# GDMCF/GDMCF

Hardware: AMD Instinct MI355X
Metric: training users/sec (higher is better)
Workload: dtype f32; 1 GPU; yelp-shape synthetic rows, batch=400/GPU, dims=[1000], T=5, noise_scale=0.01, linear-var, mean_type=x0, reweight, AdamW lr=1e-5 (BASELINE configs[1]); n_items=34395, global_batch=400, parallelism=dp1, batch_rows=device CSR rows (CsrBatch)

## Files before the change

### gdmcf_amd/_lib.py

```python
import ctypes
import os
from ctypes import c_char_p, c_double, c_float, c_int, c_int64, c_size_t, c_uint64, c_void_p

_HERE = os.path.dirname(os.path.abspath(__file__))
LIB_PATH = os.path.join(_HERE, "csrc", "libgdmcf_hip.so")

GDMCF_OK, E_SHAPE, E_ARG, E_UNSUPPORTED, E_HIP, E_WORKSPACE = 0, -1, -2, -3, -4, -5
N_TABLES = 13
TABLE_NAMES = (
    "betas", "alphas_cumprod", "alphas_cumprod_prev", "alphas_cumprod_next", "sqrt_alphas_cumprod",
    "sqrt_one_minus_alphas_cumprod", "log_one_minus_alphas_cumprod", "sqrt_recip_alphas_cumprod",
    "sqrt_recipm1_alphas_cumprod", "posterior_variance", "posterior_log_variance_clipped",
    "posterior_mean_coef1", "posterior_mean_coef2",
)

P = c_void_p
_SIGNATURES = {
    "gdmcf_version": (c_int, []),
    "gdmcf_debug_last_gemm": (c_int, []),
    "gdmcf_last_error": (c_char_p, []),
    "gdmcf_device_info": (c_int, [P, P, c_char_p, c_int]),
    "gdmcf_prof_enable": (c_int, [c_int]),
    "gdmcf_prof_collect": (c_int, [c_int, P, P, P]),
    "gdmcf_schedule_build": (c_int, [c_int, c_double, c_double, c_double, c_int, c_int, P]),
    "gdmcf_densify_rows_f32": (c_int, [P, P, P, P, c_int, c_int, P, c_int64, P]),
    "gdmcf_dnn_prep_input_f32": (c_int, [P, c_int64, P, P, P, c_int, P, c_int64, c_int, P, c_int64, c_float, c_uint64,
                                         c_uint64, c_int, P, P, c_int, c_int, c_int, P, c_int64, P, c_int64, P, P, P]),
    "gdmcf_dnn_emb_cols_f32": (c_int, [P, P, P, c_int, c_int, c_int, P, c_int64, P, P]),
    "gdmcf_topn_metrics_f64": (c_int, [P, c_int64, c_int, P, P, P, c_int, P, P]),
    "gdmcf_gemm_precision": (c_int, [c_int]),
    "gdmcf_bf16_shadow_set": (c_int, [P, P, c_int64, c_int64, c_int64]),
    "gdmcf_bf16_shadow_clear": (c_int, [P]),
    "gdmcf_bf16_shadow_get": (P, [P]),
    "gdmcf_bf16_shadow_info": (c_int, [P, P, P, P, P]),
    "gdmcf_bf16_shadow_sync": (c_int, [P, c_int64, P]),
    "gdmcf_linear_ws_bytes": (c_size_t, [c_int, c_int, c_int]),
    "gdmcf_linear_fwd_f32": (c_int, [P, c_int64, P, c_int64, P, c_int, c_int, c_int, c_int, P, c_int64, P, c_size_t, P]),
    "gdmcf_linear_fwd_wt_f32": (c_int, [P, c_int64, P, c_int64, P, c_int, c_int, c_int, c_int, P, c_int64, P, c_size_t, P]),
    "gdmcf_loss_tiles": (c_int, [c_int]),
    "gdmcf_linear_loss_fwd_f32": (c_int, [P, c_int64, P, c_int64, P, P, c_int64, P, c_int, c_int, c_int, P, c_int64, P,
                                          c_int64, P, P, P]),
    "gdmcf_linear_posterior_fwd_f32": (c_int, [P, c_int64, P, c_int64, P, P, c_int64, P, P, P, P, P, P, c_int64, c_int,
                                               c_int, c_int, P, c_int64, P, c_int64, P]),
    "gdmcf_linear_bwd_input_f32": (c_int, [P, c_int64, P, c_int64, P, P, c_int64, c_int, c_int, c_int, c_int, P,
                                           c_int64, P, c_size_t, P]),
    "gdmcf_linear_bwd_weight_f32": (c_int, [P, c_int64, P, c_int64, P, c_int, c_int, c_int, c_int, P, c_int64, P, c_int, P]),
    "gdmcf_linear_bwd_weight_adamw_f32": (c_int, [P, c_int64, P, c_int64, P, c_int, c_int, c_int, c_int, P, c_int64, P, P, P, c_float,
                                                  c_float, c_float, c_float, c_float, c_int, c_float, P]),
    "gdmcf_rowscale_f32": (c_int, [P, c_int64, P, c_int, c_int, P, c_int64, P]),
    "gdmcf_emb_bwd_f32": (c_int, [P, c_int64, P, c_int64, c_int, c_int, P, c_int, c_int, P, P, P, P]),
    "gdmcf_row_loss_finish_f64": (c_int, [P, P, P, P, P, P, c_int, c_int, c_int, P, P, c_int, P, P, P, P]),
    "gdmcf_lt_history_update": (c_int, [P, P, c_int, c_int, c_int, P, P, P]),
    "gdmcf_onehot_noise_f32": (c_int, [P, c_int64, P, c_int, c_int, c_float, P, c_int64, c_uint64, c_uint64, P, c_int64, P,
                                     c_int64, P]),
    "gdmcf_row_norms_f32": (c_int, [P, c_int64, c_int, c_int, P, P, P]),
    "gdmcf_normalize_rows_bwd_f32": (c_int, [P, c_int64, P, c_int64, P, c_int, c_int, P, c_int64, P]),
    "gdmcf_tanh_bwd_f32": (c_int, [P, c_int64, P, c_int64, P, c_int64, P, c_int, c_int, P, c_int64, P]),
    "gdmcf_gather_rows_f32": (c_int, [P, c_int64, P, c_int, c_int, P, c_int64, P]),
    "gdmcf_scatter_add_rows_f32": (c_int, [P, c_int64, P, c_int, c_int, P, c_int64, P]),
    "gdmcf_normalize_rows_bwd_adamw_f32": (c_int, [P, c_int64, P, c_int64, P, c_int, c_int, P, c_int64, P, P, c_float, c_float,
                                                   c_float, c_float, c_float, c_int, c_float, P]),
    "gdmcf_scatter_rows_adamw_f32": (c_int, [P, c_int64, P, c_int, c_int, c_int, P, c_int64, P, P, c_float, c_float, c_float,
                                             c_float, c_float, c_int, c_float, P]),
    "gdmcf_dp_pack_f64": (c_int, [P, P, c_int, P, P, c_int, c_int, c_int, P, P]),
    "gdmcf_dp_unpack_f64": (c_int, [P, P, P, c_int, c_int, c_int, P, P, P]),
    "gdmcf_randn_f32": (c_int, [P, c_int64, c_int, c_int, c_int, c_uint64, c_uint64, P]),
    "gdmcf_eps_target_f32": (c_int, [P, c_int64, P, c_int64, P, c_int64, P, P, P, c_int, c_int, c_int, P, c_int64, P, P, P]),
    "gdmcf_sample_timesteps": (c_int, [P, P, c_int, c_int, c_int, c_double, c_uint64, c_uint64, P, P, P, P]),
    "gdmcf_adamw_f32": (c_int, [P, c_int, c_int, c_float, c_float, c_float, c_float, c_float, c_int, c_float, P]),
    "gdmcf_adamw_bf16s_f32": (c_int, [P, P, c_int, c_int, c_float, c_float, c_float, c_float, c_float, c_int, c_float, P]),
    "gdmcf_topk_masked_f32": (c_int, [P, c_int64, c_int, c_int, P, P, c_int, P, P, P]),
    "gdmcf_spmm_csr_f32": (c_int, [P, P, P, P, c_int, c_int, P, P, c_int, P, P, c_int, P, c_int64, c_int, P, c_int64, P, P, c_int,
                                   c_int64, c_float, c_double, P]),
    "gdmcf_spmm_bundled_f32": (c_int, [P, c_int, P, P, P, P, c_int, P, P, P, P, c_int, P, P, c_int, P, P, c_int64, c_int, c_int, P, c_int64, c_int, P,
                                       c_int64, P, P, c_int, c_int64, c_float, c_double, P]),
    "gdmcf_spmm_stream_f32": (c_int, [P, c_int, P, c_int64, P, c_int, P, P, c_int, c_int, c_int, P, c_int64, c_int, P, c_int64, P, P,
                                      c_int, c_int64, c_float, c_double, P]),
    "gdmcf_graph_guided_step_u8": (c_int, [P, c_int64, P, c_int, c_int, c_float, P, c_int64, P, P, c_int, c_uint64, c_uint64, P,
                                           c_int64, P, P]),
    "gdmcf_debug_spmm_stamps": (c_int, [c_int, P]),
    "gdmcf_graph_state_bytes": (c_int, []),
    "gdmcf_adam_hyper_bytes": (c_int, []),
    "gdmcf_graph_state_init": (c_int, [P, c_uint64, c_uint64, c_int64, c_int64, c_int64, P]),
    "gdmcf_adam_hyper_fill": (c_int, [P, c_int, c_float, c_float, c_float, c_float, c_float, c_int64, c_float]),
    "gdmcf_graph_state_bind": (c_int, [P]),
    "gdmcf_graph_state_tick": (c_int, [P, P]),
    "gdmcf_row_loss_finish_mean_f64": (c_int, [P, P, P, P, P, P, c_int, c_int, c_int, P, P, c_int, P, P, P, P, P, P]),
    "gdmcf_dnn_prep_input_csr_f32": (c_int, [P, P, P, P, P, P, c_int, P, c_int64, c_int, P, c_int64, c_float, c_uint64, c_uint64,
                                             P, P, c_int, c_int, c_int, P, c_int64, P, P, c_int64, P]),
    "gdmcf_linear_loss_fwd_bits_f32": (c_int, [P, c_int64, P, c_int64, P, P, c_int64, P, c_int, c_int, c_int, P, c_int64, P,
                                               c_int64, P, P, P]),
    "gdmcf_scale_f32": (c_int, [P, c_int64, c_float, P, P]),
}
EXPORTED_SYMBOLS = tuple(_SIGNATURES)

_lib = None


def load():
    global _lib
    if _lib is not None:
        return _lib
    if not os.path.exists(LIB_PATH):
        raise ImportError(
            f"{LIB_PATH} is missing: build it with `python -m gdmcf_amd.build` (hipcc, gfx950). "
            "gdmcf_amd has no CPU / PyTorch fallback.")
    lib = ctypes.CDLL(LIB_PATH)
    for name, (res, args) in _SIGNATURES.items():
        fn = getattr(lib, name)
        fn.restype = res
        fn.argtypes = args
    if lib.gdmcf_version() != 1:
        raise ImportError("libgdmcf_hip.so ABI version mismatch; rebuild with `python -m gdmcf_amd.build --force`")
    _lib = lib
    return lib


_EXC = {E_SHAPE: AssertionError, E_ARG: ValueError, E_UNSUPPORTED: NotImplementedError, E_HIP: RuntimeError,
        E_WORKSPACE: RuntimeError}


def check(rc):
    if rc != GDMCF_OK:
        msg = load().gdmcf_last_error().decode(errors="replace")
        raise _EXC.get(rc, RuntimeError)(msg or f"gdmcf error {rc}")


def ptr(t):
    return None if t is None else t.data_ptr()


def require_gpu(t, what):
    if not t.is_cuda:
        raise RuntimeError(f"gdmcf_amd: {what} must live on the MI355X (got device '{t.device}'); "
                           "the HIP path has no CPU fallback")


def shadow_info(data_ptr):
    p16 = ctypes.c_void_p()
    rows, cols, ld = ctypes.c_int64(), ctypes.c_int64(), ctypes.c_int64()
    if not load().gdmcf_bf16_shadow_info(data_ptr, ctypes.byref(p16), ctypes.byref(rows), ctypes.byref(cols), ctypes.byref(ld)):
        return None
    return int(p16.value), int(rows.value), int(cols.value), int(ld.value)


def stream_ptr():
    import torch
    return torch.cuda.current_stream().cuda_stream


def philox_randn(shape, device, seed, offset, stream_id=4, out=None):
    import torch
    rows, cols = int(shape[0]), int(shape[1])
    if out is None:
        out = torch.empty(rows, cols, dtype=torch.float32, device=device)
    require_gpu(out, "philox_randn output")
    check(load().gdmcf_randn_f32(out.data_ptr(), out.stride(0), rows, cols, int(stream_id), int(seed) & (2 ** 64 - 1),
                                 int(offset) & (2 ** 64 - 1), stream_ptr()))
    return out


def schedule_tables(kind, noise_scale, noise_min, noise_max, steps, beta_fixed=True):
    import numpy as np
    out = np.zeros((N_TABLES, steps), dtype=np.float64)
    rc = load().gdmcf_schedule_build(kind, float(noise_scale), float(noise_min), float(noise_max), int(steps),
                                     int(bool(beta_fixed)), out.ctypes.data_as(c_void_p))
    check(rc)
    return out


class Bf16Shadow:

    def __init__(self, t, sync=True):
        import weakref

        import torch
        require_gpu(t, "bf16 shadow source")
        if t.dim() != 2 or t.dtype != torch.float32 or t.stride(1) != 1:
            raise RuntimeError("gdmcf_amd: a bf16 shadow needs a 2-D float32 tensor with unit column stride")
        self.rows, self.cols = t.shape
        self.ptr = t.data_ptr()
        self.ld = t.stride(0)
        self.buf = torch.zeros((self.rows + 63) // 64 * 64, (self.cols + 63) // 64 * 64, dtype=torch.bfloat16,
                               device=t.device)
        self._lib = load()
        self._fin = weakref.finalize(self, self._lib.gdmcf_bf16_shadow_clear, self.ptr)
        self.register()
        if sync:
            self.sync()

    def register(self):
        check(self._lib.gdmcf_bf16_shadow_set(self.ptr, self.buf.data_ptr(), self.rows, self.cols, self.buf.stride(0)))

    def unregister(self):
        self._lib.gdmcf_bf16_shadow_clear(self.ptr)

    def sync(self):
        check(self._lib.gdmcf_bf16_shadow_sync(self.ptr, self.ld, stream_ptr()))

    def close(self):
        self._fin()
```

### gdmcf_amd/csrc/common.h

```cpp
#pragma once
#include <hip/hip_runtime.h>
#include <stdint.h>
#include <stdio.h>

#include "../../include/gdmcf_hip.h"

typedef float f32x4 __attribute__((ext_vector_type(4)));

void gdmcf_set_error(const char* fmt, ...);

#define GD_CHECK_SHAPE(cond, msg)            \
    do {                                     \
        if (!(cond)) {                       \
            gdmcf_set_error("%s", msg);      \
            return GDMCF_E_SHAPE;            \
        }                                    \
    } while (0)

#define GD_CHECK_ARG(cond, msg)              \
    do {                                     \
        if (!(cond)) {                       \
            gdmcf_set_error("%s", msg);      \
            return GDMCF_E_ARG;              \
        }                                    \
    } while (0)

static inline int gd_launch_status(const char* what) {
    hipError_t e = hipGetLastError();
    if (e != hipSuccess) {
        gdmcf_set_error("%s: %s", what, hipGetErrorString(e));
        return GDMCF_E_HIP;
    }
    return GDMCF_OK;
}

extern bool g_gd_prof_on;
void gd_prof_begin(int tag, double work, hipStream_t s);
void gd_prof_end(hipStream_t s);
struct GdProfScope {
    hipStream_t s;
    bool on;
    GdProfScope(int tag, double work, hipStream_t st) : s(st), on(g_gd_prof_on) {
        if (on) gd_prof_begin(tag, work, s);
    }
    ~GdProfScope() {
        if (on) gd_prof_end(s);
    }
};

static inline int gd_cdiv(int a, int b) { return (a + b - 1) / b; }
static inline bool gd_aligned16(const void* p) { return (reinterpret_cast<uintptr_t>(p) & 15u) == 0; }

struct GdShadow {
    void* p16;
    int64_t ld16;
    int64_t rows, cols;
};
bool gd_shadow_lookup(const void* f32, GdShadow* out);
int gd_cast_bf16(const float* src, int64_t ld, void* dst, int64_t ld16, int64_t rows, int64_t cols, hipStream_t s);

enum { GD_LAY_KC = 0, GD_LAY_MC = 1 };
enum { GD_EPI_SLAB = 0, GD_EPI_BIAS_ACT = 1, GD_EPI_LOSS = 2, GD_EPI_POST = 3, GD_EPI_STORE = 4, GD_EPI_ADAMW = 5 };

struct GdAdamHyper {
    float decay;
    float one_m_b1;
    float beta2;
    float one_m_b2;
    float bc2_sqrt;
    float eps;
    float neg_step;
    float grad_scale;
    float inv_bc2_sqrt;
    float pad_[3];
};
GdAdamHyper gd_adam_hyper(float lr, float beta1, float beta2, float eps, float weight_decay, int step, float grad_scale);

__device__ __forceinline__ void gd_adam_elem(float& p, float g, float& m, float& v, const GdAdamHyper& h) {
#pragma clang fp contract(off)
    g = g * h.grad_scale;
    p = p * h.decay;
    m = __builtin_fmaf(g - m, h.one_m_b1, m);
    v = __builtin_fmaf(h.one_m_b2 * g, g, v * h.beta2);
    const float denom = __builtin_fmaf(__builtin_amdgcn_sqrtf(v), h.inv_bc2_sqrt, h.eps);
    p = __builtin_fmaf(h.neg_step * m, __builtin_amdgcn_rcpf(denom), p);
}

struct GdStepState {
    uint64_t prep_offset;
    uint64_t ts_offset;
    int64_t adam_step;
    int64_t table_first;
    int64_t table_len;
    const GdAdamHyper* hyper_table;
    GdAdamHyper hyper;
};
extern thread_local const GdStepState* t_gd_step_state;

struct GdGemm {
    const float* A;
    int64_t lda;
    const float* B;
    int64_t ldb;
    int M, N, K;
    int kchunk;
    int splits;
    int tiles_m, tiles_n;
    int m_fastest;
    float* C;
    int64_t ldc;
    int64_t slab_stride;
    const float* bias;
    int act;
    const float* aux;
    int64_t ldaux;
    const uint32_t* aux_bits;
    int64_t ldbits;
    const float* aux2;
    int64_t ldaux2;
    const float* r0;
    const float* r1;
    const float* r2;
    const float* r3;
    const float* r4;
    float* out2;
    int64_t ldout2;
    float* rowpart;
    int ld_rowpart;
    int accumulate;
    int prof_tag;
    GdAdamHyper adam;
    const GdAdamHyper* adam_dev;
    const void* A16;
    int64_t lda16;
    const void* B16;
    int64_t ldb16;
    void* C16;
    int64_t ldc16;
    size_t ws_cap;
    int dbg;
    int bf16;
};

int gd_dr_kn_splits(int M, int N, int K);
extern thread_local int t_gd_last_gemm;

int gd_gemm_launch(int layA, int layB, int epi, int shape_class, GdGemm& g, hipStream_t s);
int gd_gemm_bf16_launch(int layA, int layB, int epi, int shape_class, GdGemm& g, hipStream_t s);
int gd_gemm_split_launch(int layA, int layB, int epi, int shape_class, GdGemm& g, hipStream_t s);
int gd_gemm_small_launch(int layA, int layB, int epi, GdGemm& g, hipStream_t s);
enum { GD_DR_NOT_TAKEN = 1 };
int gd_gemm_dr_launch(int layA, int layB, int epi, GdGemm& g, hipStream_t s);
int gd_gemm_tile_m(int shape_class);
int gd_gemm_tile_n(int shape_class);
int gd_gemm_bk(int layA, int layB);
int gd_pick_shape_class(int M, int N);
```

### gdmcf_amd/csrc/gemm_dr.hip

```cpp
#include <stdlib.h>

#include "common.h"

namespace {

typedef int i32x4 __attribute__((ext_vector_type(4)));
typedef unsigned int u32x4 __attribute__((ext_vector_type(4)));
typedef f32x4 f32x4_dr_u __attribute__((aligned(4)));

__device__ unsigned int g_dr_ticket[32][8][32];

__device__ __forceinline__ i32x4 dr_srd(const void* p, uint32_t bytes) {
    const uint64_t a = (uint64_t)p;
    return i32x4{(int)(uint32_t)a, (int)((uint32_t)(a >> 32) & 0xffffu), (int)bytes, 0x00020000};
}

__device__ __forceinline__ f32x4 dr_load(i32x4 srd, uint32_t voff, uint32_t soff) {
    f32x4 v;
    asm volatile("buffer_load_dwordx4 %0, %1, %2, %3 offen" : "=v"(v) : "v"(voff), "s"(srd), "s"(soff) : "memory");
    return v;
}

template <int N>
__device__ __forceinline__ void dr_wait() {
    asm volatile("s_waitcnt vmcnt(%0)" ::"n"(N) : "memory");
}

__device__ __forceinline__ unsigned int dr_ticket_issue(unsigned int* ctr) {
    unsigned int t;
    unsigned long long save;
    const unsigned int zero = 0, one = 1;
    asm volatile("s_mov_b64 %1, exec\n\ts_mov_b64 exec, 1\n\tglobal_atomic_add %0, %2, %3, %4 sc0\n\ts_mov_b64 exec, %1"
                 : "=&v"(t), "=&s"(save) : "v"(zero), "v"(one), "s"(ctr) : "memory");
    return t;
}

#ifndef GD_ADAMW_DBG
#define GD_ADAMW_DBG 0
#endif
#ifndef DR_ADAM_UB
#define DR_ADAM_UB 2
#endif

struct DrArgs {
    GdGemm g;
    int tiles_m, tiles_n, m_fastest;
    int ksp;
    int ctr;
    const GdAdamHyper* adam_dev;
    int stagger;
};

template <int TA, int TB, int D, int EPI>
__global__ __launch_bounds__(512, 2) void dr_tn_kernel(const DrArgs d) {
    static_assert(EPI == GD_EPI_STORE, "plain weight-gradient product (the fused-AdamW form: dr_tn_adamw_kernel)");
    constexpr int LPS = TA + TB;
    constexpr int R = D + 1;
    static_assert(LPS * D <= 63, "vmcnt is a 6-bit counter");
    const GdGemm& g = d.g;
    const int lane = threadIdx.x & 63;
    const int r = lane & 15, q = lane >> 4;
    const int n_waves = gridDim.x * 8;
    const int minor = d.m_fastest ? d.tiles_m : d.tiles_n;
    const int panels = d.m_fastest ? d.tiles_n : d.tiles_m;
    int xcc;
    asm volatile("s_getreg_b32 %0, hwreg(HW_REG_XCC_ID)" : "=s"(xcc));
    int qx = xcc & 7;
    int visited = 0;
    auto q_tiles = [&](int x) { return ((panels - x + 7) >> 3) * minor; };
    auto tile_of = [&](int x, int t) {
        const int p = (t / minor) * 8 + x, i = t % minor;
        return p * minor + i;
    };
    auto draw_blocking = [&]() {
        for (;;) {
            if (visited == 8) return -1;
            unsigned int* c = &g_dr_ticket[d.ctr][qx][0];
            unsigned int tk = dr_ticket_issue(c);
            dr_wait<0>();
            asm volatile("" : "+v"(tk));
            const int t = __builtin_amdgcn_readfirstlane(tk);
            const int n = q_tiles(qx);
            if (t == n + n_waves - 1 && lane == 0) __hip_atomic_store(c, 0u, __ATOMIC_RELAXED, __HIP_MEMORY_SCOPE_AGENT);
            if (t < n) return tile_of(qx, t);
            qx = (qx + 1) & 7;
            ++visited;
        }
    };
    if (d.stagger > 0 && __builtin_amdgcn_readfirstlane(threadIdx.x) >= 256)
        for (int i = 0; i < d.stagger; ++i) __builtin_amdgcn_s_sleep(127);
    int cur = draw_blocking();
    if (cur < 0) return;
    const int ntiles = d.tiles_m * d.tiles_n;
    const int KSP = d.ksp;
    const i32x4 srdA = dr_srd(g.A, (uint32_t)(((int64_t)(g.K - 1) * g.lda + g.M) * 4));
    const i32x4 srdB = dr_srd(g.B, (uint32_t)(((int64_t)(g.K - 1) * g.ldb + g.N) * 4));
    const uint32_t sa = 16u * (uint32_t)g.lda, sb = 16u * (uint32_t)g.ldb;
    const uint32_t c_bytes = (uint32_t)(((int64_t)(g.M - 1) * g.ldc + (g.out2 ? g.N - 1 : g.N)) * 4);
    const __amdgpu_buffer_rsrc_t srdC = __builtin_amdgcn_make_buffer_rsrc(g.C, 0, (int)c_bytes, 0x00020000);

    uint32_t offA[TA], offB[TB];
    uint32_t ka = 0, kb = 0;
    int l_left = KSP;
    auto set_cursor = [&](int tile) {
        const bool ok = tile < ntiles;
        const int tm = d.m_fastest ? (tile % d.tiles_m) : (tile / d.tiles_n);
        const int tn = d.m_fastest ? (tile / d.tiles_m) : (tile % d.tiles_n);
#pragma unroll
        for (int a = 0; a < TA; ++a) offA[a] = ok ? (uint32_t)(q * g.lda + tm * (64 * TA) + 64 * a + 4 * r) * 4u : 0xFFFFFFF0u;
#pragma unroll
        for (int b = 0; b < TB; ++b) offB[b] = ok ? (uint32_t)(q * g.ldb + tn * (64 * TB) + 64 * b + 4 * r) * 4u : 0xFFFFFFF0u;
        ka = kb = 0;
        l_left = KSP;
    };
    set_cursor(cur);
    f32x4 ra[R][TA], rb[R][TB];
#pragma unroll
    for (int u = 0; u < D; ++u) {
#pragma unroll
        for (int a = 0; a < TA; ++a) ra[u][a] = dr_load(srdA, offA[a], ka);
#pragma unroll
        for (int b = 0; b < TB; ++b) rb[u][b] = dr_load(srdB, offB[b], kb);
        ka += sa;
        kb += sb;
        --l_left;
    }
    const int q1 = (KSP / R / 4) * R, q2 = (KSP / R / 2) * R, q3 = (KSP / R * 3 / 4) * R;
    for (;;) {
        unsigned int* tctr = &g_dr_ticket[d.ctr][qx][0];
        unsigned int tick = visited < 8 ? dr_ticket_issue(tctr) : 0u;
        const bool drew = visited < 8;
        int nxt = 0;
        const int tm = d.m_fastest ? (cur % d.tiles_m) : (cur / d.tiles_n);
        const int tn = d.m_fastest ? (cur / d.tiles_m) : (cur % d.tiles_n);
        const int m0 = tm * 64 * TA, n0 = tn * 64 * TB;
        f32x4 acc[TA][4][TB][4];
#pragma unroll
        for (int a = 0; a < TA; ++a)
#pragma unroll
            for (int e = 0; e < 4; ++e)
#pragma unroll
                for (int b = 0; b < TB; ++b)
#pragma unroll
                    for (int f = 0; f < 4; ++f) acc[a][e][b][f] = f32x4{0.f, 0.f, 0.f, 0.f};
        __builtin_amdgcn_s_setprio(0);
        for (int s0 = 0; s0 < KSP; s0 += R) {
            if (s0 == q1) __builtin_amdgcn_s_setprio(1);
            else if (s0 == q2) __builtin_amdgcn_s_setprio(2);
            else if (s0 == q3) __builtin_amdgcn_s_setprio(3);
#pragma unroll
            for (int u = 0; u < R; ++u) {
                constexpr int NM = 16 * TA * TB;
                const int v = (u + D) % R;
                dr_wait<LPS*(D - 1)>();
#pragma unroll
                for (int a = 0; a < TA; ++a) asm volatile("" : "+v"(ra[u][a]));
#pragma unroll
                for (int b = 0; b < TB; ++b) asm volatile("" : "+v"(rb[u][b]));
#pragma unroll
                for (int i = 0; i < NM; ++i) {
                    const int a = i / (16 * TB), e = (i / (4 * TB)) % 4, b = (i / 4) % TB, f = i % 4;
                    acc[a][e][b][f] = __builtin_amdgcn_mfma_f32_16x16x4f32(ra[u][a][e], rb[u][b][f], acc[a][e][b][f], 0, 0, 0);
                    if (i % 4 == 1 && i / 4 < LPS) {
                        __builtin_amdgcn_sched_barrier(0);
                        const int l = i / 4;
                        if (l < TA) ra[v][l] = dr_load(srdA, offA[l], ka);
                        else rb[v][l - TA] = dr_load(srdB, offB[l - TA], kb);
                        __builtin_amdgcn_sched_barrier(0);
                    }
                    if (i == 4 * LPS + 1) {
                        __builtin_amdgcn_sched_barrier(0);
                        ka += sa;
                        kb += sb;
                        if (--l_left == 0) {
                            nxt = -1;
                            if (drew) {
                                if (KSP < 2 * D + 2) dr_wait<0>();
                                asm volatile("" : "+v"(tick));
                                const int tk = __builtin_amdgcn_readfirstlane(tick);
                                const int nq = q_tiles(qx);
                                if (tk == nq + n_waves - 1 && lane == 0) __hip_atomic_store(tctr, 0u, __ATOMIC_RELAXED, __HIP_MEMORY_SCOPE_AGENT);
                                if (tk < nq) {
                                    nxt = tile_of(qx, tk);
                                } else {
                                    qx = (qx + 1) & 7;
                                    ++visited;
                                    nxt = draw_blocking();
                                }
                            }
                            if (nxt < 0) nxt = ntiles;
                            set_cursor(nxt);
                        }
                        __builtin_amdgcn_sched_barrier(0);
                    }
                }
                __builtin_amdgcn_sched_barrier(0);
            }
        }
#pragma unroll
        for (int b = 0; b < TB; ++b) {
            const int n = n0 + 64 * b + 4 * r;
            const uint32_t vo = (uint32_t)(16 * q * g.ldc + n) * 4u;
            if (n + 3 < (g.out2 ? g.N - 1 : g.N)) {
#pragma unroll
                for (int a = 0; a < TA; ++a)
#pragma unroll
                    for (int t = 0; t < 4; ++t)
#pragma unroll
                        for (int e = 0; e < 4; ++e) {
                            f32x4 gv = {acc[a][e][b][0][t], acc[a][e][b][1][t], acc[a][e][b][2][t], acc[a][e][b][3][t]};
                            const uint32_t so = (uint32_t)(m0 + 64 * a + 4 * t + e) * (uint32_t)g.ldc * 4u;
                            __builtin_amdgcn_raw_buffer_store_b128(__builtin_bit_cast(u32x4, gv), srdC, vo + so, 0, 0);
                        }
            } else if (n < g.N) {
                for (int a = 0; a < TA; ++a)
                    for (int t = 0; t < 4; ++t)
                        for (int e = 0; e < 4; ++e) {
                            const int m = m0 + 64 * a + 16 * q + 4 * t + e;
                            if (m >= g.M) continue;
                            for (int k = 0; k < 4; ++k) {
                                if (n + k >= g.N) continue;
                                const float gk = acc[a][e][b][k][t];
                                if (g.out2 && n + k == g.N - 1) g.out2[m] = gk;
                                else g.C[(int64_t)m * g.ldc + n + k] = gk;
                            }
                        }
            }
        }
        if (nxt >= ntiles) break;
        cur = nxt;
    }
    dr_wait<0>();
#pragma unroll
    for (int u = 0; u < R; ++u) {
#pragma unroll
        for (int a = 0; a < TA; ++a) asm volatile("" ::"v"(ra[u][a]));
#pragma unroll
        for (int b = 0; b < TB; ++b) asm volatile("" ::"v"(rb[u][b]));
    }
}

#ifdef GD_NO_SNOP
#define GD_SNOP ""
#else
#define GD_SNOP "s_nop 4\n\t"
#endif
#ifndef GD_ADAMW_ST
#define GD_ADAMW_ST 1
#endif
__device__ __forceinline__ void dr_store(f32x4 v, i32x4 srd, uint32_t voff) {
#if GD_ADAMW_ST == 1
    asm volatile(GD_SNOP "buffer_store_dwordx4 %0, %1, %2, 0 offen nt\n\ts_nop 1" ::"v"(v), "v"(voff), "s"(srd) : "memory");
#elif GD_ADAMW_ST == 2
    asm volatile(GD_SNOP "buffer_store_dwordx4 %0, %1, %2, 0 offen sc1\n\ts_nop 1" ::"v"(v), "v"(voff), "s"(srd) : "memory");
#elif GD_ADAMW_ST == 3
    asm volatile(GD_SNOP "buffer_store_dwordx4 %0, %1, %2, 0 offen sc0 sc1\n\ts_nop 1" ::"v"(v), "v"(voff), "s"(srd) : "memory");
#else
    asm volatile(GD_SNOP "buffer_store_dwordx4 %0, %1, %2, 0 offen\n\ts_nop 1" ::"v"(v), "v"(voff), "s"(srd) : "memory");
#endif
}
#ifndef GD_ADAMW_LD
#define GD_ADAMW_LD 0
#endif
template <bool NTL>
__device__ __forceinline__ void dr_load0_rw(f32x4& v, i32x4 srd, uint32_t voff) {
    if constexpr (NTL) {
        asm volatile(GD_SNOP "buffer_load_dwordx4 %0, %1, %2, 0 offen nt" : "+v"(v) : "v"(voff), "s"(srd) : "memory");
        return;
    }
#if GD_ADAMW_LD == 1
    asm volatile(GD_SNOP "buffer_load_dwordx4 %0, %1, %2, 0 offen nt" : "+v"(v) : "v"(voff), "s"(srd) : "memory");
#elif GD_ADAMW_LD == 2
    asm volatile(GD_SNOP "buffer_load_dwordx4 %0, %1, %2, 0 offen sc1" : "+v"(v) : "v"(voff), "s"(srd) : "memory");
#elif GD_ADAMW_LD == 3
    asm volatile(GD_SNOP "buffer_load_dwordx4 %0, %1, %2, 0 offen sc0 sc1" : "+v"(v) : "v"(voff), "s"(srd) : "memory");
#elif GD_ADAMW_LD == 4
    asm volatile(GD_SNOP "buffer_load_dwordx4 %0, %1, %2, 0 offen sc0 sc1 nt" : "+v"(v) : "v"(voff), "s"(srd) : "memory");
#else
    asm volatile(GD_SNOP "buffer_load_dwordx4 %0, %1, %2, 0 offen" : "+v"(v) : "v"(voff), "s"(srd) : "memory");
#endif
}

template <int D, bool NTL>
__global__ __launch_bounds__(512, 2) void dr_tn_adamw_kernel(const DrArgs d) {
    constexpr int LPS = 2;
    constexpr int R = D + 1;
    constexpr int UA = 1, UB = 1 + R / 2;
    constexpr int XS = 6;
    constexpr int XR = 12;
    static_assert(UB < R && UB > UA, "two distinct steps of a round");
    static_assert(LPS * R + XS <= 63, "vmcnt is a 6-bit counter");
    constexpr uint32_t PARK = 0xFFFFFF00u;
    const GdGemm& g = d.g;
    const int lane = threadIdx.x & 63;
    const int wave = __builtin_amdgcn_readfirstlane(threadIdx.x >> 6);
    const int r = lane & 15, q = lane >> 4;
    extern __shared__ __attribute__((aligned(16))) float dr_lds[];
    f32x4* const stash = reinterpret_cast<f32x4*>(dr_lds + wave * 4096) + lane;
    GdAdamHyper hy = g.adam;
    if (d.adam_dev) hy = *d.adam_dev;
    const int n_waves = gridDim.x * 8;
    const int minor = d.m_fastest ? d.tiles_m : d.tiles_n;
    const int panels = d.m_fastest ? d.tiles_n : d.tiles_m;
    int xcc;
    asm volatile("s_getreg_b32 %0, hwreg(HW_REG_XCC_ID)" : "=s"(xcc));
    int qx = xcc & 7, visited = 0;
    auto q_tiles = [&](int x) { return ((panels - x + 7) >> 3) * minor; };
    auto tile_of = [&](int x, int t) { return ((t / minor) * 8 + x) * minor + t % minor; };
    auto draw_blocking = [&]() {
        for (;;) {
            if (visited == 8) return -1;
            unsigned int* c = &g_dr_ticket[d.ctr][qx][0];
            unsigned int tk = dr_ticket_issue(c);
            dr_wait<0>();
            asm volatile("" : "+v"(tk));
            const int t = __builtin_amdgcn_readfirstlane(tk);
            const int n = q_tiles(qx);
            if (t == n + n_waves - 1 && lane == 0) __hip_atomic_store(c, 0u, __ATOMIC_RELAXED, __HIP_MEMORY_SCOPE_AGENT);
            if (t < n) return tile_of(qx, t);
            qx = (qx + 1) & 7;
            ++visited;
        }
    };
    if (d.stagger > 0 && __builtin_amdgcn_readfirstlane(threadIdx.x) >= 256)
        for (int i = 0; i < d.stagger; ++i) __builtin_amdgcn_s_sleep(127);
    int cur = draw_blocking();
    if (cur < 0) return;
    const int ntiles = d.tiles_m * d.tiles_n;
    const int KSP = d.ksp;
    const i32x4 srdA = dr_srd(g.A, (uint32_t)(((int64_t)(g.K - 1) * g.lda + g.M) * 4));
    const i32x4 srdB = dr_srd(g.B, (uint32_t)(((int64_t)(g.K - 1) * g.ldb + g.N) * 4));
    const uint32_t sa = 16u * (uint32_t)g.lda, sb = 16u * (uint32_t)g.ldb;
    const int n_lim = g.out2 ? g.N - 1 : g.N;
    const uint32_t c_bytes = (uint32_t)(((int64_t)(g.M - 1) * g.ldc + n_lim) * 4);
    const i32x4 srdW = dr_srd(g.C, c_bytes), srdM = dr_srd(g.aux, c_bytes), srdV = dr_srd(g.aux2, c_bytes);
    const uint32_t ldc4 = (uint32_t)g.ldc * 4u;

    uint32_t offA, offB, ka = 0, kb = 0;
    int l_left = KSP;
    auto set_cursor = [&](int tile) {
        const bool ok = tile < ntiles;
        const int tm = d.m_fastest ? (tile % d.tiles_m) : (tile / d.tiles_n);
        const int tn = d.m_fastest ? (tile / d.tiles_m) : (tile % d.tiles_n);
        offA = ok ? (uint32_t)(q * g.lda + tm * 64 + 4 * r) * 4u : 0xFFFFFFF0u;
        offB = ok ? (uint32_t)(q * g.ldb + tn * 64 + 4 * r) * 4u : 0xFFFFFFF0u;
        ka = kb = 0;
        l_left = KSP;
    };
    set_cursor(cur);
    uint32_t pend_base = PARK;
    bool pend_lane = false;
    int pend_g = 16;
    struct Slot {
        f32x4 p, m, v;
        uint32_t off;
        int gi;
        bool live;
    } sl[2];
#pragma unroll
    for (int k = 0; k < 2; ++k) {
        asm volatile("" : "=v"(sl[k].p));
        asm volatile("" : "=v"(sl[k].m));
        asm volatile("" : "=v"(sl[k].v));
        sl[k].off = PARK;
        sl[k].gi = 0;
        sl[k].live = false;
    }
    auto opt_pick = [&](Slot& s_) {
        const bool act = pend_g < 16;
        s_.live = act;
        s_.gi = act ? pend_g : 0;
        s_.off = (act && pend_lane && !(GD_ADAMW_DBG & 2)) ? pend_base + (uint32_t)pend_g * ldc4 : PARK;
        pend_g += act ? 1 : 0;
    };
    auto opt_update_store = [&](Slot& s_) {
        const float* sg = reinterpret_cast<const float*>(stash + 256 * (s_.gi & 3)) + (s_.gi >> 2);
        float gr[4];
#pragma unroll
        for (int f = 0; f < 4; ++f) gr[f] = sg[256 * f];
        f32x4 pn = s_.p, mn = s_.m, vn = s_.v;
#if !(GD_ADAMW_DBG & 1)
#pragma unroll
        for (int k = 0; k < 4; ++k) {
            float pk = pn[k], mk = mn[k], vk = vn[k];
            gd_adam_elem(pk, gr[k], mk, vk, hy);
            pn[k] = pk;
            mn[k] = mk;
            vn[k] = vk;
        }
#else
        pn[0] += gr[0] + gr[1] + gr[2] + gr[3];
#endif
        const uint32_t so = (GD_ADAMW_DBG & 8) ? PARK : ((GD_ADAMW_DBG & 16) && s_.off != PARK) ? s_.off + 448u * ldc4 : s_.off;
        dr_store(pn, srdW, so);
        dr_store(mn, srdM, so);
        dr_store(vn, srdV, so);
    };
    auto opt_load = [&](Slot& s_) {
        const uint32_t lo = (GD_ADAMW_DBG & 4) ? PARK : s_.off;
        dr_load0_rw<NTL>(s_.p, srdW, lo);
        dr_load0_rw<NTL>(s_.m, srdM, lo);
        dr_load0_rw<NTL>(s_.v, srdV, lo);
    };
    auto opt_pin = [&](Slot& s_) {
        asm volatile("" : "+v"(s_.p));
        asm volatile("" : "+v"(s_.m));
        asm volatile("" : "+v"(s_.v));
    };

    f32x4 ra[R], rb[R];
#pragma unroll
    for (int u = 0; u < D; ++u) {
        ra[u] = dr_load(srdA, offA, ka);
        rb[u] = dr_load(srdB, offB, kb);
        ka += sa;
        kb += sb;
        --l_left;
        const int w = (u + 1) % R;
        if (w == UA || w == UB) {
            const f32x4 z = {0.f, 0.f, 0.f, 0.f};
#pragma unroll
            for (int k = 0; k < XS / 3; ++k) {
                dr_store(z, srdW, PARK);
                dr_store(z, srdM, PARK);
                dr_store(z, srdV, PARK);
            }
        }
    }
    const int q1 = (KSP / R / 4) * R, q2 = (KSP / R / 2) * R, q3 = (KSP / R * 3 / 4) * R;
    const bool defer_all = KSP / R >= 9;
    for (;;) {
        unsigned int* tctr = &g_dr_ticket[d.ctr][qx][0];
        unsigned int tick = visited < 8 ? dr_ticket_issue(tctr) : 0u;
        const bool drew = visited < 8;
        int nxt = 0;
        const int tm = d.m_fastest ? (cur % d.tiles_m) : (cur / d.tiles_n);
        const int tn = d.m_fastest ? (cur / d.tiles_m) : (cur % d.tiles_n);
        const int m0 = tm * 64, n0 = tn * 64;
        f32x4 acc[4][4];
#pragma unroll
        for (int e = 0; e < 4; ++e)
#pragma unroll
            for (int f = 0; f < 4; ++f) acc[e][f] = f32x4{0.f, 0.f, 0.f, 0.f};
        __builtin_amdgcn_s_setprio(0);
        for (int s0 = 0; s0 < KSP; s0 += R) {
            if (s0 == q1) __builtin_amdgcn_s_setprio(1);
            else if (s0 == q2) __builtin_amdgcn_s_setprio(2);
            else if (s0 == q3) __builtin_amdgcn_s_setprio(3);
#pragma unroll
            for (int u = 0; u < R; ++u) {
                const int v = (u + D) % R;
                if (u == UA || u == UB) dr_wait<LPS*(D - 1) + XR - XS>();
                else dr_wait<LPS*(D - 1) + XR>();
                asm volatile("" : "+v"(ra[u]));
                asm volatile("" : "+v"(rb[u]));
#pragma unroll
                for (int i = 0; i < 16; ++i) {
                    const int e = i / 4, f = i % 4;
                    acc[e][f] = __builtin_amdgcn_mfma_f32_16x16x4f32(ra[u][e], rb[u][f], acc[e][f], 0, 0, 0);
                    if (i == 1) {
                        __builtin_amdgcn_sched_barrier(0);
                        ra[v] = dr_load(srdA, offA, ka);
                        __builtin_amdgcn_sched_barrier(0);
                    } else if (i == 5) {
                        __builtin_amdgcn_sched_barrier(0);
                        rb[v] = dr_load(srdB, offB, kb);
                        __builtin_amdgcn_sched_barrier(0);
                    } else if (i == 9) {
                        __builtin_amdgcn_sched_barrier(0);
                        ka += sa;
                        kb += sb;
                        if (--l_left == 0) {
                            nxt = -1;
                            if (drew) {
                                if (KSP < 2 * D + 2) dr_wait<0>();
                                asm volatile("" : "+v"(tick));
                                const int tk = __builtin_amdgcn_readfirstlane(tick);
                                const int nq = q_tiles(qx);
                                if (tk == nq + n_waves - 1 && lane == 0) __hip_atomic_store(tctr, 0u, __ATOMIC_RELAXED, __HIP_MEMORY_SCOPE_AGENT);
                                if (tk < nq) {
                                    nxt = tile_of(qx, tk);
                                } else {
                                    qx = (qx + 1) & 7;
                                    ++visited;
                                    nxt = draw_blocking();
                                }
                            }
                            if (nxt < 0) nxt = ntiles;
                            set_cursor(nxt);
                        }
                        __builtin_amdgcn_sched_barrier(0);
                    } else if ((u == UA || u == UB) && i == 11) {
                        __builtin_amdgcn_sched_barrier(0);
                        Slot& s_ = sl[u == UA ? 0 : 1];
                        dr_wait<LPS * R + XS>();
                        opt_pin(s_);
                        opt_update_store(s_);
                        opt_pick(s_);
                        opt_load(s_);
                        __builtin_amdgcn_sched_barrier(0);
                    }
                }
                __builtin_amdgcn_sched_barrier(0);
            }
        }
        const uint32_t vo = (uint32_t)(16 * q * g.ldc + n0 + 4 * r) * 4u;
        const int n = n0 + 4 * r;
        const bool lane_full = n + 3 < n_lim;
        if (defer_all) {
#pragma unroll
            for (int e = 0; e < 4; ++e)
#pragma unroll
                for (int f = 0; f < 4; ++f) stash[64 * (4 * e + f)] = acc[e][f];
            pend_base = vo + (uint32_t)m0 * ldc4;
            pend_lane = lane_full;
            pend_g = 0;
        } else if (lane_full) {
            const __amdgpu_buffer_rsrc_t rW = __builtin_amdgcn_make_buffer_rsrc(g.C, 0, (int)c_bytes, 0x00020000);
            const __amdgpu_buffer_rsrc_t rM = __builtin_amdgcn_make_buffer_rsrc(const_cast<float*>(g.aux), 0, (int)c_bytes, 0x00020000);
            const __amdgpu_buffer_rsrc_t rV = __builtin_amdgcn_make_buffer_rsrc(const_cast<float*>(g.aux2), 0, (int)c_bytes, 0x00020000);
#pragma unroll
            for (int t = 0; t < 4; ++t)
#pragma unroll
                for (int e = 0; e < 4; ++e) {
                    const uint32_t o = vo + (uint32_t)(m0 + 4 * t + e) * ldc4;
                    f32x4 pv = __builtin_bit_cast(f32x4, __builtin_amdgcn_raw_buffer_load_b128(rW, o, 0, 0));
                    f32x4 mv = __builtin_bit_cast(f32x4, __builtin_amdgcn_raw_buffer_load_b128(rM, o, 0, 0));
                    f32x4 vv = __builtin_bit_cast(f32x4, __builtin_amdgcn_raw_buffer_load_b128(rV, o, 0, 0));
#pragma unroll
                    for (int k = 0; k < 4; ++k) {
                        float pk = pv[k], mk = mv[k], vk = vv[k];
                        gd_adam_elem(pk, acc[e][k][t], mk, vk, hy);
                        pv[k] = pk;
                        mv[k] = mk;
                        vv[k] = vk;
                    }
                    __builtin_amdgcn_raw_buffer_store_b128(__builtin_bit_cast(u32x4, pv), rW, o, 0, 0);
                    __builtin_amdgcn_raw_buffer_store_b128(__builtin_bit_cast(u32x4, mv), rM, o, 0, 0);
                    __builtin_amdgcn_raw_buffer_store_b128(__builtin_bit_cast(u32x4, vv), rV, o, 0, 0);
                }
        }
        if (!lane_full && n < g.N) {
            float* __restrict__ Mo = const_cast<float*>(g.aux);
            float* __restrict__ Vo = const_cast<float*>(g.aux2);
            for (int t = 0; t < 4; ++t)
                for (int e = 0; e < 4; ++e) {
                    const int m = m0 + 16 * q + 4 * t + e;
                    if (m >= g.M) continue;
                    for (int k = 0; k < 4; ++k) {
                        if (n + k >= g.N) continue;
                        const int64_t o = (int64_t)m * g.ldc + n + k;
                        const float gk = acc[e][k][t];
                        if (g.out2 && n + k == g.N - 1) {
                            g.out2[m] = gk;
                            continue;
                        }
                        float pk = g.C[o], mk = Mo[o], vk = Vo[o];
                        gd_adam_elem(pk, gk, mk, vk, hy);
                        g.C[o] = pk;
                        Mo[o] = mk;
                        Vo[o] = vk;
                    }
                }
        }
        if (nxt >= ntiles) break;
        cur = nxt;
    }
    dr_wait<0>();
#pragma unroll
    for (int u = 0; u < R; ++u) {
        asm volatile("" ::"v"(ra[u]));
        asm volatile("" ::"v"(rb[u]));
    }
#pragma unroll
    for (int k = 0; k < 2; ++k) {
        opt_pin(sl[k]);
        opt_update_store(sl[k]);
    }
    dr_wait<0>();
    {
        const __amdgpu_buffer_rsrc_t rW = __builtin_amdgcn_make_buffer_rsrc(g.C, 0, (int)c_bytes, 0x00020000);
        const __amdgpu_buffer_rsrc_t rM = __builtin_amdgcn_make_buffer_rsrc(const_cast<float*>(g.aux), 0, (int)c_bytes, 0x00020000);
        const __amdgpu_buffer_rsrc_t rV = __builtin_amdgcn_make_buffer_rsrc(const_cast<float*>(g.aux2), 0, (int)c_bytes, 0x00020000);
        for (; pend_g < 16; pend_g += 4) {
            f32x4 pv[4], mv[4], vv[4];
            uint32_t oo[4];
#pragma unroll
            for (int u = 0; u < 4; ++u) {
                oo[u] = (pend_lane && !(GD_ADAMW_DBG & 2)) ? pend_base + (uint32_t)(pend_g + u) * ldc4 : PARK;
                pv[u] = __builtin_bit_cast(f32x4, __builtin_amdgcn_raw_buffer_load_b128(rW, oo[u], 0, 0));
                mv[u] = __builtin_bit_cast(f32x4, __builtin_amdgcn_raw_buffer_load_b128(rM, oo[u], 0, 0));
                vv[u] = __builtin_bit_cast(f32x4, __builtin_amdgcn_raw_buffer_load_b128(rV, oo[u], 0, 0));
            }
#pragma unroll
            for (int u = 0; u < 4; ++u) {
                const int gi = pend_g + u;
                const float* sg = reinterpret_cast<const float*>(stash + 256 * (gi & 3)) + (gi >> 2);
#pragma unroll
                for (int k = 0; k < 4; ++k) {
                    float pk = pv[u][k], mk = mv[u][k], vk = vv[u][k];
                    gd_adam_elem(pk, sg[256 * k], mk, vk, hy);
                    pv[u][k] = pk;
                    mv[u][k] = mk;
                    vv[u][k] = vk;
                }
                __builtin_amdgcn_raw_buffer_store_b128(__builtin_bit_cast(u32x4, pv[u]), rW, oo[u], 0, 2);
                __builtin_amdgcn_raw_buffer_store_b128(__builtin_bit_cast(u32x4, mv[u]), rM, oo[u], 0, 2);
                __builtin_amdgcn_raw_buffer_store_b128(__builtin_bit_cast(u32x4, vv[u]), rV, oo[u], 0, 2);
            }
        }
    }
}

template <int TMB, int NB, int D, int EPI>
__global__ __launch_bounds__(512, 2) void dr_nt_kernel(const DrArgs d) {
    static_assert(EPI == GD_EPI_BIAS_ACT || EPI == GD_EPI_LOSS || EPI == GD_EPI_POST, "forward products");
    static_assert(NB == 4 || NB == 2, "B loads per chunk: 16 NB output columns, NB consecutive ones per lane");
    constexpr int LPC = TMB + NB;
    constexpr int R = D + 1;
    constexpr int NM = 4 * TMB * NB;
    constexpr int SP = NM / (LPC + 1);
    static_assert(SP >= 2 && SP * LPC + 1 < NM, "loads and cursor step must fall inside the chunk");
    static_assert(LPC * D <= 63, "vmcnt is a 6-bit counter");
    const GdGemm& g = d.g;
    const int lane = threadIdx.x & 63;
    const int r = lane & 15, q = lane >> 4;
    const int ntiles = d.tiles_m * d.tiles_n;
    unsigned int* ctr = &g_dr_ticket[d.ctr][0][0];
    const int n_waves = gridDim.x * 8;
    int cur = __builtin_amdgcn_readfirstlane(blockIdx.x * 8 + (threadIdx.x >> 6));
    if (cur >= ntiles) return;
    if (d.stagger > 0 && __builtin_amdgcn_readfirstlane(threadIdx.x) >= 256)
        for (int i = 0; i < d.stagger; ++i) __builtin_amdgcn_s_sleep(127);
    const int NCP = d.ksp;
    const i32x4 srdA = dr_srd(g.A, (uint32_t)(((int64_t)(g.M - 1) * g.lda + g.K) * 4));
    const i32x4 srdB = dr_srd(g.B, (uint32_t)(((int64_t)(g.N - 1) * g.ldb + g.K) * 4));

    uint32_t offA[TMB], offB[NB];
    uint32_t kc = 0;
    int l_left = NCP;
    auto set_cursor = [&](int tile) {
        const bool ok = tile < ntiles;
        const int tm = tile % d.tiles_m, tn = tile / d.tiles_m;
#pragma unroll
        for (int i = 0; i < TMB; ++i) offA[i] = ok ? (uint32_t)((tm * (16 * TMB) + 16 * i + r) * g.lda + 4 * q) * 4u : 0xFFFFFFF0u;
#pragma unroll
        for (int f = 0; f < NB; ++f) offB[f] = ok ? (uint32_t)((tn * (16 * NB) + NB * r + f) * g.ldb + 4 * q) * 4u : 0xFFFFFFF0u;
        kc = 0;
        l_left = NCP;
    };
    set_cursor(cur);
    f32x4 xa[R][TMB], xb[R][NB];
#pragma unroll
    for (int u = 0; u < D; ++u) {
#pragma unroll
        for (int i = 0; i < TMB; ++i) xa[u][i] = dr_load(srdA, offA[i], kc);
#pragma unroll
        for (int f = 0; f < NB; ++f) xb[u][f] = dr_load(srdB, offB[f], kc);
        kc += 64;
        --l_left;
    }
    const int q1 = (NCP / R / 4) * R, q2 = (NCP / R / 2) * R, q3 = (NCP / R * 3 / 4) * R;
    const int c_mask = g.K >> 4;
    for (;;) {
        unsigned int tick = dr_ticket_issue(ctr);
        int nxt = 0;
        const int tm = cur % d.tiles_m, tn = cur / d.tiles_m;
        const int m0 = tm * 16 * TMB, n0 = tn * (16 * NB);
        f32x4 acc[TMB][NB];
#pragma unroll
        for (int i = 0; i < TMB; ++i)
#pragma unroll
            for (int f = 0; f < NB; ++f) acc[i][f] = f32x4{0.f, 0.f, 0.f, 0.f};
        __builtin_amdgcn_s_setprio(0);
        for (int c0 = 0; c0 < NCP; c0 += R) {
            if (c0 == q1) __builtin_amdgcn_s_setprio(1);
            else if (c0 == q2) __builtin_amdgcn_s_setprio(2);
            else if (c0 == q3) __builtin_amdgcn_s_setprio(3);
#pragma unroll
            for (int u = 0; u < R; ++u) {
                const int v = (u + D) % R;
                dr_wait<LPC*(D - 1)>();
#pragma unroll
                for (int i = 0; i < TMB; ++i) asm volatile("" : "+v"(xa[u][i]));
#pragma unroll
                for (int f = 0; f < NB; ++f) asm volatile("" : "+v"(xb[u][f]));
                if (c0 + u >= c_mask) {
                    const int kq = (c0 + u) * 16 + 4 * q;
#pragma unroll
                    for (int e = 0; e < 4; ++e) {
                        const bool keep = kq + e < g.K;
#pragma unroll
                        for (int i = 0; i < TMB; ++i) xa[u][i][e] = keep ? xa[u][i][e] : 0.f;
#pragma unroll
                        for (int f = 0; f < NB; ++f) xb[u][f][e] = keep ? xb[u][f][e] : 0.f;
                    }
                }
#pragma unroll
                for (int n = 0; n < NM; ++n) {
                    const int e = n / (TMB * NB), i = (n / NB) % TMB, f = n % NB;
                    acc[i][f] = __builtin_amdgcn_mfma_f32_16x16x4f32(xa[u][i][e], xb[u][f][e], acc[i][f], 0, 0, 0);
                    if (n % SP == 1 && n / SP < LPC) {
                        __builtin_amdgcn_sched_barrier(0);
                        const int l = n / SP;
                        if (l < TMB) xa[v][l] = dr_load(srdA, offA[l], kc);
                        else xb[v][l - TMB] = dr_load(srdB, offB[l - TMB], kc);
                        __builtin_amdgcn_sched_barrier(0);
                    }
                    if (n == SP * LPC + 1) {
                        __builtin_amdgcn_sched_barrier(0);
                        kc += 64;
                        if (--l_left == 0) {
                            if (NCP < 2 * D + 2) dr_wait<0>();
                            asm volatile("" : "+v"(tick));
                            const int tk = __builtin_amdgcn_readfirstlane(tick);
                            if (tk == ntiles - 1 && lane == 0) __hip_atomic_store(ctr, 0u, __ATOMIC_RELAXED, __HIP_MEMORY_SCOPE_AGENT);
                            nxt = n_waves + tk;
                            set_cursor(nxt);
                        }
                        __builtin_amdgcn_sched_barrier(0);
                    }
                }
                __builtin_amdgcn_sched_barrier(0);
            }
        }
        typedef float vecnb __attribute__((ext_vector_type(NB)));
        typedef vecnb vecnb_u __attribute__((aligned(4)));
        const int n = n0 + NB * r;
        const bool full = n + NB - 1 < g.N;
        float biasv[NB];
#pragma unroll
        for (int f = 0; f < NB; ++f) biasv[f] = g.bias ? g.bias[min(n + f, g.N - 1)] : 0.f;
        const bool has_z = (EPI == GD_EPI_POST) && (g.aux2 != nullptr);
        const bool has_r = (EPI == GD_EPI_POST) && (g.r2 != nullptr);
        auto put = [&](float* base, int64_t ld, int m, const float (&val)[NB]) {
            if (full) {
                vecnb w;
#pragma unroll
                for (int f = 0; f < NB; ++f) w[f] = val[f];
                *reinterpret_cast<vecnb_u*>(base + (int64_t)m * ld + n) = w;
            } else {
                for (int f = 0; f < NB; ++f)
                    if (n + f < g.N) base[(int64_t)m * ld + n + f] = val[f];
            }
        };
#pragma unroll
        for (int i = 0; i < TMB; ++i) {
            float racc[4];
#pragma unroll
            for (int t = 0; t < 4; ++t) {
                const int m = m0 + 16 * i + 4 * q + t;
                const int mc = min(m, g.M - 1);
                const bool mok = m < g.M;
                float v4[NB];
#pragma unroll
                for (int f = 0; f < NB; ++f) v4[f] = acc[i][f][t] + biasv[f];
                racc[t] = 0.f;
                if (EPI == GD_EPI_BIAS_ACT) {
                    if (g.act == 1) {
#pragma unroll
                        for (int f = 0; f < NB; ++f) v4[f] = tanhf(v4[f]);
                    }
                    if (mok) put(g.C, g.ldc, m, v4);
                } else if (EPI == GD_EPI_LOSS) {
                    const float c1 = g.r0 ? g.r0[mc] : 1.f;
                    float tg[NB];
                    if (g.aux_bits) {
                        const uint32_t w = g.aux_bits[(int64_t)mc * g.ldbits + min((int64_t)(n >> 5), g.ldbits - 1)];
#pragma unroll
                        for (int f = 0; f < NB; ++f) tg[f] = (float)((w >> ((n & 31) + f)) & 1u);
                    } else {
#pragma unroll
                        for (int f = 0; f < NB; ++f) tg[f] = g.aux[(int64_t)mc * g.ldaux + min(n + f, g.N - 1)];
                    }
                    float dd[NB], ss = 0.f;
#pragma unroll
                    for (int f = 0; f < NB; ++f) {
                        dd[f] = c1 * v4[f] - tg[f];
                        if (mok && n + f < g.N) ss += dd[f] * dd[f];
                    }
                    if (mok) {
                        put(g.C, g.ldc, m, dd);
                        if (g.out2) put(g.out2, g.ldout2, m, v4);
                    }
                    racc[t] = ss;
                } else {
                    const float c1 = g.r0[mc], c2 = g.r1[mc];
                    const float p1 = has_r ? g.r2[mc] : 0.f, p2 = has_r ? g.r3[mc] : 0.f;
                    const float sg = has_z ? g.r4[mc] : 0.f;
                    float pr[NB], mn[NB];
#pragma unroll
                    for (int f = 0; f < NB; ++f) {
                        const int nf = min(n + f, g.N - 1);
                        const float xt = g.aux[(int64_t)mc * g.ldaux + nf];
                        const float zz = has_z ? g.aux2[(int64_t)mc * g.ldaux2 + nf] : 0.f;
                        pr[f] = has_r ? (p1 * xt - p2 * v4[f]) : v4[f];
                        mn[f] = c1 * pr[f] + c2 * xt;
                        if (has_z) mn[f] += sg * zz;
                    }
                    if (mok) {
                        put(g.C, g.ldc, m, mn);
                        if (g.out2) put(g.out2, g.ldout2, m, pr);
                    }
                }
            }
            if (EPI == GD_EPI_LOSS) {
#pragma unroll
                for (int t = 0; t < 4; ++t) {
                    float sv = racc[t];
                    sv += __shfl_xor(sv, 1);
                    sv += __shfl_xor(sv, 2);
                    sv += __shfl_xor(sv, 4);
                    sv += __shfl_xor(sv, 8);
                    const int m = m0 + 16 * i + 4 * q + t;
                    if (r == 0 && m < g.M) g.rowpart[(int64_t)m * g.ld_rowpart + tn] = sv;
                }
            }
            __builtin_amdgcn_sched_barrier(0);
        }
        if (nxt >= ntiles) break;
        cur = nxt;
    }
    dr_wait<0>();
#pragma unroll
    for (int u = 0; u < R; ++u) {
#pragma unroll
        for (int i = 0; i < TMB; ++i) asm volatile("" ::"v"(xa[u][i]));
#pragma unroll
        for (int f = 0; f < NB; ++f) asm volatile("" ::"v"(xb[u][f]));
    }
}


__device__ __forceinline__ f32x4 dr_load_g(i32x4 srd, uint32_t voff, uint32_t soff) {
    f32x4 v;
    asm volatile("s_nop 4\n\tbuffer_load_dwordx4 %0, %1, %2, %3 offen" : "=v"(v) : "v"(voff), "s"(srd), "s"(soff) : "memory");
    return v;
}
__device__ __forceinline__ float dr_load1_g(i32x4 srd, uint32_t voff, uint32_t soff) {
    float v;
    asm volatile("s_nop 4\n\tbuffer_load_dword %0, %1, %2, %3 offen" : "=v"(v) : "v"(voff), "s"(srd), "s"(soff) : "memory");
    return v;
}


__global__ __launch_bounds__(256) void dr_transpose_kernel(const float* __restrict__ A, int64_t lda, int M, int K,
                                                           float* __restrict__ At, int ldt) {
    __shared__ float t[32][33];
    const int k0 = blockIdx.x * 32, m0 = blockIdx.y * 32;
    const int x = threadIdx.x & 31, y = threadIdx.x >> 5;
#pragma unroll
    for (int i = 0; i < 4; ++i) {
        const int m = m0 + y + 8 * i, k = k0 + x;
        t[y + 8 * i][x] = (m < M && k < K) ? A[(int64_t)m * lda + k] : 0.f;
    }
    __syncthreads();
#pragma unroll
    for (int i = 0; i < 4; ++i) {
        const int k = k0 + y + 8 * i, m = m0 + x;
        if (k < K && m < M) At[(int64_t)k * ldt + m] = t[x][y + 8 * i];
    }
}

__device__ __forceinline__ void dr_load_rw(f32x4& v, i32x4 srd, uint32_t voff, uint32_t soff) {
    asm volatile("buffer_load_dwordx4 %0, %1, %2, %3 offen" : "+v"(v) : "v"(voff), "s"(srd), "s"(soff) : "memory");
}
__device__ __forceinline__ void dr_load1_rw(float& v, i32x4 srd, uint32_t voff, uint32_t soff) {
    asm volatile("buffer_load_dword %0, %1, %2, %3 offen" : "+v"(v) : "v"(voff), "s"(srd), "s"(soff) : "memory");
}
#ifdef HL_NOA
#define HL_KA(x) (0x80000000u)
#else
#define HL_KA(x) (x)
#endif
#ifdef HL_NOB
#define HL_KB(x) (0x80000000u)
#else
#define HL_KB(x) (x)
#endif
template <int EPI>
__global__ __launch_bounds__(512, 2) void dr_hl_kernel(const DrArgs d) {
    static_assert(EPI == GD_EPI_LOSS, "output layer with the fused row loss");
    constexpr int LPS = 3;
    constexpr int D = 7;
    static_assert(LPS * D <= 63, "vmcnt is a 6-bit counter");
    const GdGemm& g = d.g;
    const int lane = threadIdx.x & 63;
    const int wave = __builtin_amdgcn_readfirstlane(threadIdx.x >> 6);
    const int r = lane & 15, q = lane >> 4;
    extern __shared__ __attribute__((aligned(16))) float dr_lds[];
    float* const lds = dr_lds + wave * 4096;
    const int w_ev = (lane >> 3) * 32 + (((lane & 7) ^ (lane >> 4)) << 2), w_od = w_ev ^ 16;
    const int r_h0 = r * 32 + ((q ^ ((r >> 1) & 7)) << 2), r_h1 = r_h0 ^ 16;

    const int n_waves = gridDim.x * (blockDim.x >> 6);
    const int minor = d.tiles_m, panels = d.tiles_n;
    int xcc;
    asm volatile("s_getreg_b32 %0, hwreg(HW_REG_XCC_ID)" : "=s"(xcc));
    int qx = xcc & 7, visited = 0;
    auto q_tiles = [&](int x) { return ((panels - x + 7) >> 3) * minor; };
    auto tile_of = [&](int x, int t) { return ((t / minor) * 8 + x) * minor + t % minor; };
    auto draw_blocking = [&]() {
        for (;;) {
            if (visited == 8) return -1;
            unsigned int* c = &g_dr_ticket[d.ctr][qx][0];
            unsigned int tk = dr_ticket_issue(c);
            dr_wait<0>();
            asm volatile("" : "+v"(tk));
            const int t = __builtin_amdgcn_readfirstlane(tk);
            const int n = q_tiles(qx);
            if (t == n + n_waves - 1 && lane == 0) __hip_atomic_store(c, 0u, __ATOMIC_RELAXED, __HIP_MEMORY_SCOPE_AGENT);
            if (t < n) return tile_of(qx, t);
            qx = (qx + 1) & 7;
            ++visited;
        }
    };
    if (d.stagger > 0 && __builtin_amdgcn_readfirstlane(threadIdx.x) >= 256)
        for (int i = 0; i < d.stagger; ++i) __builtin_amdgcn_s_sleep(127);
    int cur = draw_blocking();
    if (cur < 0) return;
    const int NCH = d.ksp;
    const i32x4 srdA = dr_srd(g.A, (uint32_t)(((int64_t)(g.K - 1) * g.lda + g.M) * 4));
    const i32x4 srdB = dr_srd(g.B, (uint32_t)(((int64_t)(g.N - 1) * g.ldb + g.K) * 4));
    const uint32_t sa1 = 4u * (uint32_t)g.lda, sa13 = 13u * sa1;
    const uint32_t ub8 = 32u * (uint32_t)g.ldb;
    const int q1 = (NCH / 8) * 2, q2 = (NCH / 4) * 2, q3 = (NCH * 3 / 8) * 2;

    for (;;) {
        unsigned int* tctr = &g_dr_ticket[d.ctr][qx][0];
        const bool drew = visited < 8;
        unsigned int tick = drew ? dr_ticket_issue(tctr) : 0u;
        const int tm = cur % d.tiles_m, tn = cur / d.tiles_m;
        const int m0 = tm * 80, n0 = tn * 64;
        const uint32_t oA4 = (uint32_t)(4 * q * g.lda + m0 + 4 * r) * 4u;
        const uint32_t oA1 = (uint32_t)(4 * q * g.lda + m0 + 64 + r) * 4u;
        const uint32_t oB = (uint32_t)(((int64_t)(n0 + (lane >> 3)) * g.ldb + 4 * (lane & 7)) * 4);
        uint32_t ka = 0;
        f32x4 ra4[8], G[8], FB[2][4];
        float ra1[8];
        f32x4 acc[5][4];
#pragma unroll
        for (int e = 0; e < 5; ++e)
#pragma unroll
            for (int b = 0; b < 4; ++b) acc[e][b] = f32x4{0.f, 0.f, 0.f, 0.f};
        __builtin_amdgcn_s_setprio(0);
#pragma unroll
        for (int u = 0; u < 8; ++u) G[u] = dr_load_g(srdB, oB, (uint32_t)u * ub8);
        dr_wait<0>();
#pragma unroll
        for (int u = 0; u < 8; ++u) {
            asm volatile("" : "+v"(G[u]));
            *reinterpret_cast<f32x4*>(lds + u * 256 + ((u & 1) ? w_od : w_ev)) = G[u];
        }
        G[0] = dr_load_g(srdB, oB, 128u);
#pragma unroll
        for (int u = 1; u < 8; ++u) {
            ra4[u - 1] = dr_load_g(srdA, oA4, ka);
            ra1[u - 1] = dr_load1_g(srdA, oA1, ka);
            ka += ((u - 1) & 3) == 3 ? sa13 : sa1;
            G[u] = dr_load_g(srdB, oB, 128u + (uint32_t)u * ub8);
        }
        dr_wait<21>();
        asm volatile("" : "=v"(ra4[7]));
        asm volatile("" : "=v"(ra1[7]));
        asm volatile("" : "+v"(G[0]));
        *reinterpret_cast<f32x4*>(lds + 2048 + w_ev) = G[0];
#pragma unroll
        for (int b = 0; b < 4; ++b) FB[0][b] = *reinterpret_cast<const f32x4*>(lds + b * 512 + r_h0);
        uint32_t kb = 256u;

        for (int c0 = 0; c0 < NCH; c0 += 2) {
            if (c0 == q1) __builtin_amdgcn_s_setprio(1);
            else if (c0 == q2) __builtin_amdgcn_s_setprio(2);
            else if (c0 == q3) __builtin_amdgcn_s_setprio(3);
#pragma unroll
            for (int uu = 0; uu < 16; ++uu) {
                const int p = uu >> 3, u = uu & 7, h = u >> 2, sx = u & 3;
                const int v = (u + 7) & 7;
                const int w = (u + 1) & 7;
                const uint32_t kbs = (c0 + p + 2 < NCH) ? kb : 0x80000000u;
                dr_wait<LPS * (D - 1)>();
                asm volatile("" : "+v"(ra4[u]));
                asm volatile("" : "+v"(ra1[u]));
                asm volatile("" : "+v"(G[w]));
                *reinterpret_cast<f32x4*>(lds + ((u < 7) ? (1 - p) : p) * 2048 + w * 256 + ((w & 1) ? w_od : w_ev)) = G[w];
                __builtin_amdgcn_sched_barrier(0);
#pragma unroll
                for (int i = 0; i < 20; ++i) {
                    const int e = i >> 2, b = i & 3;
                    const float av = e < 4 ? ra4[u][e] : ra1[u];
                    acc[e][b] = __builtin_amdgcn_mfma_f32_16x16x4f32(av, FB[h][b][sx], acc[e][b], 0, 0, 0);
                    if (i == 1) {
                        __builtin_amdgcn_sched_barrier(0);
                        dr_load_rw(ra4[v], srdA, oA4, HL_KA(ka));
                        __builtin_amdgcn_sched_barrier(0);
                    } else if (i == 5) {
                        __builtin_amdgcn_sched_barrier(0);
                        dr_load1_rw(ra1[v], srdA, oA1, HL_KA(ka));
                        ka += (v & 3) == 3 ? sa13 : sa1;
                        __builtin_amdgcn_sched_barrier(0);
                    } else if (i == 9) {
                        __builtin_amdgcn_sched_barrier(0);
                        dr_load_rw(G[u], srdB, oB, HL_KB(kbs + (uint32_t)u * ub8));
                        if (u == 7) kb += 128u;
                        __builtin_amdgcn_sched_barrier(0);
                    } else if (i == 13 && u == 3) {
                        __builtin_amdgcn_sched_barrier(0);
#pragma unroll
                        for (int bb = 0; bb < 4; ++bb) FB[1][bb] = *reinterpret_cast<const f32x4*>(lds + p * 2048 + bb * 512 + r_h1);
                        __builtin_amdgcn_sched_barrier(0);
                    } else if (i == 13 && u == 7) {
                        __builtin_amdgcn_sched_barrier(0);
#pragma unroll
                        for (int bb = 0; bb < 4; ++bb) FB[0][bb] = *reinterpret_cast<const f32x4*>(lds + (1 - p) * 2048 + bb * 512 + r_h0);
                        __builtin_amdgcn_sched_barrier(0);
                    }
                }
                __builtin_amdgcn_sched_barrier(0);
            }
        }
        dr_wait<0>();
#pragma unroll
        for (int u = 0; u < 8; ++u) {
            asm volatile("" ::"v"(ra4[u]));
            asm volatile("" ::"v"(ra1[u]));
            asm volatile("" ::"v"(G[u]));
        }
        int nxt = -1;
        if (drew) {
            asm volatile("" : "+v"(tick));
            const int tk = __builtin_amdgcn_readfirstlane(tick);
            const int nq = q_tiles(qx);
            if (tk == nq + n_waves - 1 && lane == 0) __hip_atomic_store(tctr, 0u, __ATOMIC_RELAXED, __HIP_MEMORY_SCOPE_AGENT);
            if (tk < nq) {
                nxt = tile_of(qx, tk);
            } else {
                qx = (qx + 1) & 7;
                ++visited;
                nxt = -2;
            }
        }
        {
            int ncl[4];
            bool nok[4];
            float biasv[4];
#pragma unroll
            for (int b = 0; b < 4; ++b) {
                const int n = n0 + 16 * b + r;
                nok[b] = n < g.N;
                ncl[b] = min(n, g.N - 1);
                biasv[b] = g.bias ? g.bias[ncl[b]] : 0.f;
            }
#pragma unroll
            for (int e = 0; e < 5; ++e) {
                float tg[4][4], c1v[4];
#pragma unroll
                for (int t = 0; t < 4; ++t) {
                    const int m = e < 4 ? m0 + 16 * q + 4 * t + e : m0 + 64 + 4 * q + t;
                    const int mc = min(m, g.M - 1);
                    c1v[t] = g.r0 ? g.r0[mc] : 1.f;
                    if (g.aux_bits) {
                        uint32_t wv[2];
#pragma unroll
                        for (int jj = 0; jj < 2; ++jj)
                            wv[jj] = g.aux_bits[(int64_t)mc * g.ldbits + min((int64_t)((n0 >> 5) + jj), g.ldbits - 1)];
#pragma unroll
                        for (int b = 0; b < 4; ++b) tg[t][b] = (float)((wv[b >> 1] >> (16 * (b & 1) + r)) & 1u);
                    } else {
#pragma unroll
                        for (int b = 0; b < 4; ++b) tg[t][b] = g.aux[(int64_t)mc * g.ldaux + ncl[b]];
                    }
                }
#pragma unroll
                for (int t = 0; t < 4; ++t) {
                    const int m = e < 4 ? m0 + 16 * q + 4 * t + e : m0 + 64 + 4 * q + t;
                    const bool mok = m < g.M;
                    float ss = 0.f;
#pragma unroll
                    for (int b = 0; b < 4; ++b) {
                        const float vv = acc[e][b][t] + biasv[b];
                        const float dd = c1v[t] * vv - tg[t][b];
                        if (mok && nok[b]) {
                            if (g.out2) g.out2[(int64_t)m * g.ldout2 + ncl[b]] = vv;
                            g.C[(int64_t)m * g.ldc + ncl[b]] = dd;
                            ss += dd * dd;
                        }
                    }
                    ss += __shfl_xor(ss, 1);
                    ss += __shfl_xor(ss, 2);
                    ss += __shfl_xor(ss, 4);
                    ss += __shfl_xor(ss, 8);
                    if (r == 0 && mok) g.rowpart[(int64_t)m * g.ld_rowpart + tn] = ss;
                }
                __builtin_amdgcn_sched_barrier(0);
            }
        }
        if (nxt == -2) nxt = draw_blocking();
        if (nxt < 0) break;
        cur = nxt;
    }
}

template <int NB, int EPI>
__global__ __launch_bounds__(256, 1) void dr_fat_kernel(const DrArgs d) {
    static_assert(EPI == GD_EPI_LOSS || EPI == GD_EPI_POST, "output layer with a fused epilogue");
    static_assert(NB >= 4 && NB <= 12, "5 x NB accumulator blocks must fit 256 registers");
    constexpr int TMB = 5;
    const GdGemm& g = d.g;
    const int lane = threadIdx.x & 63;
    const int wave = __builtin_amdgcn_readfirstlane(threadIdx.x >> 6);
    const int r = lane & 15, q = lane >> 4;
    extern __shared__ __attribute__((aligned(16))) float dr_lds[];
    float* const lds = dr_lds + wave * (2 * NB * 256);
    const int nblk = gridDim.x, per = nblk >> 3;
    const int wl = ((nblk & 7) == 0 ? ((int)(blockIdx.x & 7) * per + (int)(blockIdx.x >> 3)) : (int)blockIdx.x) * 4 + wave;
    const int n_waves = nblk * 4;
    const int ntiles = d.tiles_m * d.tiles_n;
    const __amdgpu_buffer_rsrc_t srdA = __builtin_amdgcn_make_buffer_rsrc(const_cast<float*>(g.A), 0, (int)(((int64_t)(g.M - 1) * g.lda + g.K) * 4), 0x00020000);
    const __amdgpu_buffer_rsrc_t srdB = __builtin_amdgcn_make_buffer_rsrc(const_cast<float*>(g.B), 0, (int)(((int64_t)(g.N - 1) * g.ldb + g.K) * 4), 0x00020000);
    const int NCH = d.ksp;
    const int c_mask = g.K >> 4;
    const int w_off = (lane >> 2) * 16 + (((lane & 3) ^ ((((lane >> 2) >> 2) & 1) << 1)) << 2);
    const int r_off = r * 16 + ((q ^ (((r >> 2) & 1) << 1)) << 2);
    for (int tile = wl; tile < ntiles; tile += n_waves) {
        const int tm = tile % d.tiles_m, tn = tile / d.tiles_m;
        const int m0 = tm * (16 * TMB), n0 = tn * (16 * NB);
        uint32_t offA[TMB], offB[NB];
#pragma unroll
        for (int i = 0; i < TMB; ++i) offA[i] = (uint32_t)((m0 + 16 * i + r) * g.lda + 4 * q) * 4u;
#pragma unroll
        for (int p = 0; p < NB; ++p) offB[p] = (uint32_t)(((int64_t)(n0 + 16 * p + (lane >> 2)) * g.ldb + 4 * (lane & 3)) * 4);
        f32x4 acc[TMB][NB];
#pragma unroll
        for (int i = 0; i < TMB; ++i)
#pragma unroll
            for (int b = 0; b < NB; ++b) acc[i][b] = f32x4{0.f, 0.f, 0.f, 0.f};
        f32x4 xa[2][TMB], G[NB], FB[NB];
#pragma unroll
        for (int i = 0; i < TMB; ++i) xa[0][i] = __builtin_bit_cast(f32x4, __builtin_amdgcn_raw_buffer_load_b128(srdA, offA[i], 0, 0));
#pragma unroll
        for (int p = 0; p < NB; ++p) G[p] = __builtin_bit_cast(f32x4, __builtin_amdgcn_raw_buffer_load_b128(srdB, offB[p], 0, 0));
#pragma unroll
        for (int p = 0; p < NB; ++p) *reinterpret_cast<f32x4*>(lds + p * 256 + w_off) = G[p];

#define GD_FAT_CHUNK(PAR, c)                                                                                          \
        {                                                                                                             \
             \
            const uint32_t kn = ((c) + 1 < NCH) ? (uint32_t)((c) + 1) * 64u : 0x80000000u;                            \
            _Pragma("unroll") for (int b = 0; b < NB; ++b)                                                            \
                FB[b] = *reinterpret_cast<const f32x4*>(lds + (PAR) * (NB * 256) + b * 256 + r_off);                  \
            if ((c) >= c_mask) {  \
                 \
                _Pragma("unroll") for (int e = 0; e < 4; ++e) {                                                       \
                    const bool keep = (c) * 16 + 4 * q + e < g.K;                                                     \
                    _Pragma("unroll") for (int i = 0; i < TMB; ++i) xa[PAR][i][e] = keep ? xa[PAR][i][e] : 0.f;       \
                    _Pragma("unroll") for (int b = 0; b < NB; ++b) FB[b][e] = keep ? FB[b][e] : 0.f;                  \
                }                                                                                                     \
            }                                                                                                         \
            __builtin_amdgcn_sched_barrier(0);                                                                        \
            _Pragma("unroll") for (int sx = 0; sx < 4; ++sx) {                                                        \
                _Pragma("unroll") for (int n = 0; n < TMB * NB; ++n) {                                                \
                    const int i = n / NB, b = n % NB;                                                                 \
                    if (sx == 0 && i == 0) asm volatile("" : "+v"(FB[b]));  \
                    if (sx == 0 && b == 0) asm volatile("" : "+v"(xa[PAR][i]));                                       \
                    acc[i][b] = __builtin_amdgcn_mfma_f32_16x16x4f32(xa[PAR][i][sx], FB[b][sx], acc[i][b], 0, 0, 0);  \
                     \
                    if (sx < 2 && n % 5 == 2) {      \
                        const int l = (sx == 0) ? n / 5 : NB + n / 5;                                                 \
                        if (l < TMB + NB) {                                                                           \
                            __builtin_amdgcn_sched_barrier(0);                                                        \
                            if (l < TMB)                                                                              \
                                xa[(PAR) ^ 1][l] = __builtin_bit_cast(f32x4, __builtin_amdgcn_raw_buffer_load_b128(   \
                                    srdA, offA[l], kn, 0));                                                           \
                            else                                                                                      \
                                G[l - TMB] = __builtin_bit_cast(f32x4, __builtin_amdgcn_raw_buffer_load_b128(         \
                                    srdB, offB[l - TMB], kn, 0));                                                     \
                            __builtin_amdgcn_sched_barrier(0);                                                        \
                        }                                                                                             \
                    }                                                                                                 \
                    if (sx == 3 && n % 4 == 1 && n / 4 < NB) {   \
                        __builtin_amdgcn_sched_barrier(0);                                                            \
                        *reinterpret_cast<f32x4*>(lds + ((PAR) ^ 1) * (NB * 256) + (n / 4) * 256 + w_off) = G[n / 4]; \
                        __builtin_amdgcn_sched_barrier(0);                                                            \
                    }                                                                                                 \
                }                                                                                                     \
                __builtin_amdgcn_sched_barrier(0);                                                                    \
            }                                                                                                         \
        }
        const int c_pf = d.stagger > 0 ? ((NCH > d.stagger + 2 ? NCH - d.stagger : 0) & ~1) : -2;
        for (int c = 0; c + 1 < NCH; c += 2) {
            if constexpr (EPI == GD_EPI_POST) {
                if (c == c_pf) {
                    typedef __attribute__((address_space(3))) void* lds_vp;
                    constexpr int NJL = (16 * NB * 4 + 127) / 128 + 1;
                    constexpr int NPI = (80 * NJL + 63) / 64;
                    float* const scratch = dr_lds + 4 * (2 * NB * 256) + wave * 64;
                    const __amdgpu_buffer_rsrc_t srdX = __builtin_amdgcn_make_buffer_rsrc(
                        const_cast<float*>(g.aux), 0, (int)(((int64_t)(g.M - 1) * g.ldaux + g.N) * 4), 0x00020000);
#pragma unroll
                    for (int pi = 0; pi < NPI; ++pi) {
                        const int t = min(pi * 64 + lane, 80 * NJL - 1);
                        const int row = min(m0 + t % 80, g.M - 1), j = t / 80;
                        const int col = min(j < NJL - 1 ? n0 + 32 * j : n0 + 16 * NB - 1, g.N - 1);
                        __builtin_amdgcn_raw_ptr_buffer_load_lds(srdX, (lds_vp)scratch, 4, (int)(((int64_t)row * g.ldaux + col) * 4), 0, 0, 0);
                    }
                }
            }
            GD_FAT_CHUNK(0, c);
            GD_FAT_CHUNK(1, c + 1);
        }
        if (NCH & 1) GD_FAT_CHUNK(0, NCH - 1);
#undef GD_FAT_CHUNK

        constexpr int LDS_ = 16 * NB + 4;
        constexpr int NJ = (4 * NB + 15) / 16;
        typedef f32x4 f32x4_e __attribute__((aligned(4)));
        f32x4 bias4[NJ];
        int col4[NJ];
#pragma unroll
        for (int j = 0; j < NJ; ++j) {
            col4[j] = n0 + 4 * (r + 16 * j);
            bias4[j] = f32x4{0.f, 0.f, 0.f, 0.f};
            if (g.bias && r + 16 * j < 4 * NB) {
#pragma unroll
                for (int e = 0; e < 4; ++e) bias4[j][e] = g.bias[min(col4[j] + e, g.N - 1)];
            }
        }
        const bool has_z = (EPI == GD_EPI_POST) && (g.aux2 != nullptr);
        const bool has_r = (EPI == GD_EPI_POST) && (g.r2 != nullptr);
        struct Pre {
            f32x4 a[NJ], z[NJ];
            uint32_t w[NJ];
            float c1, c2, p1, p2, sg;
        } pre[2];
        auto fetch = [&](int i, int p4, Pre& P) {
            const int mc = min(m0 + 16 * i + 4 * p4 + q, g.M - 1);
            P.c1 = 1.f; P.c2 = 0.f; P.p1 = 0.f; P.p2 = 0.f; P.sg = 0.f;
            if (EPI == GD_EPI_LOSS) {
                if (g.r0) P.c1 = g.r0[mc];
            } else {
                P.c1 = g.r0[mc];
                P.c2 = g.r1[mc];
                if (has_r) { P.p1 = g.r2[mc]; P.p2 = g.r3[mc]; }
                if (has_z) P.sg = g.r4[mc];
            }
#pragma unroll
            for (int j = 0; j < NJ; ++j) {
                const int n = col4[j];
                const bool whole = (r + 16 * j < 4 * NB) && n + 3 < g.N;
                P.w[j] = 0u;
                P.a[j] = f32x4{0.f, 0.f, 0.f, 0.f};
                P.z[j] = f32x4{0.f, 0.f, 0.f, 0.f};
                if (EPI == GD_EPI_LOSS && g.aux_bits) {
                    P.w[j] = g.aux_bits[(int64_t)mc * g.ldbits + min((int64_t)(n >> 5), g.ldbits - 1)];
                } else if (whole) {
                    P.a[j] = *reinterpret_cast<const f32x4_e*>(g.aux + (int64_t)mc * g.ldaux + n);
                    if (has_z) P.z[j] = *reinterpret_cast<const f32x4_e*>(g.aux2 + (int64_t)mc * g.ldaux2 + n);
                }
            }
        };
        fetch(0, 0, pre[0]);
#pragma unroll
        for (int i = 0; i < TMB; ++i) {
#pragma unroll
            for (int b = 0; b < NB; ++b)
#pragma unroll
                for (int t = 0; t < 4; ++t) lds[(4 * q + t) * LDS_ + 16 * b + r] = acc[i][b][t];
            __builtin_amdgcn_sched_barrier(0);
#pragma unroll
            for (int p4 = 0; p4 < 4; ++p4) {
                const int step = 4 * i + p4;
                const Pre& P = pre[step & 1];
                if (step + 1 < 4 * TMB) fetch((step + 1) >> 2, (step + 1) & 3, pre[(step + 1) & 1]);
                const int m = m0 + 16 * i + 4 * p4 + q;
                const int mc = min(m, g.M - 1);
                const bool mok = m < g.M;
                float ss = 0.f;
                const float c1 = P.c1, c2 = P.c2, p1 = P.p1, p2 = P.p2, sg = P.sg;
#pragma unroll
                for (int j = 0; j < NJ; ++j) {
                    const int c4 = r + 16 * j;
                    const bool inb = c4 < 4 * NB;
                    const int n = col4[j];
                    const bool whole = inb && n + 3 < g.N;
                    const bool full = whole && mok;
                    const f32x4 v = *reinterpret_cast<const f32x4*>(lds + (4 * p4 + q) * LDS_ + 4 * min(c4, 4 * NB - 1));
                    f32x4 o, o2 = f32x4{0.f, 0.f, 0.f, 0.f};
                    if (EPI == GD_EPI_LOSS) {
                        f32x4 tg;
                        if (g.aux_bits) {
                            const uint32_t w = P.w[j] >> (n & 31);
#pragma unroll
                            for (int e = 0; e < 4; ++e) tg[e] = (float)((w >> e) & 1u);
                        } else if (whole) {
                            tg = P.a[j];
                        } else {
#pragma unroll
                            for (int e = 0; e < 4; ++e) tg[e] = g.aux[(int64_t)mc * g.ldaux + min(n + e, g.N - 1)];
                        }
#pragma unroll
                        for (int e = 0; e < 4; ++e) {
                            o2[e] = v[e] + bias4[j][e];
                            o[e] = c1 * o2[e] - tg[e];
                            if (inb && mok && n + e < g.N) ss += o[e] * o[e];
                        }
                    } else {
                        f32x4 xt = P.a[j], zz = P.z[j];
                        if (!whole) {
#pragma unroll
                            for (int e = 0; e < 4; ++e) {
                                xt[e] = g.aux[(int64_t)mc * g.ldaux + min(n + e, g.N - 1)];
                                if (has_z) zz[e] = g.aux2[(int64_t)mc * g.ldaux2 + min(n + e, g.N - 1)];
                            }
                        }
#pragma unroll
                        for (int e = 0; e < 4; ++e) {
                            const float vv = v[e] + bias4[j][e];
                            o2[e] = has_r ? (p1 * xt[e] - p2 * vv) : vv;
                            o[e] = c1 * o2[e] + c2 * xt[e];
                            if (has_z) o[e] += sg * zz[e];
                        }
                    }
                    if (full) {
                        *reinterpret_cast<f32x4_e*>(g.C + (int64_t)m * g.ldc + n) = o;
                        if (g.out2) *reinterpret_cast<f32x4_e*>(g.out2 + (int64_t)m * g.ldout2 + n) = o2;
                    } else if (inb && mok) {
                        for (int e = 0; e < 4 && n + e < g.N; ++e) {
                            g.C[(int64_t)m * g.ldc + n + e] = o[e];
                            if (g.out2) g.out2[(int64_t)m * g.ldout2 + n + e] = o2[e];
                        }
                    }
                }
                if (EPI == GD_EPI_LOSS) {
                    ss += __shfl_xor(ss, 1);
                    ss += __shfl_xor(ss, 2);
                    ss += __shfl_xor(ss, 4);
                    ss += __shfl_xor(ss, 8);
                    if (r == 0 && mok) g.rowpart[(int64_t)m * g.ld_rowpart + tn] = ss;
                }
                __builtin_amdgcn_sched_barrier(0);
            }
        }
    }
}


#ifndef GD_KN_EVERY
#define GD_KN_EVERY 4
#endif
template <int NL>
__global__ __launch_bounds__(256, 1) void dr_kn_kernel(const DrArgs d) {
    constexpr int TMB = 5;
    const GdGemm& g = d.g;
    const int lane = threadIdx.x & 63;
    const int wave = __builtin_amdgcn_readfirstlane(threadIdx.x >> 6);
    const int r = lane & 15, q = lane >> 4;
    const int nblk = gridDim.x, per = nblk >> 3;
    const int wl = ((nblk & 7) == 0 ? ((int)(blockIdx.x & 7) * per + (int)(blockIdx.x >> 3)) : (int)blockIdx.x) * 4 + wave;
    const int n_waves = nblk * 4;
    const int ntiles = d.tiles_m * d.tiles_n;
    const int CPS = d.ksp;
    const int total_chunks = (g.K + 15) >> 4;
    const int ntasks = ntiles * g.splits;
    const __amdgpu_buffer_rsrc_t srdA = __builtin_amdgcn_make_buffer_rsrc(const_cast<float*>(g.A), 0, (int)(((int64_t)(g.M - 1) * g.lda + g.K) * 4), 0x00020000);
    const __amdgpu_buffer_rsrc_t srdB = __builtin_amdgcn_make_buffer_rsrc(const_cast<float*>(g.B), 0, (int)(((int64_t)(g.K - 1) * g.ldb + g.N) * 4), 0x00020000);
    const uint32_t ldb16 = (uint32_t)g.ldb * 64u;
    for (int task = wl; task < ntasks; task += n_waves) {
        const int split = task / ntiles, tile = task - split * ntiles;
        const int tm = tile % d.tiles_m, tn = tile / d.tiles_m;
        const int m0 = tm * (16 * TMB), n0 = tn * (64 * NL);
        const int c_lo = split * CPS;
        uint32_t offA[TMB], offB[4][NL];
#pragma unroll
        for (int a = 0; a < TMB; ++a) offA[a] = (uint32_t)(((int64_t)min(m0 + 16 * a + r, g.M - 1) * g.lda + 4 * q) * 4);
#pragma unroll
        for (int s = 0; s < 4; ++s)
#pragma unroll
            for (int l = 0; l < NL; ++l) {
                const int n = n0 + 64 * l + 4 * r;
                offB[s][l] = n < g.N ? (uint32_t)(((int64_t)(4 * q + s) * g.ldb + n) * 4) : 0x80000000u;
            }
        f32x4 acc[TMB][NL][4];
#pragma unroll
        for (int a = 0; a < TMB; ++a)
#pragma unroll
            for (int l = 0; l < NL; ++l)
#pragma unroll
                for (int e = 0; e < 4; ++e) acc[a][l][e] = f32x4{0.f, 0.f, 0.f, 0.f};
        f32x4 xa[2][TMB], xb[2][4][NL];
        {
            const uint32_t ka = (uint32_t)c_lo * 64u, kb = (uint32_t)c_lo * ldb16;
#pragma unroll
            for (int a = 0; a < TMB; ++a) xa[0][a] = __builtin_bit_cast(f32x4, __builtin_amdgcn_raw_buffer_load_b128(srdA, offA[a], ka, 0));
#pragma unroll
            for (int s = 0; s < 4; ++s)
#pragma unroll
                for (int l = 0; l < NL; ++l)
                    xb[0][s][l] = __builtin_bit_cast(f32x4, __builtin_amdgcn_raw_buffer_load_b128(srdB, offB[s][l], kb, 0));
        }
#define GD_KN_CHUNK(PAR, c)                                                                                            \
        {                                                                                                              \
            const bool more = (c) + 1 < c_lo + CPS && (c) + 1 < total_chunks;                                          \
            const uint32_t ka = more ? (uint32_t)((c) + 1) * 64u : 0x80000000u;                                        \
            const uint32_t kb = more ? (uint32_t)((c) + 1) * ldb16 : 0x80000000u;                                      \
            if ((c) * 16 + 15 >= g.K) {  \
                _Pragma("unroll") for (int e = 0; e < 4; ++e) {                                                        \
                    const bool keep = (c) * 16 + 4 * q + e < g.K;                                                      \
                    _Pragma("unroll") for (int a = 0; a < TMB; ++a) xa[PAR][a][e] = keep ? xa[PAR][a][e] : 0.f;        \
                }                                                                                                      \
            }                                                                                                          \
                    \
            _Pragma("unroll") for (int a = 0; a < TMB; ++a) asm volatile("" : "+v"(xa[PAR][a]));                       \
            _Pragma("unroll") for (int s = 0; s < 4; ++s)                                                              \
                _Pragma("unroll") for (int l = 0; l < NL; ++l) asm volatile("" : "+v"(xb[PAR][s][l]));                 \
            __builtin_amdgcn_sched_barrier(0);                                                                         \
            _Pragma("unroll") for (int s = 0; s < 4; ++s) {                                                            \
                _Pragma("unroll") for (int n = 0; n < TMB * NL * 4; ++n) {                                             \
                    const int a = n / (NL * 4), l = (n / 4) % NL, e = n % 4;                                           \
                    acc[a][l][e] = __builtin_amdgcn_mfma_f32_16x16x4f32(xa[PAR][a][s], xb[PAR][s][l][e], acc[a][l][e], 0, 0, 0); \
                    const int idx = s * (TMB * NL * 4) + n;                                                            \
                    if (idx % GD_KN_EVERY == 2 && idx / GD_KN_EVERY < TMB + 4 * NL) {                                  \
                        const int ld = idx / GD_KN_EVERY;                                                              \
                        __builtin_amdgcn_sched_barrier(0);                                                             \
                        if (ld < TMB)                                                                                  \
                            xa[(PAR) ^ 1][ld] = __builtin_bit_cast(f32x4, __builtin_amdgcn_raw_buffer_load_b128(srdA, offA[ld], ka, 0)); \
                        else                                                                                           \
                            xb[(PAR) ^ 1][(ld - TMB) / NL][(ld - TMB) % NL] = __builtin_bit_cast(                      \
                                f32x4, __builtin_amdgcn_raw_buffer_load_b128(srdB, offB[(ld - TMB) / NL][(ld - TMB) % NL], kb, 0)); \
                        __builtin_amdgcn_sched_barrier(0);                                                             \
                    }                                                                                                  \
                }                                                                                                      \
                __builtin_amdgcn_sched_barrier(0);                                                                     \
            }                                                                                                          \
        }
        for (int c = c_lo; c < c_lo + CPS && c < total_chunks; c += 2) {
            GD_KN_CHUNK(0, c);
            GD_KN_CHUNK(1, c + 1);
        }
#undef GD_KN_CHUNK
        float* __restrict__ slab = g.C + (int64_t)split * g.slab_stride;
#pragma unroll
        for (int a = 0; a < TMB; ++a)
#pragma unroll
            for (int t = 0; t < 4; ++t) {
                const int m = m0 + 16 * a + 4 * q + t;
                if (m >= g.M) continue;
#pragma unroll
                for (int l = 0; l < NL; ++l) {
                    const int n = n0 + 64 * l + 4 * r;
                    const f32x4 v = {acc[a][l][0][t], acc[a][l][1][t], acc[a][l][2][t], acc[a][l][3][t]};
                    if (n + 3 < g.ldc) {
                        *reinterpret_cast<f32x4*>(slab + (int64_t)m * g.ldc + n) = v;
                    } else {
                        for (int e = 0; e < 4; ++e)
                            if (n + e < g.N) slab[(int64_t)m * g.ldc + n + e] = v[e];
                    }
                }
            }
    }
}

template <int NB>
int dr_fat_go(const DrArgs& d, int epi, int n_cu, hipStream_t s) {
    const size_t lds = (size_t)4 * 2 * NB * 256 * sizeof(float) + 4 * 64 * sizeof(float);
    void (*kern)(const DrArgs) = epi == GD_EPI_LOSS ? dr_fat_kernel<NB, GD_EPI_LOSS> : dr_fat_kernel<NB, GD_EPI_POST>;
    static bool attr_set[2] = {false, false};
    if (!attr_set[epi == GD_EPI_LOSS] && lds > 48 * 1024) {
        hipError_t e = hipFuncSetAttribute(reinterpret_cast<const void*>(kern), hipFuncAttributeMaxDynamicSharedMemorySize, (int)lds);
        if (e != hipSuccess) {
            gdmcf_set_error("hipFuncSetAttribute(dr_fat_kernel, LDS=%zu): %s", lds, hipGetErrorString(e));
            return GDMCF_E_HIP;
        }
        attr_set[epi == GD_EPI_LOSS] = true;
    }
    hipLaunchKernelGGL(kern, dim3(n_cu), dim3(256), lds, s, d);
    return GDMCF_OK;
}

void dr_hl_go(const DrArgs& d, int n_cu, hipStream_t s) {
    static const int waves = getenv("GDMCF_HL_WAVES") ? atoi(getenv("GDMCF_HL_WAVES")) : 8;
    if (waves == 4) hipLaunchKernelGGL((dr_hl_kernel<GD_EPI_LOSS>), dim3(n_cu), dim3(256), 96 * 1024, s, d);
    else hipLaunchKernelGGL((dr_hl_kernel<GD_EPI_LOSS>), dim3(n_cu), dim3(512), 128 * 1024, s, d);
}

template <int TMB, int NB, int D, int EPI>
void dr_nt_go(const DrArgs& d, int n_cu, hipStream_t s) {
    hipLaunchKernelGGL((dr_nt_kernel<TMB, NB, D, EPI>), dim3(n_cu), dim3(512), 0, s, d);
}

int dr_cu_count_fwd();
template <int D, bool NTL>
int dr_tn_adamw_go(const DrArgs& d, hipStream_t s) {
    static bool attr_set = false;
    if (!attr_set) {
        hipError_t e = hipFuncSetAttribute(reinterpret_cast<const void*>(dr_tn_adamw_kernel<D, NTL>),
                                           hipFuncAttributeMaxDynamicSharedMemorySize, 128 * 1024);
        if (e != hipSuccess) {
            gdmcf_set_error("hipFuncSetAttribute(dr_tn_adamw_kernel, LDS=128 KB): %s", hipGetErrorString(e));
            return GDMCF_E_HIP;
        }
        attr_set = true;
    }
    hipLaunchKernelGGL((dr_tn_adamw_kernel<D, NTL>), dim3(dr_cu_count_fwd()), dim3(512), 128 * 1024, s, d);
    return GDMCF_OK;
}

template <int D, int EPI>
int dr_tn_go(const DrArgs& d, hipStream_t s) {
    if constexpr (EPI == GD_EPI_ADAMW) {
        const GdGemm& g = d.g;
        const bool lines = (g.ldc & 31) == 0 && (((uintptr_t)g.C | (uintptr_t)g.aux | (uintptr_t)g.aux2) & 127) == 0;
        static const int force = getenv("GDMCF_DR_NT_LOADS") ? atoi(getenv("GDMCF_DR_NT_LOADS")) : -1;
        return (force >= 0 ? force != 0 : lines) ? dr_tn_adamw_go<D, true>(d, s) : dr_tn_adamw_go<D, false>(d, s);
    } else {
        hipLaunchKernelGGL((dr_tn_kernel<1, 1, D, EPI>), dim3(dr_cu_count_fwd()), dim3(512), 0, s, d);
    }
    return GDMCF_OK;
}

}

static int dr_cu_count();
namespace { int dr_cu_count_fwd() { return dr_cu_count(); } }
static int dr_cu_count() {
    static int n_cu = 0;
    if (n_cu == 0) {
        int dev = 0;
        hipDeviceProp_t prop;
        n_cu = (hipGetDevice(&dev) == hipSuccess && hipGetDeviceProperties(&prop, dev) == hipSuccess) ? prop.multiProcessorCount : 256;
    }
    return n_cu;
}

int gd_dr_kn_splits(int M, int N, int K) {
    static const int on_env = getenv("GDMCF_GEMM_DR") ? atoi(getenv("GDMCF_GEMM_DR")) : 49;
    if (!(on_env & 32) || M < 16 || N < 64 || K < 4096) return 0;
    const long tiles = (long)gd_cdiv(M, 80) * gd_cdiv(N, 128);
    if ((long)gd_cdiv(M, 80) * 80 * 100 > (long)M * 112) return 0;
    if ((long)gd_cdiv(N, 128) * 128 * 100 > (long)N * 112) return 0;
    const long slots = 4L * dr_cu_count();
    if (tiles > slots) return 0;
    int splits = (int)(slots / tiles);
    const int total_chunks = gd_cdiv(K, 16);
    if (splits > total_chunks / 8) splits = total_chunks / 8;
    if (splits < 2 || splits > 64) return splits > 64 ? 64 : 0;
    return splits;
}

#include <atomic>
static std::atomic<unsigned> g_dr_seq_eager{0}, g_dr_seq_graph{0};
static int dr_ticket_slot(hipStream_t s) {
    static const int pinned = getenv("GDMCF_DR_TICKET_SLOT") ? atoi(getenv("GDMCF_DR_TICKET_SLOT")) : -1;
    if (pinned >= 0) return pinned & 31;
    hipStreamCaptureStatus st = hipStreamCaptureStatusNone;
    if (hipStreamIsCapturing(s, &st) != hipSuccess) {
        (void)hipGetLastError();
        st = hipStreamCaptureStatusNone;
    }
    if (st == hipStreamCaptureStatusActive) return 16 + (int)(g_dr_seq_graph.fetch_add(1, std::memory_order_relaxed) & 15u);
    return (int)(g_dr_seq_eager.fetch_add(1, std::memory_order_relaxed) & 15u);
}

int g_gd_dr_force = -1;
int gd_gemm_dr_launch(int layA, int layB, int epi, GdGemm& g, hipStream_t s) {
    static const int on_env = getenv("GDMCF_GEMM_DR") ? atoi(getenv("GDMCF_GEMM_DR")) : 49;
    const int on = g_gd_dr_force >= 0 ? g_gd_dr_force : on_env;
    if (!on || g.bf16) return GD_DR_NOT_TAKEN;
    if (g.accumulate || g.C16 || (g.splits > 1 && epi != GD_EPI_SLAB)) return GD_DR_NOT_TAKEN;
    static const int stagger = getenv("GDMCF_DR_STAGGER") ? atoi(getenv("GDMCF_DR_STAGGER")) : 3;
    const int64_t lim = (int64_t)1 << 32;
    DrArgs d = {};
    d.ctr = -1;
    d.stagger = stagger;
    static const int no_fused = getenv("GDMCF_DR_NO_FUSED") ? atoi(getenv("GDMCF_DR_NO_FUSED")) : 0;
    if ((on & 1) && layA == GD_LAY_MC && layB == GD_LAY_MC && (epi == GD_EPI_STORE || (epi == GD_EPI_ADAMW && !no_fused))) {
        if ((int64_t)g.K * g.lda * 4 >= lim || (int64_t)g.K * g.ldb * 4 >= lim || (int64_t)g.M * g.ldc * 4 >= lim) return GD_DR_NOT_TAKEN;
        if (g.lda < g.M || g.ldb < g.N || g.ldc < g.N) return GD_DR_NOT_TAKEN;
        const long tiles = (long)gd_cdiv(g.M, 64) * gd_cdiv(g.N, 64);
        if (tiles < 512 || g.K < 128) return GD_DR_NOT_TAKEN;
        float* const bias_db = (g.ldb > g.N) ? g.out2 : nullptr;
        const int n_user = g.N;
        if (bias_db) g.N = n_user + 1;
        d.tiles_m = gd_cdiv(g.M, 64);
        d.tiles_n = gd_cdiv(g.N, 64);
        d.m_fastest = d.tiles_m <= d.tiles_n;
        {
            static const int mf = getenv("GDMCF_DR_MF") ? atoi(getenv("GDMCF_DR_MF")) : -1;
            if (mf >= 0 && epi == GD_EPI_ADAMW) d.m_fastest = mf;
        }
        const int ks = gd_cdiv(g.K, 4);
        int best = 9, waste = 1 << 30;
        for (int dd : {9, 8, 7}) {
            const int w = gd_cdiv(ks, dd + 1) * (dd + 1) - ks;
            if (w < waste) { waste = w; best = dd; }
        }
        {
            static const int forced = getenv("GDMCF_DR_D") ? atoi(getenv("GDMCF_DR_D")) : 0;
            if (forced >= 7 && forced <= 9) { best = forced; waste = gd_cdiv(ks, best + 1) * (best + 1) - ks; }
        }
        d.ksp = ks + waste;
        g.tiles_m = d.tiles_m;
        g.tiles_n = d.tiles_n;
        d.g = g;
        d.ctr = dr_ticket_slot(s);
        d.adam_dev = epi == GD_EPI_ADAMW ? g.adam_dev : nullptr;
        d.g.out2 = bias_db;
        {
            GdProfScope prof(g.prof_tag, 2.0 * g.M * n_user * g.K, s);
#define GD_DR_GO(DD)                                                      \
    do {                                                                  \
        int rc_ = (epi == GD_EPI_STORE) ? dr_tn_go<DD, GD_EPI_STORE>(d, s) : dr_tn_go<DD, GD_EPI_ADAMW>(d, s); \
        if (rc_ != GDMCF_OK) return rc_;                                  \
    } while (0)
            if (best == 9) GD_DR_GO(9);
            else if (best == 8) GD_DR_GO(8);
            else GD_DR_GO(7);
#undef GD_DR_GO
        }
        g.N = n_user;
        t_gd_last_gemm = epi == GD_EPI_ADAMW ? 3 : 2;
        if (bias_db) g.out2 = nullptr;
        return gd_launch_status("gemm_dr");
    }
    if ((on & 32) && layA == GD_LAY_KC && layB == GD_LAY_MC && epi == GD_EPI_SLAB) {
        const int splits = gd_dr_kn_splits(g.M, g.N, g.K);
        const size_t need = (size_t)splits * g.M * g.ldc * sizeof(float);
        if (splits > 0 && g.ldc >= g.N && (g.ldc & 3) == 0 && g.ws_cap >= need && g.slab_stride >= (int64_t)g.M * g.ldc &&
            (int64_t)g.M * g.lda * 4 < ((int64_t)1 << 31) && (int64_t)g.K * g.ldb * 4 < ((int64_t)1 << 31) && g.lda >= g.K && g.ldb >= g.N &&
            (reinterpret_cast<uintptr_t>(g.B) & 15) == 0 && (g.ldb & 3) == 0 && (reinterpret_cast<uintptr_t>(g.C) & 15) == 0) {
            const int n_cu = dr_cu_count();
            const int total_chunks = gd_cdiv(g.K, 16);
            const int cps = (gd_cdiv(total_chunks, splits) + 1) & ~1;
            d.tiles_m = gd_cdiv(g.M, 80);
            d.tiles_n = gd_cdiv(g.N, 128);
            d.ksp = cps;
            g.splits = gd_cdiv(total_chunks, cps);
            g.kchunk = cps * 16;
            g.tiles_m = d.tiles_m;
            g.tiles_n = d.tiles_n;
            d.g = g;
            {
                GdProfScope prof(g.prof_tag, 2.0 * g.M * g.N * g.K, s);
                hipLaunchKernelGGL((dr_kn_kernel<2>), dim3(n_cu), dim3(256), 0, s, d);
            }
            t_gd_last_gemm = 5;
            return gd_launch_status("gemm_dr_kn");
        }
    }
    if ((on & 16) && layA == GD_LAY_KC && layB == GD_LAY_KC && (epi == GD_EPI_LOSS || epi == GD_EPI_POST)) {
        const int n_cu = dr_cu_count();
        const int tiles_m = gd_cdiv(g.M, 80);
        bool ok = (int64_t)g.M * g.lda * 4 < ((int64_t)1 << 31) && (int64_t)g.N * g.ldb * 4 < lim && g.lda >= g.K && g.ldb >= g.K &&
                  g.K >= 256 && (long)tiles_m * 80 * 100 <= (long)g.M * 112 &&
                  (n_cu & 7) == 0 && !(epi == GD_EPI_LOSS && g.rowpart == nullptr) &&
                  !(epi == GD_EPI_LOSS && g.aux_bits && g.ldbits < (g.N + 31) / 32);
        int nb = 0;
        long best = 1L << 60;
        const long slots = 4L * n_cu;
        for (int c = 12; c >= 8 && ok; --c) {
            const long t = (long)tiles_m * gd_cdiv(g.N, 16 * c);
            const long cost = ((t + slots - 1) / slots) * c;
            if (t >= slots / 2 && cost < best) { best = cost; nb = c; }
        }
        if (ok && epi == GD_EPI_POST) {
            const long t128 = (long)gd_cdiv(g.M, 80) * gd_cdiv(g.N, 128);
            const long rounds = (t128 + 2 * n_cu - 1) / (2 * n_cu);
            if (t128 * 100 >= rounds * 2 * n_cu * 90) ok = false;
        }
        if (ok && nb && !(epi == GD_EPI_LOSS && g.ld_rowpart < gd_cdiv(g.N, 16 * nb))) {
            d.tiles_m = tiles_m;
            d.tiles_n = gd_cdiv(g.N, 16 * nb);
            d.m_fastest = 1;
            d.ksp = (gd_cdiv(g.K, 16) + 1) & ~1;
            {
                static const int odd_on = getenv("GDMCF_FAT_ODD") ? atoi(getenv("GDMCF_FAT_ODD")) : 1;
                if (odd_on) d.ksp = gd_cdiv(g.K, 16);
                static const int pf = getenv("GDMCF_FAT_PF") ? atoi(getenv("GDMCF_FAT_PF")) : 10;
                d.stagger = pf;
            }
            g.tiles_m = d.tiles_m;
            g.tiles_n = d.tiles_n;
            d.g = g;
            d.ctr = 0;
            int rc = GDMCF_OK;
            {
                GdProfScope prof(g.prof_tag, 2.0 * g.M * g.N * g.K, s);
                switch (nb) {
                    case 8: rc = dr_fat_go<8>(d, epi, n_cu, s); break;
                    case 9: rc = dr_fat_go<9>(d, epi, n_cu, s); break;
                    case 10: rc = dr_fat_go<10>(d, epi, n_cu, s); break;
                    case 11: rc = dr_fat_go<11>(d, epi, n_cu, s); break;
                    default: rc = dr_fat_go<12>(d, epi, n_cu, s); break;
                }
            }
            if (rc != GDMCF_OK) return rc;
            t_gd_last_gemm = 4;
            return gd_launch_status("gemm_dr");
        }
    }
    if ((on & 8) && layA == GD_LAY_KC && layB == GD_LAY_KC && epi == GD_EPI_LOSS) {
        if ((int64_t)g.N * g.ldb * 4 >= ((int64_t)1 << 31) || (int64_t)g.K * g.M * 4 >= lim) return GD_DR_NOT_TAKEN;
        if (g.lda < g.K || g.ldb < g.K || g.K < 256 || g.M < 64) return GD_DR_NOT_TAKEN;
        if (g.ldb != g.K && (g.K & 31)) return GD_DR_NOT_TAKEN;
        if ((long)gd_cdiv(g.M, 80) * 80 * 100 > (long)g.M * 112) return GD_DR_NOT_TAKEN;
        const int tiles_m = gd_cdiv(g.M, 80), tiles_n = gd_cdiv(g.N, 64);
        if ((long)tiles_m * tiles_n < 1024) return GD_DR_NOT_TAKEN;
        if (g.aux_bits && g.ldbits < (g.N + 31) / 32) return GD_DR_NOT_TAKEN;
        const int64_t used = ((int64_t)g.M * tiles_n + 3) & ~(int64_t)3;
        if (g.rowpart == nullptr || used + (int64_t)g.K * g.M > (int64_t)g.M * g.ld_rowpart) return GD_DR_NOT_TAKEN;
        static bool attr_set = false;
        if (!attr_set) {
            hipError_t e = hipFuncSetAttribute(reinterpret_cast<const void*>(dr_hl_kernel<GD_EPI_LOSS>),
                                               hipFuncAttributeMaxDynamicSharedMemorySize, 128 * 1024);
            if (e != hipSuccess) {
                gdmcf_set_error("hipFuncSetAttribute(dr_hl_kernel, LDS=128 KB): %s", hipGetErrorString(e));
                return GDMCF_E_HIP;
            }
            attr_set = true;
        }
        float* at = g.rowpart + used;
        d.tiles_m = tiles_m;
        d.tiles_n = tiles_n;
        d.m_fastest = 1;
        d.ksp = (gd_cdiv(g.K, 32) + 1) & ~1;
        g.tiles_m = tiles_m;
        g.tiles_n = tiles_n;
        g.ld_rowpart = tiles_n;
        d.g = g;
        d.ctr = dr_ticket_slot(s);
        d.g.A = at;
        d.g.lda = g.M;
        {
            GdProfScope prof(g.prof_tag, 2.0 * g.M * g.N * g.K, s);
            hipLaunchKernelGGL(dr_transpose_kernel, dim3(gd_cdiv(g.K, 32), gd_cdiv(g.M, 32)), dim3(256), 0, s, g.A, g.lda, g.M, g.K, at, g.M);
            dr_hl_go(d, dr_cu_count(), s);
        }
        t_gd_last_gemm = 5;
        return gd_launch_status("gemm_dr");
    }
    if ((on & 2) && layA == GD_LAY_KC && layB == GD_LAY_KC && (epi == GD_EPI_LOSS || epi == GD_EPI_POST)) {
        if ((int64_t)g.M * g.lda * 4 >= lim || (int64_t)g.N * g.ldb * 4 >= lim) return GD_DR_NOT_TAKEN;
        if (g.lda < g.K || g.ldb < g.K || g.K < 256) return GD_DR_NOT_TAKEN;
        const int tmb = ((long)gd_cdiv(g.M, 80) * 80 * 100 <= (long)gd_cdiv(g.M, 64) * 64 * 103) ? 5 : 4;
        static const int nb_env = getenv("GDMCF_DR_NB") ? atoi(getenv("GDMCF_DR_NB")) : 0;
        const int n_cu = dr_cu_count();
        int nb = 4;
        {
            const long t4 = (long)gd_cdiv(g.M, 16 * tmb) * gd_cdiv(g.N, 64);
            const long per = (t4 + 4 * n_cu - 1) / (4 * n_cu);
            if (t4 * 100 < per * 4 * n_cu * 92 && per < 6) nb = 2;
        }
        if (nb_env == 2 || nb_env == 4) nb = nb_env;
        d.tiles_m = gd_cdiv(g.M, 16 * tmb);
        d.tiles_n = gd_cdiv(g.N, 16 * nb);
        if ((long)d.tiles_m * d.tiles_n < 1024) return GD_DR_NOT_TAKEN;
        if (epi == GD_EPI_LOSS && (g.ld_rowpart < d.tiles_n || g.rowpart == nullptr)) return GD_DR_NOT_TAKEN;
        if (epi == GD_EPI_LOSS && g.aux_bits && g.ldbits < (g.N + 31) / 32) return GD_DR_NOT_TAKEN;
        d.m_fastest = 1;
        const int nc = gd_cdiv(g.K, 16);
        const int ring = nb == 4 ? 2 : 3;
        d.ksp = gd_cdiv(nc, ring) * ring;
        g.tiles_m = d.tiles_m;
        g.tiles_n = d.tiles_n;
        d.g = g;
        d.ctr = dr_ticket_slot(s);
        {
            GdProfScope prof(g.prof_tag, 2.0 * g.M * g.N * g.K, s);
#define GD_DR_NT(T, NBV, DV)                                                            \
    do {                                                                                \
        if (epi == GD_EPI_LOSS) dr_nt_go<T, NBV, DV, GD_EPI_LOSS>(d, n_cu, s);          \
        else dr_nt_go<T, NBV, DV, GD_EPI_POST>(d, n_cu, s);                             \
    } while (0)
            if (tmb == 5 && nb == 4) GD_DR_NT(5, 4, 1);
            else if (tmb == 5) GD_DR_NT(5, 2, 2);
            else if (nb == 4) GD_DR_NT(4, 4, 1);
            else GD_DR_NT(4, 2, 2);
#undef GD_DR_NT
        }
        t_gd_last_gemm = 6;
        return gd_launch_status("gemm_dr");
    }
    return GD_DR_NOT_TAKEN;
}
```

### gdmcf_amd/csrc/linear.hip

```cpp
#include <stdlib.h>

#include "common.h"

int gd_splitk_reduce(const float* slabs, int64_t slab_stride, int splits, int64_t ld_slab, int M, int N, int mode,
                     const float* bias, const float* rowscale, const float* aact, int64_t ldact, int act, float* out,
                     int64_t ldo, hipStream_t s);
int gd_colsum(const float* dZ, int64_t ld, const float* rs, int M, int N, float* db, hipStream_t s);
int gd_rowpart_reduce(const float* rowpart, int ld, int M, int nt, float* rowsum, hipStream_t s);

namespace {

static const int TARGET_WGS = getenv("GDMCF_TARGET_WGS") ? atoi(getenv("GDMCF_TARGET_WGS")) : 760;

thread_local int t_gemm_prec = GDMCF_GEMM_F32;

int pick_class(int M, int N, bool fused, int prec) {
    if (prec == GDMCF_GEMM_BF16 && M > 128) {
        const long pad = (long)gd_cdiv(M, 208) * 208;
        const long tiles = (pad / 208) * gd_cdiv(N, 256);
        const long rounds = (tiles + 255) / 256;
        if (pad * 10 <= (long)M * 11 && pad / 208 <= 2 && (!fused || tiles * 100 >= rounds * 256 * 85)) return 3;
    }
    if (prec == GDMCF_GEMM_F32X3 && M > 128 && N >= 128) {
        const long pad = (long)gd_cdiv(M, 208) * 208;
        if (pad * 10 <= (long)M * 11) return 4;
    }
    return gd_pick_shape_class(M, N);
}

int pick_class_dw(int M, int N, int prec, bool fused_adamw = false) {
    static const int forced = getenv("GDMCF_BF16_DW_CLASS") ? atoi(getenv("GDMCF_BF16_DW_CLASS")) : -1;
    if (prec == GDMCF_GEMM_BF16 && forced >= 0) return forced;
    if (prec == GDMCF_GEMM_BF16 && fused_adamw && M >= 160 && N >= 256) return 0;
    if (prec == GDMCF_GEMM_BF16 && M >= 416 && N >= 512) {
        const long tiles = (long)gd_cdiv(M, 208) * gd_cdiv(N, 256);
        const long rounds = (tiles + 255) / 256;
        if (tiles * 100 >= rounds * 256 * 85) return 3;
    }
    return gd_pick_shape_class(M, N);
}

void attach_result_shadow(GdGemm& g) {
    GdShadow c;
    if (g.bf16 == 1 && gd_shadow_lookup(g.C, &c) && c.rows == g.M && c.cols >= g.N) {
        g.C16 = c.p16;
        g.ldc16 = c.ld16;
    }
}

void attach_shadows(GdGemm& g, int layA, int layB) {
    if (g.bf16 != 1) return;
    GdShadow a, b;
    if (!gd_shadow_lookup(g.A, &a) || !gd_shadow_lookup(g.B, &b)) return;
    const bool okA = layA == GD_LAY_KC ? (a.rows == g.M && a.cols == g.K) : (a.rows == g.K && a.cols == g.M);
    const bool okB = layB == GD_LAY_KC ? (b.rows == g.N && b.cols == g.K) : (b.rows == g.K && b.cols == g.N);
    if (!okA || !okB) return;
    g.A16 = a.p16; g.lda16 = a.ld16;
    g.B16 = b.p16; g.ldb16 = b.ld16;
}

int pick_splits(int M, int N, int K, int cls, int prec) {
    const int bk = prec == GDMCF_GEMM_BF16 ? 64 : 32;
    const int tiles = gd_cdiv(M, gd_gemm_tile_m(cls)) * gd_cdiv(N, gd_gemm_tile_n(cls));
    int s = (cls >= 3 ? 256 : TARGET_WGS) / tiles;
    const int max_by_k = K / (8 * bk);
    if (s > max_by_k) s = max_by_k;
    if (s < 1) s = 1;
    if (s > 64) s = 64;
    return s;
}

inline int64_t round4(int64_t x) { return (x + 3) & ~(int64_t)3; }

float* bias_col_request(int a_scale_col, int64_t lda, const float* rowscale, int K, float* db) {
    static const int on = getenv("GDMCF_BIAS_COL") ? atoi(getenv("GDMCF_BIAS_COL")) : 1;
    if (!on || !a_scale_col || db == nullptr || t_gemm_prec != GDMCF_GEMM_F32 || lda <= K) return nullptr;
    return db;
}

}

extern "C" {

int gdmcf_gemm_precision(int mode) {
    const int prev = t_gemm_prec;
    if (mode == GDMCF_GEMM_F32 || mode == GDMCF_GEMM_BF16 || mode == GDMCF_GEMM_F32X3) t_gemm_prec = mode;
    return prev;
}

size_t gdmcf_linear_ws_bytes(int M, int N, int K) {
    if (M <= 0 || N <= 0 || K <= 0) return 0;
    size_t need = 0;
    for (int prec = GDMCF_GEMM_F32; prec <= GDMCF_GEMM_F32X3; ++prec) {
        const int cf = pick_class(M, N, false, prec), cb = pick_class(M, K, false, prec);
        size_t f = (size_t)pick_splits(M, N, K, cf, prec) * M * round4(N);
        if (prec == GDMCF_GEMM_F32) {
            const size_t fk = (size_t)gd_dr_kn_splits(M, N, K) * M * round4(N);
            f = f > fk ? f : fk;
        }
        size_t b = (size_t)pick_splits(M, K, N, cb, prec) * M * round4(K);
        if (prec == GDMCF_GEMM_F32) {
            const size_t bk = (size_t)gd_dr_kn_splits(M, K, N) * M * round4(K);
            b = b > bk ? b : bk;
        }
        need = need > f ? need : f;
        need = need > b ? need : b;
    }
    return need * sizeof(float) + 256;
}

int gdmcf_loss_tiles(int N) { return gd_cdiv(N, 16); }

int gdmcf_linear_fwd_f32(const float* A, int64_t lda, const float* W, int64_t ldw, const float* bias, int act, int M,
                         int N, int K, float* C, int64_t ldc, void* ws, size_t ws_bytes, void* stream) {
    GD_CHECK_SHAPE(M > 0 && N > 0 && K > 0 && lda >= K && ldw >= K && ldc >= N, "linear_fwd: bad shape");
    GD_CHECK_ARG(act == 0 || act == 1, "linear_fwd: bad activation");
    hipStream_t s = (hipStream_t)stream;
    const int cls = pick_class(M, N, false, t_gemm_prec);
    const int splits = pick_splits(M, N, K, cls, t_gemm_prec);
    GdGemm g = {};
    g.bf16 = t_gemm_prec;
    g.A = A; g.lda = lda; g.B = W; g.ldb = ldw; g.M = M; g.N = N; g.K = K;
    g.m_fastest = gd_cdiv(M, gd_gemm_tile_m(cls)) <= gd_cdiv(N, gd_gemm_tile_n(cls));
    g.bias = bias; g.act = act; g.prof_tag = 1;
    if (splits == 1) {
        g.splits = 1; g.C = C; g.ldc = ldc;
        attach_result_shadow(g);
        attach_shadows(g, GD_LAY_KC, GD_LAY_KC);
        return gd_gemm_launch(GD_LAY_KC, GD_LAY_KC, GD_EPI_BIAS_ACT, cls, g, s);
    }
    const int64_t lds_ = round4(N);
    const size_t need = (size_t)splits * M * lds_ * sizeof(float);
    if (ws == nullptr || ws_bytes < need) {
        gdmcf_set_error("linear_fwd: workspace %zu < %zu bytes", ws_bytes, need);
        return GDMCF_E_WORKSPACE;
    }
    g.splits = splits; g.C = (float*)ws; g.ldc = lds_; g.slab_stride = (int64_t)M * lds_;
    attach_shadows(g, GD_LAY_KC, GD_LAY_KC);
    int rc = gd_gemm_launch(GD_LAY_KC, GD_LAY_KC, GD_EPI_SLAB, cls, g, s);
    if (rc) return rc;
    const int real_splits = gd_cdiv(K, g.kchunk);
    return gd_splitk_reduce((const float*)ws, g.slab_stride, real_splits, lds_, M, N, 0, bias, nullptr, nullptr, 0,
                            act, C, ldc, s);
}

int gdmcf_linear_fwd_wt_f32(const float* A, int64_t lda, const float* Wt, int64_t ldwt, const float* bias, int act, int M, int N,
                            int K, float* C, int64_t ldc, void* ws, size_t ws_bytes, void* stream) {
    GD_CHECK_SHAPE(M > 0 && N > 0 && K > 0 && lda >= K && ldwt >= N && ldc >= N, "linear_fwd_wt: bad shape");
    GD_CHECK_ARG(act == 0 || act == 1, "linear_fwd_wt: bad activation");
    if (t_gemm_prec != GDMCF_GEMM_F32) {
        gdmcf_set_error("linear_fwd_wt: float32 GEMM mode only (the bf16 / f32x3 modes keep the weight in its own orientation)");
        return GDMCF_E_UNSUPPORTED;
    }
    hipStream_t s = (hipStream_t)stream;
    const int cls = pick_class(M, N, false, t_gemm_prec);
    const int splits = pick_splits(M, N, K, cls, t_gemm_prec);
    const int64_t lds_ = round4(N);
    const size_t need = (size_t)splits * M * lds_ * sizeof(float);
    if (ws == nullptr || ws_bytes < need) {
        gdmcf_set_error("linear_fwd_wt: workspace %zu < %zu bytes", ws_bytes, need);
        return GDMCF_E_WORKSPACE;
    }
    GdGemm g = {};
    g.A = A; g.lda = lda; g.B = Wt; g.ldb = ldwt; g.M = M; g.N = N; g.K = K;
    g.m_fastest = gd_cdiv(M, gd_gemm_tile_m(cls)) <= gd_cdiv(N, gd_gemm_tile_n(cls));
    g.splits = splits; g.C = (float*)ws; g.ldc = lds_; g.slab_stride = (int64_t)M * lds_; g.prof_tag = 1;
    g.ws_cap = ws_bytes;
    int rc = gd_gemm_launch(GD_LAY_KC, GD_LAY_MC, GD_EPI_SLAB, cls, g, s);
    if (rc) return rc;
    const int real_splits = gd_cdiv(K, g.kchunk);
    return gd_splitk_reduce((const float*)ws, g.slab_stride, real_splits, lds_, M, N, 0, bias, nullptr, nullptr, 0, act, C, ldc, s);
}

int gdmcf_linear_loss_fwd_f32(const float* A, int64_t lda, const float* W, int64_t ldw, const float* bias,
                              const float* target, int64_t ldt, const float* alpha, int M, int N, int K, float* out,
                              int64_t ldo, float* diff, int64_t ldd, float* rowpart, float* rowsum, void* stream) {
    GD_CHECK_SHAPE(M > 0 && N > 0 && K > 0 && lda >= K && ldw >= K && ldt >= N && ldd >= N, "linear_loss_fwd: bad shape");
    GD_CHECK_SHAPE(out == nullptr || ldo >= N, "linear_loss_fwd: ldo < N");
    hipStream_t s = (hipStream_t)stream;
    const int cls = pick_class(M, N, true, t_gemm_prec);
    GdGemm g = {};
    g.bf16 = t_gemm_prec;
    g.A = A; g.lda = lda; g.B = W; g.ldb = ldw; g.M = M; g.N = N; g.K = K; g.splits = 1;
    g.m_fastest = gd_cdiv(M, gd_gemm_tile_m(cls)) <= gd_cdiv(N, gd_gemm_tile_n(cls));
    g.bias = bias; g.aux = target; g.ldaux = ldt; g.r0 = alpha; g.out2 = out; g.ldout2 = ldo;
    g.prof_tag = 2;
    g.C = diff; g.ldc = ldd; g.rowpart = rowpart; g.ld_rowpart = gdmcf_loss_tiles(N);
    attach_result_shadow(g);
    attach_shadows(g, GD_LAY_KC, GD_LAY_KC);
    int rc = gd_gemm_launch(GD_LAY_KC, GD_LAY_KC, GD_EPI_LOSS, cls, g, s);
    if (rc) return rc;
    return gd_rowpart_reduce(rowpart, g.ld_rowpart, M, g.tiles_n, rowsum, s);
}

int gdmcf_linear_loss_fwd_bits_f32(const float* A, int64_t lda, const float* W, int64_t ldw, const float* bias,
                                   const uint32_t* target_bits, int64_t ldbits, const float* alpha, int M, int N, int K,
                                   float* out, int64_t ldo, float* diff, int64_t ldd, float* rowpart, float* rowsum,
                                   void* stream) {
    GD_CHECK_SHAPE(M > 0 && N > 0 && K > 0 && lda >= K && ldw >= K && ldd >= N, "linear_loss_fwd_bits: bad shape");
    GD_CHECK_SHAPE(out == nullptr || ldo >= N, "linear_loss_fwd_bits: ldo < N");
    GD_CHECK_ARG(target_bits && ldbits >= (N + 31) / 32, "linear_loss_fwd_bits: target bitmap missing / ldbits < ceil(N/32)");
    hipStream_t s = (hipStream_t)stream;
    const int cls = pick_class(M, N, true, t_gemm_prec);
    GdGemm g = {};
    g.bf16 = t_gemm_prec;
    g.A = A; g.lda = lda; g.B = W; g.ldb = ldw; g.M = M; g.N = N; g.K = K; g.splits = 1;
    g.m_fastest = gd_cdiv(M, gd_gemm_tile_m(cls)) <= gd_cdiv(N, gd_gemm_tile_n(cls));
    g.bias = bias; g.aux = nullptr; g.ldaux = 0; g.aux_bits = target_bits; g.ldbits = ldbits; g.r0 = alpha; g.out2 = out;
    g.ldout2 = ldo; g.prof_tag = 2;
    g.C = diff; g.ldc = ldd; g.rowpart = rowpart; g.ld_rowpart = gdmcf_loss_tiles(N);
    attach_result_shadow(g);
    attach_shadows(g, GD_LAY_KC, GD_LAY_KC);
    int rc = gd_gemm_launch(GD_LAY_KC, GD_LAY_KC, GD_EPI_LOSS, cls, g, s);
    if (rc) return rc;
    return gd_rowpart_reduce(rowpart, g.ld_rowpart, M, g.tiles_n, rowsum, s);
}

int gdmcf_linear_posterior_fwd_f32(const float* A, int64_t lda, const float* W, int64_t ldw, const float* bias,
                                   const float* x_t, int64_t ldxt, const float* c1, const float* c2, const float* r1,
                                   const float* r2, const float* sigma, const float* z, int64_t ldz, int M, int N,
                                   int K, float* x_next, int64_t ldxn, float* pred_out, int64_t ldp, void* stream) {
    GD_CHECK_SHAPE(M > 0 && N > 0 && K > 0 && lda >= K && ldw >= K && ldxt >= N && ldxn >= N, "linear_posterior_fwd: bad shape");
    GD_CHECK_ARG(c1 && c2, "linear_posterior_fwd: c1/c2 missing");
    GD_CHECK_ARG((r1 == nullptr) == (r2 == nullptr), "linear_posterior_fwd: r1/r2 must both be set or both NULL");
    GD_CHECK_ARG(z == nullptr || (sigma != nullptr && ldz >= N), "linear_posterior_fwd: sigma missing");
    hipStream_t s = (hipStream_t)stream;
    const int cls = pick_class(M, N, true, t_gemm_prec);
    GdGemm g = {};
    g.bf16 = t_gemm_prec;
    g.A = A; g.lda = lda; g.B = W; g.ldb = ldw; g.M = M; g.N = N; g.K = K; g.splits = 1;
    g.m_fastest = gd_cdiv(M, gd_gemm_tile_m(cls)) <= gd_cdiv(N, gd_gemm_tile_n(cls));
    g.bias = bias; g.aux = x_t; g.ldaux = ldxt; g.aux2 = z; g.ldaux2 = ldz;
    g.r0 = c1; g.r1 = c2; g.r2 = r1; g.r3 = r2; g.r4 = sigma;
    g.out2 = pred_out; g.ldout2 = ldp; g.C = x_next; g.ldc = ldxn; g.prof_tag = 3;
    attach_result_shadow(g);
    attach_shadows(g, GD_LAY_KC, GD_LAY_KC);
    return gd_gemm_launch(GD_LAY_KC, GD_LAY_KC, GD_EPI_POST, cls, g, s);
}

int gdmcf_linear_bwd_input_f32(const float* dZ, int64_t lddz, const float* W, int64_t ldw, const float* rowscale,
                               const float* Aact, int64_t ldact, int act, int M, int N, int K, float* dA,
                               int64_t ldda, void* ws, size_t ws_bytes, void* stream) {
    GD_CHECK_SHAPE(M > 0 && N > 0 && K > 0 && lddz >= N && ldw >= K && ldda >= K, "linear_bwd_input: bad shape");
    GD_CHECK_ARG(act == 0 || (act == 1 && Aact && ldact >= K), "linear_bwd_input: activation output missing");
    hipStream_t s = (hipStream_t)stream;
    const int cls = pick_class(M, K, false, t_gemm_prec);
    const int splits = pick_splits(M, K, N, cls, t_gemm_prec);
    const int64_t lds_ = round4(K);
    const size_t need = (size_t)splits * M * lds_ * sizeof(float);
    if (ws == nullptr || ws_bytes < need) {
        gdmcf_set_error("linear_bwd_input: workspace %zu < %zu bytes", ws_bytes, need);
        return GDMCF_E_WORKSPACE;
    }
    GdGemm g = {};
    g.bf16 = t_gemm_prec;
    g.A = dZ; g.lda = lddz; g.B = W; g.ldb = ldw; g.M = M; g.N = K; g.K = N;
    g.m_fastest = gd_cdiv(M, gd_gemm_tile_m(cls)) <= gd_cdiv(K, gd_gemm_tile_n(cls));
    g.splits = splits; g.C = (float*)ws; g.ldc = lds_; g.slab_stride = (int64_t)M * lds_; g.prof_tag = 4;
    g.ws_cap = ws_bytes;
    attach_shadows(g, GD_LAY_KC, GD_LAY_MC);
    int rc = gd_gemm_launch(GD_LAY_KC, GD_LAY_MC, GD_EPI_SLAB, cls, g, s);
    if (rc) return rc;
    const int real_splits = gd_cdiv(N, g.kchunk);
    return gd_splitk_reduce((const float*)ws, g.slab_stride, real_splits, lds_, M, K, 1, nullptr, rowscale, Aact,
                            ldact, act, dA, ldda, s);
}

int gdmcf_linear_bwd_weight_f32(const float* dZ, int64_t lddz, const float* A, int64_t lda, const float* rowscale,
                                int a_scale_col, int M, int N, int K, float* dW, int64_t lddw, float* db, int accumulate,
                                void* stream) {
    GD_CHECK_SHAPE(M > 0 && N > 0 && K > 0 && lddz >= N && lda >= K && lddw >= K, "linear_bwd_weight: bad shape");
    hipStream_t s = (hipStream_t)stream;
    const int cls = pick_class_dw(N, K, t_gemm_prec);
    GdGemm g = {};
    g.bf16 = t_gemm_prec;
    g.A = dZ; g.lda = lddz; g.B = A; g.ldb = lda; g.M = N; g.N = K; g.K = M; g.splits = 1;
    g.m_fastest = gd_cdiv(N, gd_gemm_tile_m(cls)) <= gd_cdiv(K, gd_gemm_tile_n(cls));
    g.C = dW; g.ldc = lddw; g.accumulate = accumulate; g.prof_tag = 5;
    attach_shadows(g, GD_LAY_MC, GD_LAY_MC);
    g.out2 = bias_col_request(a_scale_col, lda, rowscale, K, db);
    const bool asked = g.out2 != nullptr;
    int rc = gd_gemm_launch(GD_LAY_MC, GD_LAY_MC, GD_EPI_STORE, cls, g, s);
    if (rc) return rc;
    if (asked && g.out2 == nullptr) return GDMCF_OK;
    if (db) return gd_colsum(dZ, lddz, rowscale, M, N, db, s);
    return GDMCF_OK;
}

int gdmcf_linear_bwd_weight_adamw_f32(const float* dZ, int64_t lddz, const float* A, int64_t lda, const float* rowscale,
                                      int a_scale_col, int M, int N, int K, float* W, int64_t ldw, float* exp_avg, float* exp_avg_sq,
                                      float* db, float lr, float beta1, float beta2, float eps, float weight_decay,
                                      int step, float grad_scale, void* stream) {
    GD_CHECK_SHAPE(M > 0 && N > 0 && K > 0 && lddz >= N && lda >= K && ldw >= K, "linear_bwd_weight_adamw: bad shape");
    GD_CHECK_ARG(W && exp_avg && exp_avg_sq && step >= 1, "linear_bwd_weight_adamw: optimizer state missing");
    hipStream_t s = (hipStream_t)stream;
    const int cls = pick_class_dw(N, K, t_gemm_prec, true);
    GdGemm g = {};
    g.bf16 = t_gemm_prec;
    g.A = dZ; g.lda = lddz; g.B = A; g.ldb = lda; g.M = N; g.N = K; g.K = M; g.splits = 1;
    g.m_fastest = gd_cdiv(N, gd_gemm_tile_m(cls)) <= gd_cdiv(K, gd_gemm_tile_n(cls));
    g.C = W; g.ldc = ldw; g.aux = exp_avg; g.aux2 = exp_avg_sq; g.prof_tag = 5;
    g.adam = gd_adam_hyper(lr, beta1, beta2, eps, weight_decay, step, grad_scale);
    g.adam_dev = t_gd_step_state ? &t_gd_step_state->hyper : nullptr;
    attach_result_shadow(g);
    attach_shadows(g, GD_LAY_MC, GD_LAY_MC);
    g.out2 = bias_col_request(a_scale_col, lda, rowscale, K, db);
    const bool asked = g.out2 != nullptr;
    int rc = gd_gemm_launch(GD_LAY_MC, GD_LAY_MC, GD_EPI_ADAMW, cls, g, s);
    if (rc) return rc;
    if (asked && g.out2 == nullptr) return GDMCF_OK;
    if (db) return gd_colsum(dZ, lddz, rowscale, M, N, db, s);
    return GDMCF_OK;
}

}
```

### gdmcf_amd/engine.py

```python

import functools

import torch

from . import _lib


def _ceil64(n):
    return (n + 63) // 64 * 64


class _Bufs:
    pass


_GEMM_MODES = {"f32": 0, "bf16": 1, "f32x3": 2}


def _with_precision(fn):
    @functools.wraps(fn)
    def wrapped(self, *a, **kw):
        prev = self.lib.gdmcf_gemm_precision(_GEMM_MODES[self.gemm_dtype])
        try:
            return fn(self, *a, **kw)
        finally:
            self.lib.gdmcf_gemm_precision(prev)
    return wrapped


class DenoiserEngine:
    supports_grad_sink = True

    def __init__(self, model):
        self.model = model
        self.lib = _lib.load()
        self.E = int(model.time_emb_dim)
        self.I = int(model.in_dims[0])
        self.version = 0
        self.seed = int(torch.initial_seed()) & 0xFFFFFFFFFFFFFFFF
        self.offset = 0
        self._bufs = {}
        self._wshadow = {}
        self._saved = None
        self.grad_sink = None
        self.fused_opt = None
        self.input_grad_first = False
        self.weight_waiters = {}
        self.static_grads = False
        self._grad_bufs = {}
        import os as _os
        self._gemm_side = _os.environ.get("GDMCF_GEMM_SIDE", "0") == "1"
        self._side2 = None
        self._side2_used = False
        self._wt = {}
        self._wt_on = _os.environ.get("GDMCF_FWD_WT", "1") == "1"

    def _grad_like(self, p):
        if not self.static_grads:
            return torch.empty_like(p)
        g = self._grad_bufs.get(id(p))
        if g is None or g.shape != p.shape or g.device != p.device:
            g = self._grad_bufs[id(p)] = torch.empty_like(p)
        return g

    def _use_weight(self, w):
        fn = self.weight_waiters.pop(id(w), None) if self.weight_waiters else None
        if fn is not None:
            fn()
            rec = self._wshadow.get(id(w))
            if rec is not None and rec[1] != w._version:
                rec[0].sync()
                rec[1] = w._version

    def flush_weight_waiters(self):
        while self.weight_waiters:
            self.weight_waiters.popitem()[1]()

    @property
    def gemm_dtype(self):
        return getattr(self.model, "gemm_dtype", "f32")

    def manual_seed(self, seed):
        self.seed = int(seed) & 0xFFFFFFFFFFFFFFFF
        self.offset = 0

    def _shadows_on(self, bufs, layers):
        if self.gemm_dtype != "bf16":
            if bufs.shadows is not None:
                for sh in bufs.shadows:
                    sh.close()
                bufs.shadows = None
                bufs.sh_xin2 = None
            for sh, _ in self._wshadow.values():
                sh.close()
            self._wshadow = {}
            return
        if bufs.shadows is None:
            I, E = self.I, self.E
            mk = lambda t, cols: _lib.Bf16Shadow(t[:, :cols], sync=False)
            sh = [mk(bufs.xin, I + E), mk(bufs.diff, I)]
            for (w, _, _), a, d in zip(layers[:-1], bufs.acts, bufs.dzs):
                sh += [mk(a, w.shape[0]), mk(d, w.shape[0])]
            sh.append(mk(bufs.hs, layers[-1][0].shape[1]))
            bufs.shadows = sh
            bufs.sh_xin = sh[0]
        live = {id(w) for w, _, _ in layers}
        for key in [k for k in self._wshadow if k not in live]:
            self._wshadow.pop(key)[0].close()
        for w, _, _ in layers:
            rec = self._wshadow.get(id(w))
            if rec is None or rec[0].ptr != w.data_ptr():
                self._use_weight(w)
                if rec is not None:
                    rec[0].close()
                self._wshadow[id(w)] = [_lib.Bf16Shadow(w.detach()), w._version]
            elif id(w) in self.weight_waiters:
                continue
            elif rec[1] != w._version:
                rec[0].sync()
                rec[1] = w._version

    def _layers(self):
        layers = self.model.layer_list()
        for w, b, _ in layers:
            _lib.require_gpu(w, "DNN parameters")
            if not (w.stride(1) == 1 and w.stride(0) >= w.shape[1] and b.is_contiguous() and w.dtype == torch.float32):
                raise RuntimeError("gdmcf_amd: DNN parameters must be float32 with unit column stride")
        return layers

    def buffers(self, B, device):
        key = (B, str(device))
        b = self._bufs.get(key)
        if b is not None:
            return b
        lib, I, E = self.lib, self.I, self.E
        layers = self.model.layer_list()
        f32 = dict(dtype=torch.float32, device=device)
        b = _Bufs()
        b.ldk = _ceil64(I + E)
        b.xin = torch.zeros(B, b.ldk, **f32)
        b.xin2 = None
        b.temb = torch.zeros(B, max(E, 1), **f32)
        b.rownorm = torch.zeros(B, **f32)
        b.acts = [torch.zeros(B, _ceil64(w.shape[0]), **f32) for (w, _, _) in layers[:-1]]
        b.dzs = [torch.zeros(B, _ceil64(w.shape[0]), **f32) for (w, _, _) in layers[:-1]]
        b.hs = torch.zeros(B, _ceil64(layers[-1][0].shape[1]), **f32)
        b.ldi = _ceil64(I)
        b.diff = torch.zeros(B, b.ldi, **f32)
        b.xt = None
        b.shadows = None
        b.rowpart = torch.zeros(B, lib.gdmcf_loss_tiles(layers[-1][0].shape[0]), **f32)
        b.rowsum = torch.zeros(B, **f32)
        b.gradcoef = torch.zeros(B, **f32)
        b.rowdiv_mse = torch.full((B,), float(I), **f32)
        b.lu = torch.zeros(B, dtype=torch.float64, device=device)
        b.demb = torch.zeros((B + layers[0][0].shape[0]) * max(E, 1), **f32)
        ws = 0
        for (w, _, _) in layers:
            ws = max(ws, lib.gdmcf_linear_ws_bytes(B, w.shape[0], w.shape[1]))
        b.ws_bytes = int(ws)
        b.ws = torch.empty(max(ws, 256), dtype=torch.uint8, device=device)
        self._bufs[key] = b
        return b

    def _prep(self, bufs, x, ts, ca, cb, noise, drop_mask, training, xt_out=None, xin=None):
        m, lib = self.model, self.lib
        B = x.shape[0]
        if x.dtype != torch.float32 or x.stride(-1) != 1:
            x = x.float().contiguous()
        xin = bufs.xin if xin is None else xin
        noise_mode = 0
        if ca is not None:
            noise_mode = 1 if noise is not None else 2
            if noise is not None and (noise.dtype != torch.float32 or noise.stride(-1) != 1):
                noise = noise.float().contiguous()
        p = float(m.drop.p)
        drop_mode = 0
        keep = None
        if drop_mask is not None:
            drop_mode = 1
            keep = drop_mask if drop_mask.dtype == torch.uint8 else (drop_mask != 0).to(torch.uint8)
            keep = keep.contiguous()
        elif training and p > 0.0:
            drop_mode = 2
        self.offset += 1
        rc = lib.gdmcf_dnn_prep_input_f32(
            x.data_ptr(), x.stride(0), _lib.ptr(ts), _lib.ptr(ca), _lib.ptr(cb), noise_mode, _lib.ptr(noise),
            noise.stride(0) if noise is not None else 0, drop_mode, _lib.ptr(keep),
            keep.stride(0) if keep is not None else 0, p, self.seed, self.offset, int(bool(m.norm)),
            m.emb_layer.weight.data_ptr(), m.emb_layer.bias.data_ptr(), self.E, B, self.I, xin.data_ptr(),
            xin.stride(0), _lib.ptr(xt_out), xt_out.stride(0) if xt_out is not None else 0, bufs.temb.data_ptr(),
            bufs.rownorm.data_ptr(), _lib.stream_ptr())
        _lib.check(rc)
        if xin is bufs.xin:
            bufs.xin_ones = True
        return x, noise, keep

    def _prep_csr(self, bufs, batch, ts, ca, cb, noise, drop_mask, training):
        m, lib = self.model, self.lib
        B, I = batch.shape
        if getattr(bufs, "x0bits", None) is None:
            bufs.x0bits = torch.zeros(B, (I + 31) // 32, dtype=torch.int32, device=batch.device)
        noise_mode = 0
        if ca is not None:
            noise_mode = 1 if noise is not None else 2
            if noise is not None and (noise.dtype != torch.float32 or noise.stride(-1) != 1):
                noise = noise.float().contiguous()
        p = float(m.drop.p)
        drop_mode, keep = 0, None
        if drop_mask is not None:
            drop_mode = 1
            keep = (drop_mask if drop_mask.dtype == torch.uint8 else (drop_mask != 0).to(torch.uint8)).contiguous()
        elif training and p > 0.0:
            drop_mode = 2
        self.offset += 1
        c = batch.csr
        _lib.check(lib.gdmcf_dnn_prep_input_csr_f32(
            c.indptr.data_ptr(), c.indices.data_ptr(), batch.row_ids.data_ptr(), _lib.ptr(ts), _lib.ptr(ca), _lib.ptr(cb),
            noise_mode, _lib.ptr(noise), noise.stride(0) if noise is not None else 0, drop_mode, _lib.ptr(keep),
            keep.stride(0) if keep is not None else 0, p, self.seed, self.offset, m.emb_layer.weight.data_ptr(),
            m.emb_layer.bias.data_ptr(), self.E, B, I, bufs.xin.data_ptr(), bufs.xin.stride(0), bufs.temb.data_ptr(),
            bufs.x0bits.data_ptr(), bufs.x0bits.stride(0), _lib.stream_ptr()))
        bufs.xin_ones = True
        return batch, noise, keep

    def _eps_target(self, bufs, spec, ts, x0, noise):
        B, dev = ts.shape[0], ts.device
        if x0.dtype != torch.float32 or x0.stride(-1) != 1:
            x0 = x0.float().contiguous()
        target = noise if spec.get("noise_owned", False) else torch.empty(B, self.I, dtype=torch.float32, device=dev)
        alpha = torch.empty(B, dtype=torch.float32, device=dev)
        rowdiv = torch.empty(B, dtype=torch.float32, device=dev)
        _lib.check(self.lib.gdmcf_eps_target_f32(
            noise.data_ptr(), noise.stride(0), bufs.xt.data_ptr(), bufs.xt.stride(0), x0.data_ptr(), x0.stride(0), ts.data_ptr(),
            spec["r1_0"].data_ptr(), spec["r2_0"].data_ptr(), int(bool(spec.get("t0_likelihood", True))), B, self.I,
            target.data_ptr(), target.stride(0), alpha.data_ptr(), rowdiv.data_ptr(), _lib.stream_ptr()))
        return target, alpha, rowdiv

    def _transposed(self, w):
        rec = self._wt.get(id(w))
        if rec is None or rec[0] is not w or rec[1] != w._version or rec[2].device != w.device:
            n, k = w.shape
            buf = torch.zeros(k, (n + 31) // 32 * 32, dtype=torch.float32, device=w.device)
            buf[:, :n].copy_(w.detach().t())
            rec = self._wt[id(w)] = (w, w._version, buf)
        return rec[2]

    def _hidden_forward(self, bufs, layers, B, xin=None, frozen=False):
        lib, st = self.lib, _lib.stream_ptr()
        A, lda = (bufs.xin if xin is None else xin), bufs.ldk
        for li, (w, bias, act) in enumerate(layers[:-1]):
            N, K = w.shape
            out = bufs.acts[li]
            self._use_weight(w)
            if frozen and self._wt_on and self.gemm_dtype == "f32" and K >= 4096 and w.numel() >= (1 << 20):
                wt = self._transposed(w)
                _lib.check(lib.gdmcf_linear_fwd_wt_f32(A.data_ptr(), lda, wt.data_ptr(), wt.stride(0), bias.data_ptr(), act, B, N, K,
                                                       out.data_ptr(), out.stride(0), bufs.ws.data_ptr(), bufs.ws_bytes, st))
            else:
                _lib.check(lib.gdmcf_linear_fwd_f32(A.data_ptr(), lda, w.data_ptr(), w.stride(0), bias.data_ptr(), act, B,
                                                    N, K, out.data_ptr(), out.stride(0), bufs.ws.data_ptr(),
                                                    bufs.ws_bytes, st))
            A, lda = out, out.stride(0)
        return A, lda

    @_with_precision
    def train_forward(self, spec):
        x0, ts = spec["x_start"], spec["ts"]
        csr = spec.get("csr")
        B, dev = (csr.shape[0], csr.device) if csr is not None else (x0.shape[0], x0.device)
        layers = self._layers()
        bufs = self.buffers(B, dev)
        self._shadows_on(bufs, layers)
        lib, st = self.lib, _lib.stream_ptr()
        self.version += 1
        eps_mode = spec["eps_mode"]
        xt_out = None
        if eps_mode:
            if bufs.xt is None:
                bufs.xt = torch.zeros(B, bufs.ldi, dtype=torch.float32, device=dev)
            xt_out = bufs.xt
        if csr is not None:
            keepalive = self._prep_csr(bufs, csr, ts, spec["ca"], spec["cb"], spec["noise"], spec["drop_mask"], self.model.training)
        else:
            keepalive = self._prep(bufs, x0, ts, spec["ca"], spec["cb"], spec["noise"], spec["drop_mask"],
                                   self.model.training, xt_out=xt_out)
        x0c = keepalive[0]
        alpha = None
        if eps_mode:
            target, alpha, rowdiv = self._eps_target(bufs, spec, ts, x0c, keepalive[1])
        else:
            target = x0c
            rowdiv = bufs.rowdiv_mse
        A, lda = self._hidden_forward(bufs, layers, B)
        w, bias, _ = layers[-1]
        N, K = w.shape
        self._use_weight(w)
        if csr is not None:
            _lib.check(lib.gdmcf_linear_loss_fwd_bits_f32(A.data_ptr(), lda, w.data_ptr(), w.stride(0), bias.data_ptr(),
                                                          bufs.x0bits.data_ptr(), bufs.x0bits.stride(0), None, B, N, K, None,
                                                          0, bufs.diff.data_ptr(), bufs.ldi, bufs.rowpart.data_ptr(),
                                                          bufs.rowsum.data_ptr(), st))
        else:
            _lib.check(lib.gdmcf_linear_loss_fwd_f32(A.data_ptr(), lda, w.data_ptr(), w.stride(0), bias.data_ptr(),
                                                     target.data_ptr(), target.stride(0), _lib.ptr(alpha), B, N, K, None,
                                                     0, bufs.diff.data_ptr(), bufs.ldi, bufs.rowpart.data_ptr(),
                                                     bufs.rowsum.data_ptr(), st))
        loss = torch.empty(B, dtype=torch.float64, device=dev)
        pt = spec["pt"]
        self.last_loss_mean = torch.empty((), dtype=torch.float64, device=dev)
        if getattr(bufs, "rowscale_mean", None) is None:
            bufs.rowscale_mean = torch.zeros(B, dtype=torch.float32, device=dev)
        _lib.check(lib.gdmcf_row_loss_finish_mean_f64(bufs.rowsum.data_ptr(), rowdiv.data_ptr(), _lib.ptr(alpha),
                                                      ts.data_ptr(), spec["weight_t"].data_ptr(), pt.data_ptr(), B,
                                                      spec["T"], spec["H"], spec["Lt_history"].data_ptr(),
                                                      spec["Lt_count"].data_ptr(), int(spec["update_history"]),
                                                      bufs.lu.data_ptr(), loss.data_ptr(), bufs.gradcoef.data_ptr(),
                                                      self.last_loss_mean.data_ptr(), bufs.rowscale_mean.data_ptr(), st))
        self._saved = dict(kind="train", B=B, bufs=bufs, layers=layers, keepalive=(keepalive, target, alpha, rowdiv, pt))
        return loss

    @_with_precision
    def train_backward(self, gloss):
        sv = self._saved
        if sv is None or sv.get("kind") != "train":
            raise RuntimeError("gdmcf_amd: train_backward without a preceding training_losses")
        bufs = sv["bufs"]
        if isinstance(gloss, float) and gloss == 1.0 / sv["B"] and getattr(bufs, "rowscale_mean", None) is not None:
            rowscale = bufs.rowscale_mean
        elif isinstance(gloss, float):
            rowscale = bufs.gradcoef * gloss
        else:
            rowscale = (gloss.to(torch.float32) * bufs.gradcoef).contiguous()
        return self._backward(sv, bufs.diff, bufs.ldi, rowscale)

    @_with_precision
    def forward_plain(self, x, timesteps, training, drop_mask=None):
        self.flush_weight_waiters()
        B, dev = x.shape[0], x.device
        layers = self._layers()
        bufs = self.buffers(B, dev)
        self._shadows_on(bufs, layers)
        lib, st = self.lib, _lib.stream_ptr()
        self.version += 1
        ts = timesteps.to(device=dev, dtype=torch.int64).contiguous()
        keepalive = self._prep(bufs, x, ts, None, None, None, drop_mask, training)
        A, lda = self._hidden_forward(bufs, layers, B)
        w, bias, act = layers[-1]
        N, K = w.shape
        out = torch.empty(B, N, dtype=torch.float32, device=dev)
        _lib.check(lib.gdmcf_linear_fwd_f32(A.data_ptr(), lda, w.data_ptr(), w.stride(0), bias.data_ptr(), act, B, N,
                                            K, out.data_ptr(), out.stride(0), bufs.ws.data_ptr(), bufs.ws_bytes, st))
        self._saved = dict(kind="plain", B=B, bufs=bufs, layers=layers, keepalive=(keepalive, ts))
        return out

    @_with_precision
    def backward_plain(self, gout):
        sv = self._saved
        g = gout.to(torch.float32)
        if g.stride(-1) != 1:
            g = g.contiguous()
        return self._backward(sv, g, g.stride(0), None)

    def _backward(self, sv, dz_last, ld_last, rowscale):
        lib, st = self.lib, _lib.stream_ptr()
        bufs, layers, B = sv["bufs"], sv["layers"], sv["B"]
        m = self.model
        L = len(layers)
        grads_w = [None] * L
        grads_b = [None] * L
        dWe = dbe = None
        fused = self.fused_opt if self.grad_sink is None else None
        dz, lddz, rs = dz_last, ld_last, rowscale

        def input_grad(li, w, A_prev, lda_prev, N, K):
            nonlocal dWe, dbe
            if li > 0:
                dprev = bufs.dzs[li - 1]
                act_prev = layers[li - 1][2]
                _lib.check(lib.gdmcf_linear_bwd_input_f32(dz.data_ptr(), lddz, w.data_ptr(), w.stride(0), _lib.ptr(rs),
                                                          A_prev.data_ptr(), lda_prev, act_prev, B, N, K,
                                                          dprev.data_ptr(), dprev.stride(0), bufs.ws.data_ptr(),
                                                          bufs.ws_bytes, st))
                return dprev, dprev.stride(0), None
            dWe = self._grad_like(m.emb_layer.weight)
            dbe = self._grad_like(m.emb_layer.bias)
            _lib.check(lib.gdmcf_emb_bwd_f32(dz.data_ptr(), lddz, w.data_ptr(), w.stride(0), self.I, self.E,
                                             bufs.temb.data_ptr(), B, w.shape[0], bufs.demb.data_ptr(), dWe.data_ptr(),
                                             dbe.data_ptr(), st))
            return None, 0, None

        def weight_grad(li, w, bias, A_prev, lda_prev, N, K):
            db = self._grad_like(bias)
            A_use, lda_use = A_prev, lda_prev
            scol = int(rs is None and li == 0 and getattr(bufs, "xin_ones", False) and lda_use > K)
            if rs is not None:
                _lib.check(lib.gdmcf_rowscale_f32(A_prev.data_ptr(), lda_prev, rs.data_ptr(), B, K, bufs.hs.data_ptr(),
                                                  bufs.hs.stride(0), st))
                A_use, lda_use = bufs.hs, bufs.hs.stride(0)
                scol = int(lda_use > K)
            fs = fused.fused_state(w) if fused is not None else None
            if fs is not None:
                if fs["exp_avg"].stride() != w.stride() or fs["exp_avg_sq"].stride() != w.stride():
                    raise RuntimeError("gdmcf_amd: the moments of a fused weight must share its leading dimension")
                _lib.check(lib.gdmcf_linear_bwd_weight_adamw_f32(
                    dz.data_ptr(), lddz, A_use.data_ptr(), lda_use, _lib.ptr(rs), scol, B, N, K, w.data_ptr(), w.stride(0),
                    fs["exp_avg"].data_ptr(), fs["exp_avg_sq"].data_ptr(), db.data_ptr(), fs["lr"], fs["beta1"],
                    fs["beta2"], fs["eps"], fs["weight_decay"], fs["step"], fs["grad_scale"], st))
                if not (self.gemm_dtype == "bf16" and _lib.shadow_info(w.data_ptr()) is not None):
                    torch.autograd.graph.increment_version(w)
                dW = None
            else:
                dW = self._grad_like(w)
                if self._gemm_side and self.grad_sink is None and li == L - 1 and L > 1:
                    if self._side2 is None:
                        self._side2 = torch.cuda.Stream()
                    self._side2.wait_stream(torch.cuda.current_stream())
                    with torch.cuda.stream(self._side2):
                        _lib.check(lib.gdmcf_linear_bwd_weight_f32(dz.data_ptr(), lddz, A_use.data_ptr(), lda_use, _lib.ptr(rs),
                                                                   scol, B, N, K, dW.data_ptr(), dW.stride(0), db.data_ptr(), 0,
                                                                   _lib.stream_ptr()))
                    self._side2_used = True
                else:
                    _lib.check(lib.gdmcf_linear_bwd_weight_f32(dz.data_ptr(), lddz, A_use.data_ptr(), lda_use, _lib.ptr(rs),
                                                               scol, B, N, K, dW.data_ptr(), dW.stride(0), db.data_ptr(), 0, st))
            grads_w[li], grads_b[li] = dW, db
            if self.grad_sink is not None:
                self.grad_sink(w, dW)
                self.grad_sink(bias, db)
                grads_w[li] = grads_b[li] = None

        for li in range(L - 1, -1, -1):
            w, bias, _ = layers[li]
            N, K = w.shape
            if li > 0:
                A_prev, lda_prev = bufs.acts[li - 1], bufs.acts[li - 1].stride(0)
            else:
                A_prev, lda_prev = bufs.xin, bufs.ldk
            if fused is not None or self.input_grad_first:
                nxt = input_grad(li, w, A_prev, lda_prev, N, K)
                weight_grad(li, w, bias, A_prev, lda_prev, N, K)
            else:
                weight_grad(li, w, bias, A_prev, lda_prev, N, K)
                nxt = input_grad(li, w, A_prev, lda_prev, N, K)
            dz, lddz, rs = nxt
        if self._side2_used:
            torch.cuda.current_stream().wait_stream(self._side2)
            self._side2_used = False
        if self.grad_sink is not None:
            self.grad_sink(m.emb_layer.weight, dWe)
            self.grad_sink(m.emb_layer.bias, dbe)
            dWe = dbe = None
        out = [dWe, dbe]
        for li in range(L):
            out += [grads_w[li], grads_b[li]]
        return out

    @_with_precision
    def p_sample_loop(self, x_start, steps, T, tabs32, eps_mode, sampling_noise, noise0=None, step_noise=None,
                      capture=None, draw_noise=None):
        m, lib = self.model, self.lib
        if draw_noise is None:
            def draw_noise(like):
                self.offset += 1
                return _lib.philox_randn(like.shape, like.device, self.seed, self.offset, 7)
        self.flush_weight_waiters()
        B, dev, I = x_start.shape[0], x_start.device, self.I
        layers = self._layers()
        bufs = self.buffers(B, dev)
        self._shadows_on(bufs, layers)
        st = _lib.stream_ptr()
        self.version += 1
        if bufs.xin2 is None:
            bufs.xin2 = torch.zeros_like(bufs.xin)
        if self.gemm_dtype == "bf16" and getattr(bufs, "sh_xin2", None) is None:
            bufs.sh_xin2 = _lib.Bf16Shadow(bufs.xin2[:, : I + self.E], sync=False)
            bufs.shadows.append(bufs.sh_xin2)
        norm = bool(m.norm)
        keep = []
        t_vec = torch.full((B,), max(steps - 1, 0), dtype=torch.int64, device=dev)
        ca = cb = None
        if steps > 0:
            ca, cb = tabs32["sqrt_ab"], tabs32["sqrt_1mab"]
        w, bias, _ = layers[-1]
        N, K = w.shape
        out = None

        key = (id(tabs32), T, B)
        if getattr(bufs, "step_tabs_key", None) != key:
            bufs.step_tabs = {k: tabs32[k][:T, None].expand(T, B).contiguous() for k in ("c1", "c2", "r1", "r2", "sigma")
                              if k in tabs32}
            bufs.step_ts = torch.arange(T, dtype=torch.int64, device=dev)[:, None].expand(T, B).contiguous()
            bufs.step_tabs_key = key
        stabs, step_ts = bufs.step_tabs, bufs.step_ts

        def posterior(i, n, A, lda, xt, xn):
            c1, c2 = stabs["c1"][i], stabs["c2"][i]
            r1 = r2 = sg = z = None
            if eps_mode:
                r1, r2 = stabs["r1"][i], stabs["r2"][i]
            if sampling_noise and i != 0:
                sg = stabs["sigma"][i]
                z = step_noise[n] if step_noise is not None else draw_noise(xt[:, :I])
                z = z.contiguous()
            pred = torch.empty(B, I, dtype=torch.float32, device=dev) if capture is not None else None
            _lib.check(lib.gdmcf_linear_posterior_fwd_f32(
                A.data_ptr(), lda, w.data_ptr(), w.stride(0), bias.data_ptr(), xt.data_ptr(), xt.stride(0),
                c1.data_ptr(), c2.data_ptr(), _lib.ptr(r1), _lib.ptr(r2), _lib.ptr(sg), _lib.ptr(z),
                z.stride(0) if z is not None else 0, B, N, K, xn.data_ptr(), xn.stride(0), _lib.ptr(pred),
                pred.stride(0) if pred is not None else 0, st))
            keep.append((c1, c2, r1, r2, sg, z))
            if capture is not None:
                capture.setdefault("pred_xstart", []).append(pred)
                capture.setdefault("mean", []).append(xn[:, :I].clone())

        if not norm:
            cur, nxt = bufs.xin, bufs.xin2
            keep.append(self._prep(bufs, x_start, t_vec, ca, cb, noise0, None, False, xin=cur))
            bufs.xin_ones = False
            for n, i in enumerate(range(T - 1, -1, -1)):
                ts = step_ts[i]
                _lib.check(lib.gdmcf_dnn_emb_cols_f32(ts.data_ptr(), m.emb_layer.weight.data_ptr(),
                                                      m.emb_layer.bias.data_ptr(), self.E, B, I, cur.data_ptr(),
                                                      cur.stride(0), bufs.temb.data_ptr(), st))
                keep.append(ts)
                A, lda = self._hidden_forward(bufs, layers, B, xin=cur, frozen=True)
                out = torch.empty(B, I, dtype=torch.float32, device=dev) if i == 0 else None
                posterior(i, n, A, lda, cur, out if out is not None else nxt)
                cur, nxt = nxt, cur
        else:
            if bufs.xt is None:
                bufs.xt = torch.zeros(B, bufs.ldi, dtype=torch.float32, device=dev)
            xt = bufs.xt
            keep.append(self._prep(bufs, x_start, t_vec, ca, cb, noise0, None, False, xt_out=xt, xin=bufs.xin2))
            for n, i in enumerate(range(T - 1, -1, -1)):
                ts = step_ts[i]
                keep.append(self._prep(bufs, xt[:, :I], ts, None, None, None, None, False, xin=bufs.xin))
                A, lda = self._hidden_forward(bufs, layers, B, xin=bufs.xin, frozen=True)
                out = torch.empty(B, I, dtype=torch.float32, device=dev) if i == 0 else None
                xn = out if out is not None else (bufs.diff if xt is bufs.xt else bufs.xt)
                posterior(i, n, A, lda, xt, xn)
                xt = xn
        self._saved = None
        del keep
        return out
```

### include/gdmcf_hip.h

```cpp
#ifndef GDMCF_HIP_H
#define GDMCF_HIP_H
#include <stddef.h>
#include <stdint.h>

#ifdef __cplusplus
extern "C" {
#endif

#define GDMCF_OK 0
#define GDMCF_E_SHAPE (-1)
#define GDMCF_E_ARG (-2)
#define GDMCF_E_UNSUPPORTED (-3)
#define GDMCF_E_HIP (-4)
#define GDMCF_E_WORKSPACE (-5)

int gdmcf_version(void);
const char* gdmcf_last_error(void);
int gdmcf_device_info(int* n_cu, int* wave_size, char* arch_host, int arch_len);
int gdmcf_debug_last_gemm(void);

int gdmcf_prof_enable(int on);
int gdmcf_prof_collect(int cap, int* tags_host, float* ms_host, double* work_host);

#define GDMCF_N_TABLES 13
int gdmcf_schedule_build(int kind, double noise_scale, double noise_min, double noise_max, int T,
                         int beta_fixed, double* out_tables_host);

int gdmcf_densify_rows_f32(const int64_t* indptr, const int32_t* indices, const float* values,
                           const int64_t* row_ids, int B, int I, float* out, int64_t ldo, void* stream);

int gdmcf_dnn_prep_input_f32(const float* x, int64_t ldx, const int64_t* ts, const float* ca,
                             const float* cb, int noise_mode, const float* noise, int64_t ldn,
                             int drop_mode, const uint8_t* keep, int64_t ldkeep, float drop_p,
                             uint64_t seed, uint64_t offset, int normalize, const float* emb_w,
                             const float* emb_b, int E, int B, int I, float* xin, int64_t ldxin,
                             float* xt_out, int64_t ldxt, float* temb_out, float* rownorm_ws,
                             void* stream);
int gdmcf_dnn_prep_input_csr_f32(const int64_t* indptr, const int32_t* indices, const int64_t* rows, const int64_t* ts,
                                 const float* ca, const float* cb, int noise_mode, const float* noise, int64_t ldn,
                                 int drop_mode, const uint8_t* keep, int64_t ldkeep, float drop_p, uint64_t seed,
                                 uint64_t offset, const float* emb_w, const float* emb_b, int E, int B, int I, float* xin,
                                 int64_t ldxin, float* temb_out, uint32_t* bits_out, int64_t ldbits, void* stream);

int gdmcf_onehot_noise_f32(const float* x0, int64_t ldx, const int64_t* ts, int B, int I, float discrete,
                           const uint8_t* sampled, int64_t lds, uint64_t seed, uint64_t offset,
                           float* xU, int64_t ldu, uint8_t* sampled_out, int64_t ldso, void* stream);

int gdmcf_randn_f32(float* out, int64_t ld, int rows, int cols, int stream_id, uint64_t seed, uint64_t offset, void* stream);

int gdmcf_eps_target_f32(const float* noise, int64_t ldn, const float* xt, int64_t ldxt, const float* x0, int64_t ldx0,
                         const int64_t* ts, const float* r1, const float* r2, int t0_likelihood, int B, int I, float* target,
                         int64_t ldt, float* alpha, float* rowdiv, void* stream);

int gdmcf_graph_guided_step_u8(uint8_t* graph, int64_t ldg, const int64_t* ts, int B, int I, float discrete,
                               const uint8_t* sampled_in, int64_t lds, const uint8_t* pick_in, const float* degree_prob,
                               int user_guided, uint64_t seed, uint64_t offset, uint8_t* sampled_out, int64_t ldso,
                               uint8_t* pick_out, void* stream);

int gdmcf_dnn_emb_cols_f32(const int64_t* ts, const float* emb_w, const float* emb_b, int E, int B,
                           int I, float* xin, int64_t ldxin, float* temb_out, void* stream);

enum { GDMCF_GEMM_F32 = 0, GDMCF_GEMM_BF16 = 1, GDMCF_GEMM_F32X3 = 2 };
int gdmcf_gemm_precision(int mode);
int gdmcf_bf16_shadow_set(const float* f32, void* bf16, int64_t rows, int64_t cols, int64_t ld_bf16);
int gdmcf_bf16_shadow_clear(const float* f32 );
void* gdmcf_bf16_shadow_get(const float* f32);
int gdmcf_bf16_shadow_info(const float* f32, void** bf16, int64_t* rows, int64_t* cols, int64_t* ld_bf16);
int gdmcf_bf16_shadow_sync(const float* f32, int64_t ld, void* stream);
size_t gdmcf_linear_ws_bytes(int M, int N, int K);
int gdmcf_linear_fwd_f32(const float* A, int64_t lda, const float* W, int64_t ldw,
                         const float* bias, int act, int M, int N, int K, float* C, int64_t ldc,
                         void* ws, size_t ws_bytes, void* stream);
int gdmcf_linear_fwd_wt_f32(const float* A, int64_t lda, const float* Wt, int64_t ldwt,
                            const float* bias, int act, int M, int N, int K, float* C, int64_t ldc,
                            void* ws, size_t ws_bytes, void* stream);
int gdmcf_loss_tiles(int N);
int gdmcf_linear_loss_fwd_f32(const float* A, int64_t lda, const float* W, int64_t ldw,
                              const float* bias, const float* target, int64_t ldt,
                              const float* alpha, int M, int N, int K, float* out, int64_t ldo,
                              float* diff, int64_t ldd, float* rowpart, float* rowsum,
                              void* stream);
int gdmcf_linear_loss_fwd_bits_f32(const float* A, int64_t lda, const float* W, int64_t ldw, const float* bias,
                                   const uint32_t* target_bits, int64_t ldbits, const float* alpha, int M, int N, int K,
                                   float* out, int64_t ldo, float* diff, int64_t ldd, float* rowpart, float* rowsum,
                                   void* stream);
int gdmcf_linear_posterior_fwd_f32(const float* A, int64_t lda, const float* W, int64_t ldw,
                                   const float* bias, const float* x_t, int64_t ldxt,
                                   const float* c1, const float* c2, const float* r1,
                                   const float* r2, const float* sigma, const float* z,
                                   int64_t ldz, int M, int N, int K, float* x_next,
                                   int64_t ldxn, float* pred_out, int64_t ldp, void* stream);
int gdmcf_linear_bwd_input_f32(const float* dZ, int64_t lddz, const float* W, int64_t ldw,
                               const float* rowscale, const float* Aact, int64_t ldact, int act,
                               int M, int N, int K, float* dA, int64_t ldda, void* ws,
                               size_t ws_bytes, void* stream);
int gdmcf_linear_bwd_weight_f32(const float* dZ, int64_t lddz, const float* A, int64_t lda,
                                const float* rowscale, int a_scale_col, int M, int N, int K,
                                float* dW, int64_t lddw, float* db, int accumulate, void* stream);
int gdmcf_linear_bwd_weight_adamw_f32(const float* dZ, int64_t lddz, const float* A, int64_t lda,
                                      const float* rowscale, int a_scale_col, int M, int N, int K, float* W,
                                      int64_t ldw, float* exp_avg, float* exp_avg_sq, float* db, float lr,
                                      float beta1, float beta2, float eps, float weight_decay, int step,
                                      float grad_scale, void* stream);
int gdmcf_rowscale_f32(const float* A, int64_t lda, const float* rowscale, int M, int K, float* out,
                       int64_t ldo, void* stream);
int gdmcf_row_norms_f32(const float* X, int64_t ld, int rows, int cols, float* norm, float* inv_norm,
                        void* stream);
int gdmcf_normalize_rows_bwd_f32(const float* dY, int64_t lddy, const float* Y, int64_t ldy,
                                 const float* inv_norm, int rows, int cols, float* dX, int64_t lddx,
                                 void* stream);
int gdmcf_tanh_bwd_f32(const float* dA, int64_t ldd, const float* A, int64_t lda, const float* extra,
                       int64_t lde, const float* scale, int M, int N, float* out, int64_t ldo,
                       void* stream);
int gdmcf_gather_rows_f32(const float* src, int64_t lds, const int64_t* index, int n, int cols, float* dst,
                          int64_t ldd, void* stream);
int gdmcf_scatter_add_rows_f32(const float* src, int64_t lds, const int64_t* index, int n, int cols,
                               float* dst, int64_t ldd, void* stream);
int gdmcf_normalize_rows_bwd_adamw_f32(const float* dY, int64_t lddy, const float* Y, int64_t ldy,
                                       const float* inv_norm, int rows, int cols, float* X, int64_t ldx,
                                       float* exp_avg, float* exp_avg_sq, float lr, float beta1, float beta2,
                                       float eps, float weight_decay, int step, float grad_scale, void* stream);
int gdmcf_scatter_rows_adamw_f32(const float* src, int64_t lds, const int64_t* index, int n, int rows, int cols,
                                 float* W, int64_t ldw, float* exp_avg, float* exp_avg_sq, float lr, float beta1,
                                 float beta2, float eps, float weight_decay, int step, float grad_scale,
                                 void* stream);
int gdmcf_emb_bwd_f32(const float* dZ1, int64_t lddz, const float* W1, int64_t ldw, int I, int E,
                      const float* temb, int M, int N, float* demb_ws, float* dWe, float* dbe,
                      void* stream);

int gdmcf_row_loss_finish_f64(const float* rowsum, const float* rowdiv, const float* alpha,
                              const int64_t* ts, const double* weight_t, const double* pt, int B,
                              int T, int H, double* Lt_history, int64_t* Lt_count,
                              int update_history, double* loss_unscaled, double* loss,
                              float* gradcoef, void* stream);
int gdmcf_row_loss_finish_mean_f64(const float* rowsum, const float* rowdiv, const float* alpha, const int64_t* ts,
                                   const double* weight_t, const double* pt, int B, int T, int H, double* Lt_history,
                                   int64_t* Lt_count, int update_history, double* loss_unscaled, double* loss,
                                   float* gradcoef, double* loss_mean, float* rowscale_mean, void* stream);
int gdmcf_lt_history_update(const int64_t* ts, const double* loss_unscaled, int B, int T, int H,
                            double* Lt_history, int64_t* Lt_count, void* stream);

int gdmcf_dp_pack_f64(const float* const* grads, const int64_t* counts, int n, const int64_t* ts,
                      const double* loss_unscaled, int B, int rank, int world, double* flat,
                      void* stream);
int gdmcf_dp_unpack_f64(const double* flat, float* const* grads, const int64_t* counts, int n, int B,
                        int world, int64_t* ts_all, double* loss_unscaled_all, void* stream);

int gdmcf_sample_timesteps(const double* Lt_history, const int64_t* Lt_count, int T, int H, int B,
                           double uniform_prob, uint64_t seed, uint64_t offset, int64_t* ts,
                           double* pt, double* p_out, void* stream);

int gdmcf_adamw_f32(const int64_t* table, int n_tensors, int total_blocks, float lr, float beta1,
                    float beta2, float eps, float weight_decay, int step, float grad_scale,
                    void* stream);
int gdmcf_adamw_bf16s_f32(const int64_t* table, const int64_t* shadow_table, int n_tensors, int total_blocks, float lr,
                          float beta1, float beta2, float eps, float weight_decay, int step, float grad_scale,
                          void* stream);

int gdmcf_topk_masked_f32(const float* pred, int64_t ldp, int B, int I, const int64_t* mask_indptr,
                          const int32_t* mask_indices, int k, int64_t* idx_out, float* val_out,
                          void* stream);

int gdmcf_topn_metrics_f64(const int64_t* pred_idx, int64_t ldp, int U, const int64_t* gt_indptr, const int32_t* gt_indices,
                           const int* topN_host, int n_topn, double* out, void* stream);

int gdmcf_spmm_csr_f32(const int64_t* vbeg, const int64_t* vend, const int32_t* vrow, const int32_t* vslot,
                       int n_virtual, int n_short, const int32_t* lrow, const int32_t* lptr, int n_long, const int32_t* col,
                       const float* val, int n_rows, const float* X, int64_t ldx, int d, float* Y,
                       int64_t ldy, float* partial_ws, const float* const* addends_host, int n_add,
                       int64_t ld_add, float scale, double alg_bytes, void* stream);
int gdmcf_spmm_bundled_f32(const int32_t* wdesc, int n_waves, const int64_t* lbeg, const int32_t* llen, const int32_t* lrow,
                           const int32_t* lslot, int n_pieces, const int64_t* sbeg, const int32_t* slen, const int32_t* srow,
                           const int32_t* smax, int n_bundles, const int32_t* crow, const int32_t* cptr, int n_cut,
                           const int32_t* col, const float* val, int64_t nnz, int n_rows, int n_x_rows, const float* X,
                           int64_t ldx, int d, float* Y, int64_t ldy, float* partial_ws, const float* const* addends_host, int n_add, int64_t ld_add,
                           float scale, double alg_bytes, void* stream);
int gdmcf_spmm_stream_f32(const int32_t* wdesc, int n_waves, const int32_t* cw, int64_t n_entries, const int32_t* ud, int n_units,
                          const int32_t* crow, const int32_t* cptr, int n_cut, int n_rows, int n_x_rows, const float* X,
                          int64_t ldx, int d, float* Y, int64_t ldy, float* partial_ws, const float* const* addends_host,
                          int n_add, int64_t ld_add, float scale, double alg_bytes, void* stream);
int gdmcf_debug_spmm_stamps(int n_waves, long long* host_out);
int gdmcf_graph_state_bytes(void);
int gdmcf_adam_hyper_bytes(void);
int gdmcf_graph_state_init(void* state_host, uint64_t prep_offset, uint64_t ts_offset, int64_t adam_step, int64_t table_first,
                           int64_t table_len, const void* hyper_table_dev);
int gdmcf_adam_hyper_fill(void* out_host, int n, float lr, float beta1, float beta2, float eps, float weight_decay,
                          int64_t first_step, float grad_scale);
int gdmcf_graph_state_bind(const void* state_dev);
int gdmcf_graph_state_tick(void* state_dev, void* stream);
int gdmcf_scale_f32(const float* acc, int64_t n, float scale, float* out, void* stream);

#ifdef __cplusplus
}
#endif
#endif
```

Before: 306,200 users/s.

## Batch all fused weight-grad AdamW GEMMs into one multi-product persistent launch

Weight-gradient plus AdamW updates for every layer are now queued during backward and issued as one persistent kernel that walks a combined tile space over up to four products. Tiles carry a product index in their high bits, and the kernel rebuilds buffer descriptors and Adam hyperparameters per product. The goal is fewer launches and no tail idle time between small per-layer GEMMs, so CUs stay busy across layers. In exchange the weight updates move to the end of backward, the kernel carries more scalar state and per-tile indirection, and an unsupported shape falls back to the per-layer path.

Measured after the change: 317,100 users/s (median of 6 runs). 3.6% higher.

```diff
diff --git a/gdmcf_amd/_lib.py b/gdmcf_amd/_lib.py
--- a/gdmcf_amd/_lib.py
+++ b/gdmcf_amd/_lib.py
@@ -47,6 +47,7 @@
     "gdmcf_linear_bwd_weight_f32": (c_int, [P, c_int64, P, c_int64, P, c_int, c_int, c_int, c_int, P, c_int64, P, c_int, P]),
     "gdmcf_linear_bwd_weight_adamw_f32": (c_int, [P, c_int64, P, c_int64, P, c_int, c_int, c_int, c_int, P, c_int64, P, P, P, c_float,
                                                   c_float, c_float, c_float, c_float, c_int, c_float, P]),
+    "gdmcf_linear_bwd_weight_adamw_multi_f32": (c_int, [P, c_int, P]),
     "gdmcf_rowscale_f32": (c_int, [P, c_int64, P, c_int, c_int, P, c_int64, P]),
     "gdmcf_emb_bwd_f32": (c_int, [P, c_int64, P, c_int64, c_int, c_int, P, c_int, c_int, P, P, P, P]),
     "gdmcf_row_loss_finish_f64": (c_int, [P, P, P, P, P, P, c_int, c_int, c_int, P, P, c_int, P, P, P, P]),
@@ -94,6 +95,13 @@
 }
 EXPORTED_SYMBOLS = tuple(_SIGNATURES)
 
+
+class GdDwAdamw(ctypes.Structure):
+    _fields_ = [("dZ", c_void_p), ("lddz", c_int64), ("A", c_void_p), ("lda", c_int64), ("rowscale", c_void_p),
+                ("a_scale_col", c_int), ("M", c_int), ("N", c_int), ("K", c_int), ("W", c_void_p), ("ldw", c_int64),
+                ("exp_avg", c_void_p), ("exp_avg_sq", c_void_p), ("db", c_void_p), ("lr", c_float), ("beta1", c_float),
+                ("beta2", c_float), ("eps", c_float), ("weight_decay", c_float), ("step", c_int), ("grad_scale", c_float)]
+
 _lib = None
 
 
diff --git a/gdmcf_amd/csrc/common.h b/gdmcf_amd/csrc/common.h
--- a/gdmcf_amd/csrc/common.h
+++ b/gdmcf_amd/csrc/common.h
@@ -151,6 +151,7 @@
 int gd_gemm_small_launch(int layA, int layB, int epi, GdGemm& g, hipStream_t s);
 enum { GD_DR_NOT_TAKEN = 1 };
 int gd_gemm_dr_launch(int layA, int layB, int epi, GdGemm& g, hipStream_t s);
+int gd_gemm_dr_adamw_multi(GdGemm* gs, int n, hipStream_t s);
 int gd_gemm_tile_m(int shape_class);
 int gd_gemm_tile_n(int shape_class);
 int gd_gemm_bk(int layA, int layB);
diff --git a/gdmcf_amd/csrc/gemm_dr.hip b/gdmcf_amd/csrc/gemm_dr.hip
--- a/gdmcf_amd/csrc/gemm_dr.hip
+++ b/gdmcf_amd/csrc/gemm_dr.hip
@@ -48,6 +48,28 @@
     int ksp;
     int ctr;
     const GdAdamHyper* adam_dev;
+    int stagger;
+};
+
+struct DrAdamProd {
+    const float* A;
+    const float* B;
+    float* W;
+    float* ea;
+    float* ea2;
+    float* bias;
+    int lda, ldb, ldc;
+    int M, N, K;
+    int tiles_m, tiles_n, m_fastest;
+    const GdAdamHyper* adam_dev;
+    GdAdamHyper adam;
+};
+constexpr int DR_MULTI_MAX = 4;
+struct DrMultiArgs {
+    DrAdamProd p[DR_MULTI_MAX];
+    int n;
+    int ksp;
+    int ctr;
     int stagger;
 };
 
@@ -281,8 +303,11 @@
 #endif
 }
 
+constexpr int DR_VT_SHIFT = 24;
+constexpr int DR_VT_PARK = 0x7fffffff;
+
 template <int D, bool NTL>
-__global__ __launch_bounds__(512, 2) void dr_tn_adamw_kernel(const DrArgs d) {
+__global__ __launch_bounds__(512, 2) void dr_tn_adamw_kernel(const DrMultiArgs d) {
     constexpr int LPS = 2;
     constexpr int R = D + 1;
     constexpr int UA = 1, UB = 1 + R / 2;
@@ -291,22 +316,38 @@
     static_assert(UB < R && UB > UA, "two distinct steps of a round");
     static_assert(LPS * R + XS <= 63, "vmcnt is a 6-bit counter");
     constexpr uint32_t PARK = 0xFFFFFF00u;
-    const GdGemm& g = d.g;
     const int lane = threadIdx.x & 63;
     const int wave = __builtin_amdgcn_readfirstlane(threadIdx.x >> 6);
     const int r = lane & 15, q = lane >> 4;
     extern __shared__ __attribute__((aligned(16))) float dr_lds[];
     f32x4* const stash = reinterpret_cast<f32x4*>(dr_lds + wave * 4096) + lane;
-    GdAdamHyper hy = g.adam;
-    if (d.adam_dev) hy = *d.adam_dev;
     const int n_waves = gridDim.x * 8;
-    const int minor = d.m_fastest ? d.tiles_m : d.tiles_n;
-    const int panels = d.m_fastest ? d.tiles_n : d.tiles_m;
     int xcc;
     asm volatile("s_getreg_b32 %0, hwreg(HW_REG_XCC_ID)" : "=s"(xcc));
     int qx = xcc & 7, visited = 0;
-    auto q_tiles = [&](int x) { return ((panels - x + 7) >> 3) * minor; };
-    auto tile_of = [&](int x, int t) { return ((t / minor) * 8 + x) * minor + t % minor; };
+    auto minor_of = [&](int p) { return d.p[p].m_fastest ? d.p[p].tiles_m : d.p[p].tiles_n; };
+    auto q_tiles_of = [&](int p, int x) { return (((d.p[p].m_fastest ? d.p[p].tiles_n : d.p[p].tiles_m) - x + 7) >> 3) * minor_of(p); };
+    auto q_tiles = [&](int x) {
+        int n = 0;
+        for (int p = 0; p < d.n; ++p) n += q_tiles_of(p, x);
+        return n;
+    };
+    auto tile_of = [&](int x, int t) {
+        int p = 0;
+        for (; p < d.n - 1; ++p) {
+            const int n = q_tiles_of(p, x);
+            if (t < n) break;
+            t -= n;
+        }
+        const int minor = minor_of(p);
+        return (p << DR_VT_SHIFT) | (((t / minor) * 8 + x) * minor + t % minor);
+    };
+    auto tile_mn = [&](int vt, int& tm, int& tn) {
+        const DrAdamProd& P = d.p[vt >> DR_VT_SHIFT];
+        const int t = vt & ((1 << DR_VT_SHIFT) - 1);
+        tm = P.m_fastest ? (t % P.tiles_m) : (t / P.tiles_n);
+        tn = P.m_fastest ? (t / P.tiles_m) : (t % P.tiles_n);
+    };
     auto draw_blocking = [&]() {
         for (;;) {
             if (visited == 8) return -1;
@@ -326,28 +367,49 @@
         for (int i = 0; i < d.stagger; ++i) __builtin_amdgcn_s_sleep(127);
     int cur = draw_blocking();
     if (cur < 0) return;
-    const int ntiles = d.tiles_m * d.tiles_n;
     const int KSP = d.ksp;
-    const i32x4 srdA = dr_srd(g.A, (uint32_t)(((int64_t)(g.K - 1) * g.lda + g.M) * 4));
-    const i32x4 srdB = dr_srd(g.B, (uint32_t)(((int64_t)(g.K - 1) * g.ldb + g.N) * 4));
-    const uint32_t sa = 16u * (uint32_t)g.lda, sb = 16u * (uint32_t)g.ldb;
-    const int n_lim = g.out2 ? g.N - 1 : g.N;
-    const uint32_t c_bytes = (uint32_t)(((int64_t)(g.M - 1) * g.ldc + n_lim) * 4);
-    const i32x4 srdW = dr_srd(g.C, c_bytes), srdM = dr_srd(g.aux, c_bytes), srdV = dr_srd(g.aux2, c_bytes);
-    const uint32_t ldc4 = (uint32_t)g.ldc * 4u;
-
-    uint32_t offA, offB, ka = 0, kb = 0;
+
+    i32x4 srdA, srdB;
+    uint32_t sa, sb, offA, offB, ka = 0, kb = 0;
     int l_left = KSP;
-    auto set_cursor = [&](int tile) {
-        const bool ok = tile < ntiles;
-        const int tm = d.m_fastest ? (tile % d.tiles_m) : (tile / d.tiles_n);
-        const int tn = d.m_fastest ? (tile / d.tiles_m) : (tile % d.tiles_n);
-        offA = ok ? (uint32_t)(q * g.lda + tm * 64 + 4 * r) * 4u : 0xFFFFFFF0u;
-        offB = ok ? (uint32_t)(q * g.ldb + tn * 64 + 4 * r) * 4u : 0xFFFFFFF0u;
+    auto set_cursor = [&](int vt) {
+        vt = __builtin_amdgcn_readfirstlane(vt);
+        const bool ok = vt != DR_VT_PARK;
+        const int vo = ok ? vt : 0;
+        const DrAdamProd& P = d.p[vo >> DR_VT_SHIFT];
+        int tm, tn;
+        tile_mn(vo, tm, tn);
+        srdA = dr_srd(P.A, (uint32_t)(((int64_t)(P.K - 1) * P.lda + P.M) * 4));
+        srdB = dr_srd(P.B, (uint32_t)(((int64_t)(P.K - 1) * P.ldb + P.N) * 4));
+        sa = 16u * (uint32_t)P.lda;
+        sb = 16u * (uint32_t)P.ldb;
+        offA = ok ? (uint32_t)(q * P.lda + tm * 64 + 4 * r) * 4u : 0xFFFFFFF0u;
+        offB = ok ? (uint32_t)(q * P.ldb + tn * 64 + 4 * r) * 4u : 0xFFFFFFF0u;
         ka = kb = 0;
         l_left = KSP;
     };
     set_cursor(cur);
+    auto c_bytes_of = [&](int p) {
+        const DrAdamProd& P = d.p[p];
+        return (uint32_t)(((int64_t)(P.M - 1) * P.ldc + (P.bias ? P.N - 1 : P.N)) * 4);
+    };
+    i32x4 srdW, srdM, srdV;
+    uint32_t ldc4;
+    GdAdamHyper hy;
+    int pp;
+    auto set_pending_product = [&](int p) {
+        p = __builtin_amdgcn_readfirstlane(p);
+        const DrAdamProd& P = d.p[p];
+        const uint32_t cb = c_bytes_of(p);
+        srdW = dr_srd(P.W, cb);
+        srdM = dr_srd(P.ea, cb);
+        srdV = dr_srd(P.ea2, cb);
+        ldc4 = (uint32_t)P.ldc * 4u;
+        hy = P.adam;
+        if (P.adam_dev) hy = *P.adam_dev;
+        pp = p;
+    };
+    set_pending_product(cur >> DR_VT_SHIFT);
     uint32_t pend_base = PARK;
     bool pend_lane = false;
     int pend_g = 16;
@@ -434,8 +496,8 @@
         unsigned int tick = visited < 8 ? dr_ticket_issue(tctr) : 0u;
         const bool drew = visited < 8;
         int nxt = 0;
-        const int tm = d.m_fastest ? (cur % d.tiles_m) : (cur / d.tiles_n);
-        const int tn = d.m_fastest ? (cur / d.tiles_m) : (cur % d.tiles_n);
+        int tm, tn;
+        tile_mn(cur, tm, tn);
         const int m0 = tm * 64, n0 = tn * 64;
         f32x4 acc[4][4];
 #pragma unroll
@@ -486,7 +548,7 @@
                                     nxt = draw_blocking();
                                 }
                             }
-                            if (nxt < 0) nxt = ntiles;
+                            if (nxt < 0) nxt = DR_VT_PARK;
                             set_cursor(nxt);
                         }
                         __builtin_amdgcn_sched_barrier(0);
@@ -504,6 +566,10 @@
                 __builtin_amdgcn_sched_barrier(0);
             }
         }
+        const int pc = cur >> DR_VT_SHIFT;
+        const DrAdamProd& g = d.p[pc];
+        set_pending_product(pc);
+        const int n_lim = g.bias ? g.N - 1 : g.N;
         const uint32_t vo = (uint32_t)(16 * q * g.ldc + n0 + 4 * r) * 4u;
         const int n = n0 + 4 * r;
         const bool lane_full = n + 3 < n_lim;
@@ -516,9 +582,10 @@
             pend_lane = lane_full;
             pend_g = 0;
         } else if (lane_full) {
-            const __amdgpu_buffer_rsrc_t rW = __builtin_amdgcn_make_buffer_rsrc(g.C, 0, (int)c_bytes, 0x00020000);
-            const __amdgpu_buffer_rsrc_t rM = __builtin_amdgcn_make_buffer_rsrc(const_cast<float*>(g.aux), 0, (int)c_bytes, 0x00020000);
-            const __amdgpu_buffer_rsrc_t rV = __builtin_amdgcn_make_buffer_rsrc(const_cast<float*>(g.aux2), 0, (int)c_bytes, 0x00020000);
+            const int c_bytes = (int)c_bytes_of(pc);
+            const __amdgpu_buffer_rsrc_t rW = __builtin_amdgcn_make_buffer_rsrc(g.W, 0, c_bytes, 0x00020000);
+            const __amdgpu_buffer_rsrc_t rM = __builtin_amdgcn_make_buffer_rsrc(g.ea, 0, c_bytes, 0x00020000);
+            const __amdgpu_buffer_rsrc_t rV = __builtin_amdgcn_make_buffer_rsrc(g.ea2, 0, c_bytes, 0x00020000);
 #pragma unroll
             for (int t = 0; t < 4; ++t)
 #pragma unroll
@@ -541,8 +608,8 @@
                 }
         }
         if (!lane_full && n < g.N) {
-            float* __restrict__ Mo = const_cast<float*>(g.aux);
-            float* __restrict__ Vo = const_cast<float*>(g.aux2);
+            float* __restrict__ Mo = g.ea;
+            float* __restrict__ Vo = g.ea2;
             for (int t = 0; t < 4; ++t)
                 for (int e = 0; e < 4; ++e) {
                     const int m = m0 + 16 * q + 4 * t + e;
@@ -551,19 +618,19 @@
                         if (n + k >= g.N) continue;
                         const int64_t o = (int64_t)m * g.ldc + n + k;
                         const float gk = acc[e][k][t];
-                        if (g.out2 && n + k == g.N - 1) {
-                            g.out2[m] = gk;
+                        if (g.bias && n + k == g.N - 1) {
+                            g.bias[m] = gk;
                             continue;
                         }
-                        float pk = g.C[o], mk = Mo[o], vk = Vo[o];
+                        float pk = g.W[o], mk = Mo[o], vk = Vo[o];
                         gd_adam_elem(pk, gk, mk, vk, hy);
-                        g.C[o] = pk;
+                        g.W[o] = pk;
                         Mo[o] = mk;
                         Vo[o] = vk;
                     }
                 }
         }
-        if (nxt >= ntiles) break;
+        if (nxt == DR_VT_PARK) break;
         cur = nxt;
     }
     dr_wait<0>();
@@ -578,10 +645,13 @@
         opt_update_store(sl[k]);
     }
     dr_wait<0>();
+#if !(GD_ADAMW_DBG & 32)
     {
-        const __amdgpu_buffer_rsrc_t rW = __builtin_amdgcn_make_buffer_rsrc(g.C, 0, (int)c_bytes, 0x00020000);
-        const __amdgpu_buffer_rsrc_t rM = __builtin_amdgcn_make_buffer_rsrc(const_cast<float*>(g.aux), 0, (int)c_bytes, 0x00020000);
-        const __amdgpu_buffer_rsrc_t rV = __builtin_amdgcn_make_buffer_rsrc(const_cast<float*>(g.aux2), 0, (int)c_bytes, 0x00020000);
+        const DrAdamProd& g = d.p[pp];
+        const int c_bytes = (int)c_bytes_of(pp);
+        const __amdgpu_buffer_rsrc_t rW = __builtin_amdgcn_make_buffer_rsrc(g.W, 0, c_bytes, 0x00020000);
+        const __amdgpu_buffer_rsrc_t rM = __builtin_amdgcn_make_buffer_rsrc(g.ea, 0, c_bytes, 0x00020000);
+        const __amdgpu_buffer_rsrc_t rV = __builtin_amdgcn_make_buffer_rsrc(g.ea2, 0, c_bytes, 0x00020000);
         for (; pend_g < 16; pend_g += 4) {
             f32x4 pv[4], mv[4], vv[4];
             uint32_t oo[4];
@@ -610,6 +680,7 @@
             }
         }
     }
+#endif
 }
 
 template <int TMB, int NB, int D, int EPI>
@@ -1490,7 +1561,7 @@
 
 int dr_cu_count_fwd();
 template <int D, bool NTL>
-int dr_tn_adamw_go(const DrArgs& d, hipStream_t s) {
+int dr_tn_adamw_go(const DrMultiArgs& d, hipStream_t s) {
     static bool attr_set = false;
     if (!attr_set) {
         hipError_t e = hipFuncSetAttribute(reinterpret_cast<const void*>(dr_tn_adamw_kernel<D, NTL>),
@@ -1505,16 +1576,20 @@
     return GDMCF_OK;
 }
 
-template <int D, int EPI>
+template <int D>
+int dr_tn_adamw_go(const DrMultiArgs& d, hipStream_t s) {
+    bool lines = true;
+    for (int i = 0; i < d.n; ++i) {
+        const DrAdamProd& p = d.p[i];
+        lines = lines && (p.ldc & 31) == 0 && (((uintptr_t)p.W | (uintptr_t)p.ea | (uintptr_t)p.ea2) & 127) == 0;
+    }
+    static const int force = getenv("GDMCF_DR_NT_LOADS") ? atoi(getenv("GDMCF_DR_NT_LOADS")) : -1;
+    return (force >= 0 ? force != 0 : lines) ? dr_tn_adamw_go<D, true>(d, s) : dr_tn_adamw_go<D, false>(d, s);
+}
+
+template <int D>
 int dr_tn_go(const DrArgs& d, hipStream_t s) {
-    if constexpr (EPI == GD_EPI_ADAMW) {
-        const GdGemm& g = d.g;
-        const bool lines = (g.ldc & 31) == 0 && (((uintptr_t)g.C | (uintptr_t)g.aux | (uintptr_t)g.aux2) & 127) == 0;
-        static const int force = getenv("GDMCF_DR_NT_LOADS") ? atoi(getenv("GDMCF_DR_NT_LOADS")) : -1;
-        return (force >= 0 ? force != 0 : lines) ? dr_tn_adamw_go<D, true>(d, s) : dr_tn_adamw_go<D, false>(d, s);
-    } else {
-        hipLaunchKernelGGL((dr_tn_kernel<1, 1, D, EPI>), dim3(dr_cu_count_fwd()), dim3(512), 0, s, d);
-    }
+    hipLaunchKernelGGL((dr_tn_kernel<1, 1, D, GD_EPI_STORE>), dim3(dr_cu_count_fwd()), dim3(512), 0, s, d);
     return GDMCF_OK;
 }
 
@@ -1561,64 +1636,139 @@
     return (int)(g_dr_seq_eager.fetch_add(1, std::memory_order_relaxed) & 15u);
 }
 
+static bool dr_tn_prepare(int epi, GdGemm& g, DrArgs& d, float** bias_db, int* depth) {
+    const int64_t lim = (int64_t)1 << 32;
+    if ((int64_t)g.K * g.lda * 4 >= lim || (int64_t)g.K * g.ldb * 4 >= lim || (int64_t)g.M * g.ldc * 4 >= lim) return false;
+    if (g.lda < g.M || g.ldb < g.N || g.ldc < g.N) return false;
+    const long tiles = (long)gd_cdiv(g.M, 64) * gd_cdiv(g.N, 64);
+    if (tiles < 512 || g.K < 128) return false;
+    *bias_db = (g.ldb > g.N) ? g.out2 : nullptr;
+    if (*bias_db) g.N += 1;
+    d.tiles_m = gd_cdiv(g.M, 64);
+    d.tiles_n = gd_cdiv(g.N, 64);
+    d.m_fastest = d.tiles_m <= d.tiles_n;
+    {
+        static const int mf = getenv("GDMCF_DR_MF") ? atoi(getenv("GDMCF_DR_MF")) : -1;
+        if (mf >= 0 && epi == GD_EPI_ADAMW) d.m_fastest = mf;
+    }
+    const int ks = gd_cdiv(g.K, 4);
+    int best = 9, waste = 1 << 30;
+    for (int dd : {9, 8, 7}) {
+        const int w = gd_cdiv(ks, dd + 1) * (dd + 1) - ks;
+        if (w < waste) { waste = w; best = dd; }
+    }
+    {
+        static const int forced = getenv("GDMCF_DR_D") ? atoi(getenv("GDMCF_DR_D")) : 0;
+        if (forced >= 7 && forced <= 9) { best = forced; waste = gd_cdiv(ks, best + 1) * (best + 1) - ks; }
+    }
+    d.ksp = ks + waste;
+    *depth = best;
+    g.tiles_m = d.tiles_m;
+    g.tiles_n = d.tiles_n;
+    return true;
+}
+
+static DrAdamProd dr_adam_prod(const GdGemm& g, const DrArgs& d, float* bias_db) {
+    DrAdamProd p = {};
+    p.A = g.A; p.B = g.B; p.W = g.C; p.ea = const_cast<float*>(g.aux); p.ea2 = const_cast<float*>(g.aux2); p.bias = bias_db;
+    p.lda = (int)g.lda; p.ldb = (int)g.ldb; p.ldc = (int)g.ldc;
+    p.M = g.M; p.N = g.N; p.K = g.K;
+    p.tiles_m = d.tiles_m; p.tiles_n = d.tiles_n; p.m_fastest = d.m_fastest;
+    p.adam = g.adam;
+    p.adam_dev = g.adam_dev;
+    return p;
+}
+
+static int dr_adamw_launch(DrMultiArgs& m, int depth, hipStream_t s) {
+    m.ctr = dr_ticket_slot(s);
+    if (depth == 9) return dr_tn_adamw_go<9>(m, s);
+    if (depth == 8) return dr_tn_adamw_go<8>(m, s);
+    return dr_tn_adamw_go<7>(m, s);
+}
+
 int g_gd_dr_force = -1;
+static int dr_on_flags() {
+    static const int on_env = getenv("GDMCF_GEMM_DR") ? atoi(getenv("GDMCF_GEMM_DR")) : 49;
+    return g_gd_dr_force >= 0 ? g_gd_dr_force : on_env;
+}
+static int dr_stagger() {
+    static const int stagger = getenv("GDMCF_DR_STAGGER") ? atoi(getenv("GDMCF_DR_STAGGER")) : 3;
+    return stagger;
+}
+static bool dr_fused_on() {
+    static const int no_fused = getenv("GDMCF_DR_NO_FUSED") ? atoi(getenv("GDMCF_DR_NO_FUSED")) : 0;
+    return (dr_on_flags() & 1) && !no_fused;
+}
+
+int gd_gemm_dr_adamw_multi(GdGemm* gs, int n, hipStream_t s) {
+    if (n < 1 || n > DR_MULTI_MAX || !dr_fused_on()) return GD_DR_NOT_TAKEN;
+    DrMultiArgs m = {};
+    float* bias_db[DR_MULTI_MAX] = {};
+    int n_user[DR_MULTI_MAX] = {};
+    int depth = 0;
+    bool ok = true;
+    double flop = 0.0;
+    for (int i = 0; i < n && ok; ++i) {
+        GdGemm& g = gs[i];
+        ok = !g.bf16 && !g.accumulate && !g.C16 && g.splits <= 1;
+        DrArgs d = {};
+        int dep = 0;
+        n_user[i] = g.N;
+        if (ok) ok = dr_tn_prepare(GD_EPI_ADAMW, g, d, &bias_db[i], &dep);
+        if (ok) {
+            ok = (i == 0 || (dep == depth && d.ksp == m.ksp)) && (long)d.tiles_m * d.tiles_n < (1L << DR_VT_SHIFT);
+            depth = dep;
+            m.ksp = d.ksp;
+            m.p[i] = dr_adam_prod(g, d, bias_db[i]);
+            flop += 2.0 * g.M * n_user[i] * g.K;
+        }
+    }
+    if (!ok) {
+        for (int i = 0; i < n; ++i) gs[i].N = n_user[i] ? n_user[i] : gs[i].N;
+        return GD_DR_NOT_TAKEN;
+    }
+    m.n = n;
+    m.stagger = dr_stagger();
+    {
+        GdProfScope prof(gs[0].prof_tag, flop, s);
+        const int rc = dr_adamw_launch(m, depth, s);
+        if (rc != GDMCF_OK) return rc;
+    }
+    for (int i = 0; i < n; ++i) {
+        gs[i].N = n_user[i];
+        if (bias_db[i]) gs[i].out2 = nullptr;
+    }
+    t_gd_last_gemm = 3;
+    return gd_launch_status("gemm_dr");
+}
+
 int gd_gemm_dr_launch(int layA, int layB, int epi, GdGemm& g, hipStream_t s) {
-    static const int on_env = getenv("GDMCF_GEMM_DR") ? atoi(getenv("GDMCF_GEMM_DR")) : 49;
-    const int on = g_gd_dr_force >= 0 ? g_gd_dr_force : on_env;
+    const int on = dr_on_flags();
     if (!on || g.bf16) return GD_DR_NOT_TAKEN;
     if (g.accumulate || g.C16 || (g.splits > 1 && epi != GD_EPI_SLAB)) return GD_DR_NOT_TAKEN;
-    static const int stagger = getenv("GDMCF_DR_STAGGER") ? atoi(getenv("GDMCF_DR_STAGGER")) : 3;
     const int64_t lim = (int64_t)1 << 32;
     DrArgs d = {};
     d.ctr = -1;
-    d.stagger = stagger;
-    static const int no_fused = getenv("GDMCF_DR_NO_FUSED") ? atoi(getenv("GDMCF_DR_NO_FUSED")) : 0;
-    if ((on & 1) && layA == GD_LAY_MC && layB == GD_LAY_MC && (epi == GD_EPI_STORE || (epi == GD_EPI_ADAMW && !no_fused))) {
-        if ((int64_t)g.K * g.lda * 4 >= lim || (int64_t)g.K * g.ldb * 4 >= lim || (int64_t)g.M * g.ldc * 4 >= lim) return GD_DR_NOT_TAKEN;
-        if (g.lda < g.M || g.ldb < g.N || g.ldc < g.N) return GD_DR_NOT_TAKEN;
-        const long tiles = (long)gd_cdiv(g.M, 64) * gd_cdiv(g.N, 64);
-        if (tiles < 512 || g.K < 128) return GD_DR_NOT_TAKEN;
-        float* const bias_db = (g.ldb > g.N) ? g.out2 : nullptr;
+    d.stagger = dr_stagger();
+    if (epi == GD_EPI_ADAMW && layA == GD_LAY_MC && layB == GD_LAY_MC) return gd_gemm_dr_adamw_multi(&g, 1, s);
+    if ((on & 1) && layA == GD_LAY_MC && layB == GD_LAY_MC && epi == GD_EPI_STORE) {
         const int n_user = g.N;
-        if (bias_db) g.N = n_user + 1;
-        d.tiles_m = gd_cdiv(g.M, 64);
-        d.tiles_n = gd_cdiv(g.N, 64);
-        d.m_fastest = d.tiles_m <= d.tiles_n;
-        {
-            static const int mf = getenv("GDMCF_DR_MF") ? atoi(getenv("GDMCF_DR_MF")) : -1;
-            if (mf >= 0 && epi == GD_EPI_ADAMW) d.m_fastest = mf;
-        }
-        const int ks = gd_cdiv(g.K, 4);
-        int best = 9, waste = 1 << 30;
-        for (int dd : {9, 8, 7}) {
-            const int w = gd_cdiv(ks, dd + 1) * (dd + 1) - ks;
-            if (w < waste) { waste = w; best = dd; }
-        }
-        {
-            static const int forced = getenv("GDMCF_DR_D") ? atoi(getenv("GDMCF_DR_D")) : 0;
-            if (forced >= 7 && forced <= 9) { best = forced; waste = gd_cdiv(ks, best + 1) * (best + 1) - ks; }
-        }
-        d.ksp = ks + waste;
-        g.tiles_m = d.tiles_m;
-        g.tiles_n = d.tiles_n;
+        float* bias_db = nullptr;
+        int best = 9;
+        if (!dr_tn_prepare(epi, g, d, &bias_db, &best)) {
+            g.N = n_user;
+            return GD_DR_NOT_TAKEN;
+        }
         d.g = g;
         d.ctr = dr_ticket_slot(s);
-        d.adam_dev = epi == GD_EPI_ADAMW ? g.adam_dev : nullptr;
         d.g.out2 = bias_db;
         {
             GdProfScope prof(g.prof_tag, 2.0 * g.M * n_user * g.K, s);
-#define GD_DR_GO(DD)                                                      \
-    do {                                                                  \
-        int rc_ = (epi == GD_EPI_STORE) ? dr_tn_go<DD, GD_EPI_STORE>(d, s) : dr_tn_go<DD, GD_EPI_ADAMW>(d, s); \
-        if (rc_ != GDMCF_OK) return rc_;                                  \
-    } while (0)
-            if (best == 9) GD_DR_GO(9);
-            else if (best == 8) GD_DR_GO(8);
-            else GD_DR_GO(7);
-#undef GD_DR_GO
+            int rc_ = best == 9 ? dr_tn_go<9>(d, s) : best == 8 ? dr_tn_go<8>(d, s) : dr_tn_go<7>(d, s);
+            if (rc_ != GDMCF_OK) return rc_;
         }
         g.N = n_user;
-        t_gd_last_gemm = epi == GD_EPI_ADAMW ? 3 : 2;
+        t_gd_last_gemm = 2;
         if (bias_db) g.out2 = nullptr;
         return gd_launch_status("gemm_dr");
     }
diff --git a/gdmcf_amd/csrc/linear.hip b/gdmcf_amd/csrc/linear.hip
--- a/gdmcf_amd/csrc/linear.hip
+++ b/gdmcf_amd/csrc/linear.hip
@@ -78,6 +78,30 @@
     return db;
 }
 
+int dw_adamw_setup(const GdDwAdamw& e, GdGemm& g, int& cls) {
+    GD_CHECK_SHAPE(e.M > 0 && e.N > 0 && e.K > 0 && e.lddz >= e.N && e.lda >= e.K && e.ldw >= e.K, "linear_bwd_weight_adamw: bad shape");
+    GD_CHECK_ARG(e.W && e.exp_avg && e.exp_avg_sq && e.step >= 1, "linear_bwd_weight_adamw: optimizer state missing");
+    const int M = e.M, N = e.N, K = e.K;
+    cls = pick_class_dw(N, K, t_gemm_prec, true);
+    g = GdGemm{};
+    g.bf16 = t_gemm_prec;
+    g.A = e.dZ; g.lda = e.lddz; g.B = e.A; g.ldb = e.lda; g.M = N; g.N = K; g.K = M; g.splits = 1;
+    g.m_fastest = gd_cdiv(N, gd_gemm_tile_m(cls)) <= gd_cdiv(K, gd_gemm_tile_n(cls));
+    g.C = e.W; g.ldc = e.ldw; g.aux = e.exp_avg; g.aux2 = e.exp_avg_sq; g.prof_tag = 5;
+    g.adam = gd_adam_hyper(e.lr, e.beta1, e.beta2, e.eps, e.weight_decay, e.step, e.grad_scale);
+    g.adam_dev = t_gd_step_state ? &t_gd_step_state->hyper : nullptr;
+    attach_result_shadow(g);
+    attach_shadows(g, GD_LAY_MC, GD_LAY_MC);
+    g.out2 = bias_col_request(e.a_scale_col, e.lda, e.rowscale, K, e.db);
+    return GDMCF_OK;
+}
+
+int dw_adamw_finish(const GdDwAdamw& e, bool asked, const GdGemm& g, hipStream_t s) {
+    if (asked && g.out2 == nullptr) return GDMCF_OK;
+    if (e.db) return gd_colsum(e.dZ, e.lddz, e.rowscale, e.M, e.N, e.db, s);
+    return GDMCF_OK;
+}
+
 }
 
 extern "C" {
@@ -291,25 +315,49 @@
                                       int a_scale_col, int M, int N, int K, float* W, int64_t ldw, float* exp_avg, float* exp_avg_sq,
                                       float* db, float lr, float beta1, float beta2, float eps, float weight_decay,
                                       int step, float grad_scale, void* stream) {
-    GD_CHECK_SHAPE(M > 0 && N > 0 && K > 0 && lddz >= N && lda >= K && ldw >= K, "linear_bwd_weight_adamw: bad shape");
-    GD_CHECK_ARG(W && exp_avg && exp_avg_sq && step >= 1, "linear_bwd_weight_adamw: optimizer state missing");
-    hipStream_t s = (hipStream_t)stream;
-    const int cls = pick_class_dw(N, K, t_gemm_prec, true);
-    GdGemm g = {};
-    g.bf16 = t_gemm_prec;
-    g.A = dZ; g.lda = lddz; g.B = A; g.ldb = lda; g.M = N; g.N = K; g.K = M; g.splits = 1;
-    g.m_fastest = gd_cdiv(N, gd_gemm_tile_m(cls)) <= gd_cdiv(K, gd_gemm_tile_n(cls));
-    g.C = W; g.ldc = ldw; g.aux = exp_avg; g.aux2 = exp_avg_sq; g.prof_tag = 5;
-    g.adam = gd_adam_hyper(lr, beta1, beta2, eps, weight_decay, step, grad_scale);
-    g.adam_dev = t_gd_step_state ? &t_gd_step_state->hyper : nullptr;
-    attach_result_shadow(g);
-    attach_shadows(g, GD_LAY_MC, GD_LAY_MC);
-    g.out2 = bias_col_request(a_scale_col, lda, rowscale, K, db);
+    const GdDwAdamw e = {dZ, lddz, A, lda, rowscale, a_scale_col, M, N, K, W, ldw, exp_avg, exp_avg_sq, db,
+                         lr, beta1, beta2, eps, weight_decay, step, grad_scale};
+    GdGemm g;
+    int cls;
+    int rc = dw_adamw_setup(e, g, cls);
+    if (rc) return rc;
     const bool asked = g.out2 != nullptr;
-    int rc = gd_gemm_launch(GD_LAY_MC, GD_LAY_MC, GD_EPI_ADAMW, cls, g, s);
-    if (rc) return rc;
-    if (asked && g.out2 == nullptr) return GDMCF_OK;
-    if (db) return gd_colsum(dZ, lddz, rowscale, M, N, db, s);
+    rc = gd_gemm_launch(GD_LAY_MC, GD_LAY_MC, GD_EPI_ADAMW, cls, g, (hipStream_t)stream);
+    if (rc) return rc;
+    return dw_adamw_finish(e, asked, g, (hipStream_t)stream);
+}
+
+int gdmcf_linear_bwd_weight_adamw_multi_f32(const GdDwAdamw* list, int n, void* stream) {
+    GD_CHECK_ARG(n >= 0 && (n == 0 || list), "linear_bwd_weight_adamw_multi: bad list");
+    hipStream_t s = (hipStream_t)stream;
+    constexpr int MAXN = 4;
+    for (int i0 = 0; i0 < n; i0 += MAXN) {
+        const int k = n - i0 < MAXN ? n - i0 : MAXN;
+        GdGemm g[MAXN];
+        bool asked[MAXN];
+        int cls;
+        for (int j = 0; j < k; ++j) {
+            const int rc = dw_adamw_setup(list[i0 + j], g[j], cls);
+            if (rc) return rc;
+            asked[j] = g[j].out2 != nullptr;
+        }
+        int rc = gd_gemm_dr_adamw_multi(g, k, s);
+        if (rc == GD_DR_NOT_TAKEN) {
+            for (int j = 0; j < k; ++j) {
+                const GdDwAdamw& e = list[i0 + j];
+                rc = gdmcf_linear_bwd_weight_adamw_f32(e.dZ, e.lddz, e.A, e.lda, e.rowscale, e.a_scale_col, e.M, e.N, e.K, e.W,
+                                                       e.ldw, e.exp_avg, e.exp_avg_sq, e.db, e.lr, e.beta1, e.beta2, e.eps,
+                                                       e.weight_decay, e.step, e.grad_scale, stream);
+                if (rc) return rc;
+            }
+            continue;
+        }
+        if (rc) return rc;
+        for (int j = 0; j < k; ++j) {
+            rc = dw_adamw_finish(list[i0 + j], asked[j], g[j], s);
+            if (rc) return rc;
+        }
+    }
     return GDMCF_OK;
 }
 
diff --git a/gdmcf_amd/engine.py b/gdmcf_amd/engine.py
--- a/gdmcf_amd/engine.py
+++ b/gdmcf_amd/engine.py
@@ -1,5 +1,7 @@
 
+import ctypes
 import functools
+import os
 
 import torch
 
@@ -372,6 +374,7 @@
         dWe = dbe = None
         fused = self.fused_opt if self.grad_sink is None else None
         dz, lddz, rs = dz_last, ld_last, rowscale
+        dw_queue = [] if (fused is not None and self.gemm_dtype == "f32" and os.environ.get("GDMCF_DW_MULTI", "1") != "0") else None
 
         def input_grad(li, w, A_prev, lda_prev, N, K):
             nonlocal dWe, dbe
@@ -403,12 +406,18 @@
             if fs is not None:
                 if fs["exp_avg"].stride() != w.stride() or fs["exp_avg_sq"].stride() != w.stride():
                     raise RuntimeError("gdmcf_amd: the moments of a fused weight must share its leading dimension")
-                _lib.check(lib.gdmcf_linear_bwd_weight_adamw_f32(
-                    dz.data_ptr(), lddz, A_use.data_ptr(), lda_use, _lib.ptr(rs), scol, B, N, K, w.data_ptr(), w.stride(0),
-                    fs["exp_avg"].data_ptr(), fs["exp_avg_sq"].data_ptr(), db.data_ptr(), fs["lr"], fs["beta1"],
-                    fs["beta2"], fs["eps"], fs["weight_decay"], fs["step"], fs["grad_scale"], st))
-                if not (self.gemm_dtype == "bf16" and _lib.shadow_info(w.data_ptr()) is not None):
-                    torch.autograd.graph.increment_version(w)
+                if dw_queue is not None:
+                    dw_queue.append((_lib.GdDwAdamw(
+                        dz.data_ptr(), lddz, A_use.data_ptr(), lda_use, _lib.ptr(rs), scol, B, N, K, w.data_ptr(), w.stride(0),
+                        fs["exp_avg"].data_ptr(), fs["exp_avg_sq"].data_ptr(), db.data_ptr(), fs["lr"], fs["beta1"],
+                        fs["beta2"], fs["eps"], fs["weight_decay"], fs["step"], fs["grad_scale"]), w))
+                else:
+                    _lib.check(lib.gdmcf_linear_bwd_weight_adamw_f32(
+                        dz.data_ptr(), lddz, A_use.data_ptr(), lda_use, _lib.ptr(rs), scol, B, N, K, w.data_ptr(), w.stride(0),
+                        fs["exp_avg"].data_ptr(), fs["exp_avg_sq"].data_ptr(), db.data_ptr(), fs["lr"], fs["beta1"],
+                        fs["beta2"], fs["eps"], fs["weight_decay"], fs["step"], fs["grad_scale"], st))
+                    if not (self.gemm_dtype == "bf16" and _lib.shadow_info(w.data_ptr()) is not None):
+                        torch.autograd.graph.increment_version(w)
                 dW = None
             else:
                 dW = self._grad_like(w)
@@ -444,6 +453,11 @@
                 weight_grad(li, w, bias, A_prev, lda_prev, N, K)
                 nxt = input_grad(li, w, A_prev, lda_prev, N, K)
             dz, lddz, rs = nxt
+        if dw_queue:
+            arr = (_lib.GdDwAdamw * len(dw_queue))(*[e for e, _ in dw_queue])
+            _lib.check(lib.gdmcf_linear_bwd_weight_adamw_multi_f32(ctypes.addressof(arr), len(dw_queue), st))
+            for _, w in dw_queue:
+                torch.autograd.graph.increment_version(w)
         if self._side2_used:
             torch.cuda.current_stream().wait_stream(self._side2)
             self._side2_used = False
diff --git a/include/gdmcf_hip.h b/include/gdmcf_hip.h
--- a/include/gdmcf_hip.h
+++ b/include/gdmcf_hip.h
@@ -102,6 +102,23 @@
                                       int64_t ldw, float* exp_avg, float* exp_avg_sq, float* db, float lr,
                                       float beta1, float beta2, float eps, float weight_decay, int step,
                                       float grad_scale, void* stream);
+typedef struct GdDwAdamw {
+    const float* dZ;
+    int64_t lddz;
+    const float* A;
+    int64_t lda;
+    const float* rowscale;
+    int a_scale_col, M, N, K;
+    float* W;
+    int64_t ldw;
+    float* exp_avg;
+    float* exp_avg_sq;
+    float* db;
+    float lr, beta1, beta2, eps, weight_decay;
+    int step;
+    float grad_scale;
+} GdDwAdamw;
+int gdmcf_linear_bwd_weight_adamw_multi_f32(const GdDwAdamw* list, int n, void* stream);
 int gdmcf_rowscale_f32(const float* A, int64_t lda, const float* rowscale, int M, int K, float* out,
                        int64_t ldo, void* stream);
 int gdmcf_row_norms_f32(const float* X, int64_t ld, int rows, int cols, float* norm, float* inv_norm,
```
